# bittremieux/falcon

Hardware: AMD Instinct MI355X
Metric: spectra clustered/sec @1/2/4/8 GPU; cosine-kernel HBM GB/s vs roofline (higher is better)
Workload: dtype f32; 1 GPU; one dataset of 1000000 synthetic spectra (1000000 per GPU; charges 2+3; precursor m/z 400-1200), low_dim=400, n_neighbors=64, n_neighbors_ann=128, n_probe=16, eps=0.1, precursor_tol=20ppm, mz_interval=1.0, batch_size=32768; exchange=none, parallelism=1 GPU

## Files before the change

falcon_amd/_lib.py:

```python
from __future__ import annotations

import ctypes as C
import os
from typing import Optional

_HERE = os.path.dirname(os.path.abspath(__file__))
LIB_PATH = os.path.join(_HERE, "libfalcon_hip.so")

FAL_DTYPE_F32, FAL_DTYPE_F16, FAL_DTYPE_SPLIT16, FAL_OUT_F32_F16, FAL_OUT_F16_IMAGE = 0, 1, 2, 3, 4
PEAK_F64, PEAK_ZLIB, PEAK_BIG_ENDIAN, PEAK_PAIRS = 1, 2, 4, 8
PEAK_NUMPRESS_LINEAR, PEAK_NUMPRESS_PIC, PEAK_NUMPRESS_SLOF, PEAK_NUMPRESS_MASK = 16, 32, 48, 48
PEAK_STATUS = {1: "bad descriptor", 2: "bad base64", 4: "bad zlib header", 8: "bad deflate stream", 16: "more values than declared",
               32: "fewer values than declared", 64: "Adler-32 mismatch", 128: "decode buffer too small",
               256: "bad MS-Numpress stream"}
MGF_FLAG_BYTES, MGF_FLAG_LINES, MGF_ST_HOST = 1, 2, 1
MGF_NUM_MAX = 23
FAL_EINVAL = -1
MZML_FLAG_STRUCT, MZML_FLAG_MARKUP, MZML_FLAG_TAGS = 1, 2, 4
MZML_ST_OK, MZML_ST_SKIP, MZML_ST_HOST = 0, 1, 2
CONS_FALLBACK, CONS_GLOBAL, CONS_CAPACITY, CONS_LDS_PEAKS = 1, 2, 4, 4096
STAGES = {"vectorize": 0, "build": 1, "coarse": 2, "scan": 3, "select": 4, "filter": 5, "dbscan": 6, "tail": 7,
          "kernel": 8}


class FalconHipError(RuntimeError):
    pass


_lib: Optional[C.CDLL] = None

c_void_p, c_int, c_int64, c_uint32, c_float, c_double = C.c_void_p, C.c_int, C.c_int64, C.c_uint32, C.c_float, C.c_double
P = C.POINTER

_SIGNATURES = {
    "fal_version": ([], c_int),
    "fal_last_error": ([], C.c_char_p),
    "fal_device_count": ([P(c_int)], c_int),
    "fal_ctx_create": ([c_int, c_void_p, c_int, P(c_void_p)], c_int),
    "fal_ctx_destroy": ([c_void_p], c_int),
    "fal_ctx_sync": ([c_void_p], c_int),
    "fal_ctx_plan": ([c_void_p, c_int64, c_int, c_int, c_int, c_int64], c_int),
    "fal_ctx_trim": ([c_void_p], c_int),
    "fal_ctx_stage_ms": ([c_void_p, c_int, P(c_float), P(c_int64)], c_int),
    "fal_ctx_enable_timing": ([c_void_p, c_int], c_int),
    "fal_ctx_counter": ([c_void_p, c_int, P(c_int64)], c_int),
    "fal_get_dim": ([c_float, c_float, c_float, P(c_uint32), P(c_float), P(c_float)], c_int),
    "fal_hash_lookup": ([c_uint32, c_uint32, c_uint32, c_void_p], c_int),
    "fal_to_vector_indices": ([c_void_p, c_void_p, c_int64, c_double, c_double, c_void_p], c_int),
    "fal_vectorize": ([c_void_p, c_void_p, c_void_p, c_void_p, c_void_p, c_int64, c_double, c_double,
                       c_uint32, c_uint32, c_uint32, c_int, c_int, c_void_p], c_int),
    "fal_vectorize_pair": ([c_void_p, c_void_p, c_void_p, c_void_p, c_void_p, c_int64, c_double, c_double,
                            c_uint32, c_uint32, c_uint32, c_int, c_void_p, c_void_p], c_int),
    "fal_vectorize_f16_image": ([c_void_p, c_void_p, c_void_p, c_void_p, c_void_p, c_int64, c_double, c_double,
                                 c_uint32, c_uint32, c_uint32, c_int, c_void_p, c_void_p], c_int),
    "fal_row_width": ([c_uint32, P(c_uint32)], c_int),
    "fal_vectorize_rows": ([c_void_p, c_void_p, c_void_p, c_void_p, c_void_p, c_int64, c_double, c_double,
                            c_uint32, c_uint32, c_uint32, c_uint32, c_int, c_int, c_void_p, c_void_p], c_int),
    "fal_window_counts": ([c_void_p, c_void_p, c_void_p, c_int, c_double, c_int64, c_void_p, c_void_p], c_int),
    "fal_window_select": ([c_void_p, c_void_p, c_int64, c_double, c_int64, c_void_p, c_int, c_void_p, c_void_p, P(c_int64)], c_int),
    "fal_precursor_splits": ([c_void_p, c_void_p, c_int64, c_double, c_int, c_int64, c_double, c_int,
                              c_void_p, c_int64, P(c_int64)], c_int),
    "fal_ivf_build": ([c_void_p, c_void_p, c_int64, c_int, c_void_p, c_int64, c_void_p, c_int, P(c_void_p)], c_int),
    "fal_ivf_build_x16": ([c_void_p, c_void_p, c_void_p, c_int64, c_int, c_void_p, c_int64, c_void_p, c_int, P(c_void_p)], c_int),
    "fal_ivf_attach_f16": ([c_void_p, c_void_p, c_int], c_int),
    "fal_ivf_attach_prefilter": ([c_void_p, c_void_p], c_int),
    "fal_ivf_attach_prefilter_ex": ([c_void_p, c_void_p, c_int], c_int),
    "fal_ivf_destroy": ([c_void_p], c_int),
    "fal_ivf_total_lists": ([c_void_p, P(c_int64)], c_int),
    "fal_ivf_export": ([c_void_p, c_void_p, c_void_p, c_void_p, c_void_p, c_void_p], c_int),
    "fal_ivf_search_topk": ([c_void_p, c_void_p, c_int, c_int, c_void_p, c_void_p], c_int),
    "fal_filter_neighbors": ([c_void_p, c_void_p, c_void_p, c_int64, c_int, c_void_p, c_void_p, c_double, c_int,
                              c_double, c_int, c_void_p, c_void_p], c_int),
    "fal_ivf_search_neighbors": ([c_void_p, c_void_p, c_int, c_int, c_void_p, c_void_p, c_double, c_int, c_double, c_int,
                                  c_void_p, c_void_p, c_void_p], c_int),
    "fal_process_spectra": ([c_void_p, c_void_p, c_void_p, c_void_p, c_int64, c_int64, c_void_p, c_void_p, c_int, c_double,
                             c_double, c_double, c_double, c_double, c_int, c_int, c_void_p, c_void_p, c_void_p,
                             c_void_p], c_int),
    "fal_rescore_neighbors": ([c_void_p, c_void_p, c_void_p, c_int64, c_int, c_void_p, c_void_p, c_void_p, c_void_p, c_double,
                               c_int], c_int),
    "fal_neighbors_to_csr": ([c_void_p, c_void_p, c_void_p, c_void_p, c_int64, c_int, c_int64, c_int64, c_void_p, c_void_p, c_void_p],
                             c_int),
    "fal_neighbors_to_csr_mapped": ([c_void_p, c_void_p, c_void_p, c_void_p, c_int64, c_int, c_void_p, c_int64, c_int64, c_void_p,
                                     c_void_p, c_void_p], c_int),
    "fal_dbscan": ([c_void_p, c_void_p, c_void_p, c_int64, c_int, c_float, c_void_p, P(c_int64)], c_int),
    "fal_refine_clusters": ([c_void_p, c_void_p, c_int64, c_void_p, c_void_p, c_double, c_int, c_double,
                             P(c_int64)], c_int),
    "fal_finalize": ([c_void_p, c_void_p, c_int64, c_int64, c_void_p, c_void_p, c_void_p, c_int, c_void_p,
                      c_void_p, P(c_int64)], c_int),
    "fal_cluster_graph": ([c_void_p, c_void_p, c_void_p, c_int64, c_int, c_float, c_void_p, c_void_p, c_double, c_int,
                           c_double, c_void_p, c_void_p, c_void_p, c_void_p, P(c_int64), P(c_int64)], c_int),
    "fal_cluster_graph_counted": ([c_void_p, c_void_p, c_void_p, c_void_p, c_int64, c_int, c_float, c_void_p, c_void_p, c_double,
                                   c_int, c_double, c_void_p, c_void_p, c_void_p, c_void_p, P(c_int64), P(c_int64)], c_int),
    "fal_cluster_graph_linkage": ([c_void_p, c_void_p, c_void_p, c_int64, c_int, c_float, c_int, c_void_p, c_void_p, c_double, c_int,
                                   c_double, c_void_p, c_void_p, c_void_p, c_void_p, P(c_int64), P(c_int64)], c_int),
    "fal_linkage_cluster": ([c_void_p, c_void_p, c_void_p, c_int64, c_int, c_float, c_int, c_void_p, P(c_int64)], c_int),
    "fal_exact_edges": ([c_void_p, c_void_p, c_void_p, c_void_p, c_void_p, c_int64, c_void_p, c_int64, c_double, c_int, c_double,
                         c_void_p, c_void_p, c_void_p, c_int64, P(c_int64)], c_int),
    "fal_linkage_cluster_csr": ([c_void_p, c_void_p, c_void_p, c_void_p, c_int64, c_double, c_int, c_void_p, c_void_p, c_void_p,
                                 c_void_p, c_double, c_int, c_void_p, P(c_int64)], c_int),
    "fal_cluster_exact": ([c_void_p, c_void_p, c_void_p, c_void_p, c_void_p, c_int64, c_void_p, c_int64, c_double, c_int, c_double,
                           c_int, c_void_p, c_void_p, c_double, c_int, c_double, c_void_p, c_void_p, c_void_p, P(c_int64),
                           P(c_int64)], c_int),
    "fal_sort_by_precursor": ([c_void_p, c_void_p, c_int64, c_void_p, c_void_p], c_int),
    "fal_gather_f32": ([c_void_p, c_void_p, c_void_p, c_int64, c_void_p], c_int),
    "fal_decode_peaks": ([c_void_p, c_void_p, c_int64, c_void_p, c_int64, c_void_p, c_int64, c_int64, c_int64, c_void_p, c_void_p,
                          c_void_p, c_void_p], c_int),
    "fal_mgf_index": ([c_void_p, c_void_p, c_int64, P(c_int64)], c_int),
    "fal_mgf_parse": ([c_void_p, c_void_p, c_int64, c_int64, c_int64, c_void_p, c_void_p, c_void_p, c_void_p, c_void_p, c_void_p,
                       c_void_p, c_void_p, c_void_p, c_void_p], c_int),
    "fal_mgf_write_sizes": ([c_void_p, c_void_p, c_void_p, c_void_p, c_int64, c_int64, c_void_p, c_int64, c_void_p, c_void_p, c_void_p,
                             c_void_p, c_void_p, c_int64, c_void_p, c_void_p, P(c_int64)], c_int),
    "fal_mgf_write": ([c_void_p, c_void_p, c_void_p, c_void_p, c_int64, c_int64, c_void_p, c_int64, c_void_p, c_void_p, c_void_p,
                       c_void_p, c_void_p, c_void_p, c_int64, c_void_p, c_int64, c_int64, c_void_p, c_int64, c_void_p], c_int),
    "fal_mzml_index": ([c_void_p, c_void_p, c_int64, P(c_int64)], c_int),
    "fal_mzml_parse": ([c_void_p, c_void_p, c_int64, c_int64, c_void_p, c_int64, c_void_p, c_void_p, c_void_p, c_void_p, c_void_p,
                        c_void_p, c_void_p], c_int),
    "fal_consensus_spectra": ([c_void_p, c_void_p, c_void_p, c_void_p, c_int64, c_void_p, c_void_p, c_int64, c_double, c_double,
                               c_int64, c_void_p, c_void_p, c_void_p, c_void_p], c_int),
    "fal_assign_nearest": ([c_void_p, c_void_p, c_void_p, c_void_p, c_void_p, c_void_p, c_int64, c_void_p, c_void_p, c_void_p,
                            c_void_p, c_void_p, c_int64, c_double, c_int, c_double, c_double, c_int, c_void_p, c_void_p,
                            c_void_p], c_int),
}


def load() -> C.CDLL:
    global _lib
    if _lib is not None:
        return _lib
    if not os.path.isfile(LIB_PATH):
        raise FalconHipError(
            f"{LIB_PATH} is missing: build it with `python -c 'import __graft_entry__ as g; g.build()'` "
            f"(or `make -C falcon_amd/csrc`). falcon_amd has no CPU fallback.")
    import torch
    lib = C.CDLL(LIB_PATH)
    for name, (args, res) in _SIGNATURES.items():
        fn = getattr(lib, name)
        fn.argtypes = args
        fn.restype = res
    _lib = lib
    return lib


def check(rc: int, what: str = "") -> None:
    if rc != 0:
        msg = load().fal_last_error().decode("utf-8", "replace")
        raise FalconHipError(f"{what or 'libfalcon_hip'} failed with code {rc}: {msg}")


def exported_symbols():
    return list(_SIGNATURES)
```

falcon_amd/cluster/cluster.py:

```python
from __future__ import annotations

import logging
import math
from dataclasses import dataclass
from typing import Optional, Tuple

import numpy as np

from .. import device as _device

logger = logging.getLogger("falcon")

F16_INDEX_DIMS = (64, 128, 256, 400, 800)
F16_FLAT_DIMS = (64, 128, 256, 400)
FLAT_MAX = 100
MIN_PTS_PER_LIST = 39
MAX_N_LIST = 1 << 17


class _DefaultClustering(str):
    """AnnParams.clustering's default "dbscan" -- equal to the string, but distinguishable from an explicit choice
    (exact mode turns the default into "hierarchical" and refuses an explicit "dbscan")"""


@dataclass
class AnnParams:
    eps: float = 0.1
    low_dim: int = 400
    n_probe: int = 16
    n_neighbors: int = 64
    n_neighbors_ann: int = 128
    mz_interval: float = 1.0
    kmeans_iters: int = 10
    hash_seed: int = 0
    min_mz: float = 101.0
    max_mz: float = 1500.0
    dtype: str = "f32"
    f16_index: bool = True
    scan: str = "f32"
    prefilter: bool = False
    ivf_prefilter: bool = True
    kmeans_prefilter: bool = True
    rescore: bool = False
    min_matches: int = 0
    clustering: str = _DefaultClustering("dbscan")
    linkage: str = "complete"
    exact: bool = False


def n_list_rule(sizes: np.ndarray, n_probe: int) -> np.ndarray:
    sizes = np.asarray(sizes, np.int64)
    nl = np.ones(len(sizes), np.int64)
    big = sizes > FLAT_MAX
    if big.any():
        nl[big] = 2 ** np.floor(np.log2(sizes[big] / MIN_PTS_PER_LIST)).astype(np.int64)
    nl = np.minimum(nl, MAX_N_LIST)
    nl[nl <= n_probe] = 1
    return nl.astype(np.int32)


class SpectrumDataset:

    def __init__(self, precursor_mz, retention_time, mz, intensity, indptr, precursor_charge=None):
        self.precursor_mz, self.retention_time = precursor_mz, retention_time
        self.mz, self.intensity, self.indptr = mz, intensity, indptr
        self.precursor_charge = precursor_charge

    def __len__(self):
        return int(self.precursor_mz.shape[0])

    def columns(self):
        return (self.precursor_mz, self.retention_time, self.mz, self.intensity, self.indptr)

    def on_host(self) -> bool:
        return not any(t is not None and hasattr(t, "is_cuda") and t.is_cuda for t in self.columns())

    def to_device(self, dev, non_blocking: bool = True) -> "SpectrumDataset":
        import torch
        want = (torch.float32, torch.float32, torch.float32, torch.float32, torch.int64)
        up = []
        for t, dt in zip(self.columns(), want):
            if t is None:
                up.append(None)
                continue
            if not isinstance(t, torch.Tensor):
                t = torch.from_numpy(np.ascontiguousarray(t, dtype=np.float32 if dt == torch.float32 else np.int64))
            up.append(t.to(dev, dtype=dt, non_blocking=non_blocking))
        return SpectrumDataset(*up, self.precursor_charge)

    def take_rows(self, rows: np.ndarray) -> "SpectrumDataset":
        import torch
        as_np = lambda t: t.numpy() if isinstance(t, torch.Tensor) else np.asarray(t)
        rows = np.asarray(rows, np.int64)
        indptr = as_np(self.indptr)
        cnt = indptr[rows + 1] - indptr[rows]
        out = np.zeros(len(rows) + 1, np.int64)
        np.cumsum(cnt, out=out[1:])
        pos = np.repeat(indptr[rows] - out[:-1], cnt) + np.arange(int(out[-1]), dtype=np.int64)

        def pick(col, idx, dt):
            src = as_np(col)
            t = torch.empty(len(idx), dtype=dt, pin_memory=torch.cuda.is_available())
            dst = t.numpy()
            if src.dtype == dst.dtype:
                np.take(src, idx, out=dst)
            else:
                dst[:] = src[idx]
            return t
        rt = None if self.retention_time is None else pick(self.retention_time, rows, torch.float32)
        return SpectrumDataset(pick(self.precursor_mz, rows, torch.float32), rt, pick(self.mz, pos, torch.float32),
                               pick(self.intensity, pos, torch.float32), torch.from_numpy(out), self.precursor_charge)

    @classmethod
    def from_table(cls, table):
        if hasattr(table, "to_pandas"):
            table = table.to_pandas()
        mzs = [np.asarray(x, np.float32) for x in table["mz"]]
        its = [np.asarray(x, np.float32) for x in table["intensity"]]
        indptr = np.zeros(len(mzs) + 1, np.int64)
        np.cumsum([len(x) for x in mzs], out=indptr[1:])
        cat = lambda xs: np.concatenate(xs) if xs else np.zeros(0, np.float32)
        return cls(np.asarray(table["precursor_mz"], np.float32), np.asarray(table["retention_time"], np.float32),
                   cat(mzs), cat(its), indptr,
                   np.asarray(table["precursor_charge"]) if "precursor_charge" in table else None)


class ClusterPipeline:

    def __init__(self, ctx: Optional[_device.Context] = None, device: int = 0):
        self.ctx = ctx or _device.Context(device)
        self.last = {}

    def plan(self, n: int, batch_size: int, p: "AnnParams"):
        if p.exact:
            return
        key = (int(n), int(batch_size), p.low_dim, p.n_neighbors_ann, p.n_probe)
        if getattr(self, "_planned", None) is not None and self._planned[0] >= key[0] and self._planned[1:] == key[1:]:
            return
        self.ctx.plan(n, _device.row_width(p.low_dim), p.n_neighbors_ann, p.n_probe, batch_size)
        self._planned = key

    def trim(self):
        import torch
        for c in (self.ctx, getattr(self, "_front_ctx", None)):
            if c is not None:
                c.trim()
        self._planned = None
        torch.cuda.empty_cache()

    def _front(self, c, ds, precursor_tol_mass, precursor_tol_mode, rt_tol, batch_size, p, pmz=None):
        import torch
        if pmz is None:
            pmz = c.to_dev(ds.precursor_mz, torch.float32)
        order, mzs = c.sort_by_precursor(pmz)
        rts = c.gather_f32(ds.retention_time, order) if (rt_tol is not None and ds.retention_time is not None) else None
        splits = c.precursor_splits(mzs, precursor_tol_mass, precursor_tol_mode, batch_size, p.mz_interval)
        n_list = n_list_rule(np.diff(splits), p.n_probe)
        if p.dtype == "f16" and not p.f16_index:
            n_list[:] = 1
        return dict(order=order, mzs=mzs, rts=rts, splits=splits, n_list=n_list)

    def plan_shards(self, c, datasets, batch_size, p, world, tol=None):
        import torch
        from .. import distributed as fdist
        for ds in datasets:
            if ds.on_host():
                ds._pmz_dev = c.to_dev(ds.precursor_mz, torch.float32)
        counts = c.window_counts([getattr(ds, "_pmz_dev", None) if ds.on_host() else ds.precursor_mz for ds in datasets],
                                 p.mz_interval)
        if p.exact:
            costs = fdist.exact_window_costs(counts, batch_size)
        else:
            costs = fdist.window_costs(counts, batch_size, p.n_probe, p.mz_interval, tol, p.n_neighbors_ann, p.n_neighbors)
        return fdist.deal_job(list(costs), world)

    def _front_windows(self, c, ds, precursor_tol_mass, precursor_tol_mode, rt_tol, batch_size, p, shard, owner=None):
        import torch
        from .. import distributed as fdist
        rank, world = shard[0], shard[1]
        pmz = ds.__dict__.pop("_pmz_dev", None) if ds.on_host() else None
        if pmz is None:
            pmz = c.to_dev(ds.precursor_mz, torch.float32)
        n = int(pmz.numel())
        if owner is None:
            owner = self.plan_shards(c, [ds], batch_size, p, world, tol=(precursor_tol_mass, precursor_tol_mode))[0]
        if len(owner) and (owner == rank).all():
            st = self._front(c, ds, precursor_tol_mass, precursor_tol_mode, rt_tol, batch_size, p, pmz=pmz)
            st.update(rows=st["order"], n_total=n)
            return st
        if not (owner == rank).any():
            rows = torch.zeros(0, dtype=torch.int64, device=c.tdev)
        else:
            rows, mz_sub = c.window_select(pmz, p.mz_interval, owner, rank)
        if rows.numel() == 0:
            e = rows.new_zeros(0)
            return dict(order=e, mzs=pmz[:0], rts=None, splits=np.zeros(1, np.int64), n_list=np.zeros(0, np.int32), rows=e,
                        n_total=n)
        order_sub, mzs = c.sort_by_precursor(mz_sub)
        rows_sorted = rows[order_sub]
        rts = c.gather_f32(ds.retention_time, rows_sorted) if (rt_tol is not None and ds.retention_time is not None) else None
        splits = c.precursor_splits(mzs, precursor_tol_mass, precursor_tol_mode, batch_size, p.mz_interval)
        n_list = n_list_rule(np.diff(splits), p.n_probe)
        if p.dtype == "f16" and not p.f16_index:
            n_list[:] = 1
        return dict(order=rows_sorted, mzs=mzs, rts=rts, splits=splits, n_list=n_list, rows=rows_sorted, n_total=n)

    def _restrict(self, c, st, p, shard):
        import torch
        from .. import distributed as fdist
        rank, world = shard
        splits = np.asarray(st["splits"], np.int64)
        sizes = np.diff(splits)
        costs = fdist.exact_bucket_costs(sizes) if p.exact else fdist.bucket_costs(sizes, st["n_list"], p.n_probe)
        owner = fdist.shard_units(costs, world)
        first, sizes, sub_splits, mine = fdist.shard_buckets(splits, owner, rank)
        n_sub = int(sub_splits[-1])
        if n_sub:
            shift = c.to_dev(np.stack([first - sub_splits[:-1], sizes]), torch.int64)
            pos_d = torch.repeat_interleave(shift[0], shift[1], output_size=n_sub) + torch.arange(n_sub, device=c.tdev)
        order_sub = st["order"][pos_d] if n_sub else st["order"][:0]
        rts = st["rts"]
        return dict(order=order_sub, mzs=st["mzs"][pos_d] if n_sub else st["mzs"][:0],
                    rts=None if rts is None else (rts[pos_d] if n_sub else rts[:0]), splits=sub_splits,
                    n_list=np.asarray(st["n_list"])[mine], rows=order_sub, n_total=int(st["order"].numel()),
                    buckets=mine)

    def _search(self, ds, st, precursor_tol_mass, precursor_tol_mode, rt_tol, fragment_tol, p, keep_intermediates):
        c = self.ctx
        order, mzs, rts, splits, n_list = st["order"], st["mzs"], st["rts"], st["splits"], st["n_list"]
        n_bins, start, _ = _device.get_dim(p.min_mz, p.max_mz, fragment_tol)
        all_flat = bool((n_list == 1).all())
        W = _device.row_width(p.low_dim)
        assert W in F16_INDEX_DIMS
        vec = lambda dt: c.vectorize(ds.mz, ds.intensity, ds.indptr, order, start, fragment_tol, n_bins, p.low_dim,
                                     p.hash_seed, True, dt, width=W)
        X = X16 = Xpre = Xkm = None
        which = 0
        if p.dtype not in ("f32", "f16"):
            raise ValueError(f"unknown dtype {p.dtype!r} (f32 or f16)")
        if p.dtype == "f16" and not all_flat:
            X, X16 = vec("f16+image")
            Xkm = X16 if p.kmeans_prefilter else None
            if p.ivf_prefilter and not keep_intermediates:
                which, Xpre = 2, X16
        elif p.dtype == "f16":
            X16 = vec("f16")
        elif p.scan == "f16x3":
            if W not in F16_FLAT_DIMS:
                raise ValueError(f"scan='f16x3' needs low_dim <= {F16_FLAT_DIMS[-1]} (got {p.low_dim})")
            X16 = vec("split16")
            if not all_flat:
                X = vec("f32")
        else:
            if p.prefilter and not keep_intermediates and W in F16_FLAT_DIMS and bool((n_list == 1).any()):
                which |= 1
            if p.ivf_prefilter and not keep_intermediates and bool((n_list > 1).any()):
                which |= 2
            want_km = p.kmeans_prefilter and bool(((n_list > 1) & (n_list <= 2048)).any())
            if want_km or which:
                X, x16 = vec("f32+f16")
                Xkm = x16 if want_km else None
                Xpre = x16 if which else None
            else:
                X = vec("f32")
        index = c.ivf_build(X, splits, n_list, p.kmeans_iters, X16=X16, Xpre=Xpre, Xkm=Xkm, prefilter_which=max(which, 1))
        if keep_intermediates:
            sim, idx = index.search(p.n_probe, p.n_neighbors_ann)
            nb_idx, nb_dist = c.filter_neighbors(sim, idx, mzs, rts, precursor_tol_mass, precursor_tol_mode, rt_tol,
                                                 p.n_neighbors)
            st.update(sim=sim, idx=idx)
        else:
            nb_idx, nb_dist = index.search_neighbors(p.n_probe, p.n_neighbors_ann, mzs, rts, precursor_tol_mass,
                                                     precursor_tol_mode, rt_tol, p.n_neighbors)
        if p.rescore:
            nb_dist = c.rescore_neighbors(nb_idx, nb_dist, ds.mz, ds.intensity, ds.indptr, order, fragment_tol,
                                          p.min_matches)
        st.update(X=X, X16=X16, Xpre=Xpre, index=index, nb_idx=nb_idx, nb_dist=nb_dist,
                  nb_count=None if keep_intermediates else index.nb_count)

    def _graph(self, st, precursor_tol_mass, precursor_tol_mode, rt_tol, p, keep_intermediates):
        c = self.ctx
        order, mzs, rts, nb_idx, nb_dist, index = (st[k] for k in ("order", "mzs", "rts", "nb_idx", "nb_dist", "index"))
        hier = p.linkage if p.clustering == "hierarchical" else None
        if keep_intermediates:
            db, n_db = c.linkage_cluster(nb_idx, nb_dist, p.eps, hier) if hier else c.dbscan(nb_idx, nb_dist, p.eps)
            last = dict(order=order, mz_sorted=mzs, rt_sorted=rts, splits=st["splits"], X=st["X"], X16=st["X16"],
                        n_list=st["n_list"], sim=st["sim"], idx=st["idx"], nb_idx=nb_idx, nb_dist=nb_dist, db=db.clone(),
                        n_db=n_db, index=index)
            lab, n_cl = c.refine_clusters(db, n_db, mzs, rts, precursor_tol_mass, precursor_tol_mode, rt_tol)
            last.update(lab_sorted=lab, n_clusters=n_cl)
            labels, medoids = c.finalize(lab, n_cl, order, nb_idx, nb_dist)
        else:
            labels, medoids, _, _ = c.cluster_graph(nb_idx, nb_dist, p.eps, mzs, rts, precursor_tol_mass,
                                                    precursor_tol_mode, rt_tol, order, linkage=hier, nb_count=st["nb_count"])
            last = dict(nb_idx=nb_idx, nb_dist=nb_dist, nb_count=st["nb_count"], order=order, n_list=st["n_list"],
                        splits=st["splits"])
            index.close()
        return labels, medoids, last

    def _exact(self, ds, st, precursor_tol_mass, precursor_tol_mode, rt_tol, fragment_tol, p, keep_intermediates):
        c = self.ctx
        order, mzs, rts, splits = (st[k] for k in ("order", "mzs", "rts", "splits"))
        last = dict(order=order, mz_sorted=mzs, rt_sorted=rts, splits=splits, csr=None)
        if keep_intermediates:
            last["csr"] = c.exact_edges(ds.mz, ds.intensity, ds.indptr, order, splits, fragment_tol, p.min_matches, p.eps)
        labels, medoids, lab_sorted, n_cl = c.cluster_exact(ds.mz, ds.intensity, ds.indptr, order, splits, fragment_tol,
                                                            p.min_matches, p.eps, p.linkage, mzs, rts, precursor_tol_mass,
                                                            precursor_tol_mode, rt_tol)
        last.update(lab_sorted=lab_sorted, n_clusters=n_cl)
        return labels, medoids, last

    def run(self, ds: SpectrumDataset, precursor_tol_mass: float, precursor_tol_mode: str,
            rt_tol: Optional[float], fragment_tol: float, batch_size: int, p: AnnParams,
            keep_intermediates: bool = False):
        import torch
        c = self.ctx
        if len(ds) == 0:
            return c.empty((0,), torch.int32), c.empty((0,), torch.int32)
        self.plan(len(ds), batch_size, p)
        st = self._front(c, ds, precursor_tol_mass, precursor_tol_mode, rt_tol, batch_size, p)
        if p.exact:
            labels, medoids, self.last = self._exact(ds, st, precursor_tol_mass, precursor_tol_mode, rt_tol, fragment_tol, p,
                                                     keep_intermediates)
            return labels, medoids
        self._search(ds, st, precursor_tol_mass, precursor_tol_mode, rt_tol, fragment_tol, p, keep_intermediates)
        labels, medoids, self.last = self._graph(st, precursor_tol_mass, precursor_tol_mode, rt_tol, p, keep_intermediates)
        return labels, medoids

    def run_many(self, datasets, precursor_tol_mass: float, precursor_tol_mode: str, rt_tol: Optional[float],
                 fragment_tol: float, batch_size: int, p: AnnParams, shard: Optional[Tuple[int, int]] = None):
        import torch
        c = self.ctx
        if p.exact and shard is not None and shard[1] > 1:
            return self._run_many_exact_sharded(datasets, precursor_tol_mass, precursor_tol_mode, rt_tol, fragment_tol,
                                                batch_size, p, shard)
        if p.exact:
            outs, self.lasts = [], []
            for ds in datasets:
                outs.append(self.run(ds, precursor_tol_mass, precursor_tol_mode, rt_tol, fragment_tol, batch_size, p))
                self.lasts.append(self.last if len(ds) > 0 else {})
            if self.lasts:
                self.last = self.lasts[-1]
            return outs
        args = (precursor_tol_mass, precursor_tol_mode, rt_tol)
        live = [i for i, ds in enumerate(datasets) if len(ds) > 0]
        if live:
            self.plan(max(len(datasets[i]) for i in live), batch_size, p)
        if len(live) > 1 and not hasattr(self, "_front_ctx"):
            self._front_stream = torch.cuda.Stream(device=c.tdev)
            with torch.cuda.stream(self._front_stream):
                self._front_ctx = _device.Context(c.device)
        front_stream = self._front_stream if len(live) > 1 else torch.cuda.current_stream(c.tdev)
        front_ctx = self._front_ctx if len(live) > 1 else c
        states = {}
        sharded = shard is not None and shard[1] > 1
        windows = sharded and bool(p.mz_interval and p.mz_interval > 0)
        owners = None
        if windows:
            owners = shard[2] if len(shard) > 2 else None
            if owners is None:
                front_stream.wait_stream(torch.cuda.current_stream(c.tdev))
                with torch.cuda.stream(front_stream):
                    owners = self.plan_shards(front_ctx, datasets, batch_size, p, shard[1], tol=args[:2])

        def front(i):
            with torch.cuda.stream(front_stream):
                if windows:
                    st = self._front_windows(front_ctx, datasets[i], *args, batch_size, p, shard, owner=owners[i])
                else:
                    st = self._front(front_ctx, datasets[i], *args, batch_size, p)
                    if sharded:
                        st = self._restrict(front_ctx, st, p, shard[:2])
                if sharded:
                    st["order"] = torch.arange(st["rows"].numel(), dtype=torch.int64, device=c.tdev)
                states[i] = st

        if live:
            front_stream.wait_stream(torch.cuda.current_stream(c.tdev))
            front(live[0])
        for pos, i in enumerate(live):
            if states[i]["order"].numel() > 0:
                if sharded and datasets[i].on_host():
                    front_stream.synchronize()
                    sub = datasets[i].take_rows(states[i]["rows"].cpu().numpy())
                    sub = SpectrumDataset(None, None, c.to_dev(sub.mz), c.to_dev(sub.intensity), c.to_dev(sub.indptr))
                    self._search(sub, states[i], *args, fragment_tol, p, False)
                elif sharded:
                    st = dict(states[i], order=states[i]["rows"])
                    torch.cuda.current_stream(c.tdev).wait_stream(front_stream)
                    self._search(datasets[i], st, *args, fragment_tol, p, False)
                    st["order"] = states[i]["order"]
                    states[i] = st
                else:
                    self._search(datasets[i], states[i], *args, fragment_tol, p, False)
            if pos + 1 < len(live):
                front(live[pos + 1])
        outs, self.lasts = [], []
        for i, ds in enumerate(datasets):
            if len(ds) == 0 or states[i]["order"].numel() == 0:
                outs.append((c.empty((0,), torch.int32), c.empty((0,), torch.int32)))
                self.lasts.append({"rows": c.empty((0,), torch.int64)} if sharded else {})
                continue
            labels, medoids, last = self._graph(states[i], *args, p, False)
            if sharded:
                last["rows"] = states[i]["rows"]
            outs.append((labels, medoids))
            self.lasts.append(last)
        if self.lasts:
            self.last = self.lasts[-1]
        return outs

    def _run_many_exact_sharded(self, datasets, precursor_tol_mass, precursor_tol_mode, rt_tol, fragment_tol, batch_size, p,
                                shard):
        import torch
        c = self.ctx
        args = (precursor_tol_mass, precursor_tol_mode, rt_tol)
        windows = bool(p.mz_interval and p.mz_interval > 0)
        owners = shard[2] if len(shard) > 2 else None
        if windows and owners is None:
            owners = self.plan_shards(c, datasets, batch_size, p, shard[1])
        outs, self.lasts = [], []
        for j, ds in enumerate(datasets):
            st = None
            if len(ds) > 0:
                if windows:
                    st = self._front_windows(c, ds, *args, batch_size, p, shard[:2], owner=owners[j])
                else:
                    st = self._restrict(c, self._front(c, ds, *args, batch_size, p), p, shard[:2])
            if st is None or st["rows"].numel() == 0:
                outs.append((c.empty((0,), torch.int32), c.empty((0,), torch.int32)))
                self.lasts.append({"rows": c.empty((0,), torch.int64)})
                continue
            rows = st["rows"]
            st["order"] = torch.arange(rows.numel(), dtype=torch.int64, device=c.tdev)
            labels, medoids, last = self._exact(self._take_rows(c, ds, rows), st, *args, fragment_tol, p, False)
            last["rows"] = rows
            outs.append((labels, medoids))
            self.lasts.append(last)
        if self.lasts:
            self.last = self.lasts[-1]
        return outs

    @staticmethod
    def _take_rows(c, ds, rows):
        import torch
        if ds.on_host():
            sub = ds.take_rows(rows.cpu().numpy())
            return SpectrumDataset(None, None, c.to_dev(sub.mz), c.to_dev(sub.intensity), c.to_dev(sub.indptr))
        indptr = c.to_dev(ds.indptr, torch.int64)
        start = indptr[rows]
        cnt = indptr[rows + 1] - start
        out = torch.zeros(rows.numel() + 1, dtype=torch.int64, device=c.tdev)
        torch.cumsum(cnt, 0, out=out[1:])
        nnz = int(out[-1].item())
        pos = torch.repeat_interleave(start - out[:-1], cnt, output_size=nnz) + torch.arange(nnz, device=c.tdev)
        return SpectrumDataset(None, None, c.to_dev(ds.mz, torch.float32)[pos], c.to_dev(ds.intensity, torch.float32)[pos],
                               out)

    def run_chunked(self, datasets, precursor_tol_mass: float, precursor_tol_mode: str, rt_tol: Optional[float],
                    fragment_tol: float, batch_size: int, p: AnnParams, n_chunks: int, on_chunk=None):
        import torch
        c = self.ctx
        if n_chunks <= 1 or p.exact:
            return self.run_many(datasets, precursor_tol_mass, precursor_tol_mode, rt_tol, fragment_tol, batch_size, p)
        labels = [torch.full((len(ds),), -1, dtype=torch.int32, device=c.tdev) for ds in datasets]
        medoids = [[] for _ in datasets]
        off = [0] * len(datasets)
        for ch in range(n_chunks):
            outs = self.run_many(datasets, precursor_tol_mass, precursor_tol_mode, rt_tol, fragment_tol, batch_size, p,
                                 shard=(ch, n_chunks))
            _merge_share(labels, medoids, off, outs, self.lasts)
            if on_chunk is not None:
                on_chunk(ch, outs, self.lasts)
            del outs
        return [(labels[j], torch.cat(medoids[j]) if medoids[j] else c.empty((0,), torch.int32)) for j in range(len(datasets))]


def _merge_share(labels, medoids, off, outs, lasts):
    import torch
    for j, ((lab, med), last) in enumerate(zip(outs, lasts)):
        rows = last.get("rows")
        if rows is None or rows.numel() == 0:
            continue
        labels[j][rows] = lab + off[j]
        medoids[j].append(rows[med.long()].to(torch.int32))
        off[j] += int(med.numel())


class PartitionRunner:

    def __init__(self, device: int = 0, n_slots: int = 2):
        import threading
        from concurrent.futures import ThreadPoolExecutor
        self.device, self.n_slots = device, n_slots
        self._tls = threading.local()
        self._pool = ThreadPoolExecutor(max_workers=n_slots, thread_name_prefix="falcon-part")
        self.pipelines = []
        self._lock = threading.Lock()

    def _pipeline(self):
        import torch
        if not hasattr(self._tls, "pipe"):
            torch.cuda.set_device(self.device)
            self._tls.stream = torch.cuda.Stream(device=self.device)
            with torch.cuda.stream(self._tls.stream):
                self._tls.pipe = ClusterPipeline(device=self.device)
            with self._lock:
                self.pipelines.append(self._tls.pipe)
        return self._tls.pipe, self._tls.stream

    def _run_one(self, ds, args, kwargs, shard, arrived=None):
        import torch
        pipe, stream = self._pipeline()
        with torch.cuda.stream(stream):
            if arrived is not None:
                stream.wait_event(arrived)
            if shard is not None and shard[1] > 1:
                out = pipe.run_many([ds], *args, shard=shard, **kwargs)[0]
                pipe.last = pipe.lasts[0]
            else:
                out = pipe.run(ds, *args, **kwargs)
            stream.synchronize()
        return out, pipe, dict(pipe.last)

    def run(self, datasets, *args, shard: Optional[Tuple[int, int]] = None, **kwargs):
        return self.collect(self.submit(datasets, *args, shard=shard, **kwargs))

    def collect(self, handle):
        futs, n, nothing = handle
        res = [futs[i].result()[::2] if i in futs else nothing() for i in range(n)]
        self.lasts = [r[1] for r in res]
        return [r[0] for r in res]

    def submit(self, datasets, *args, shard: Optional[Tuple[int, int]] = None, inputs_ready: bool = False, **kwargs):
        import torch
        if not inputs_ready:
            torch.cuda.current_stream(self.device).synchronize()
        p = args[5] if len(args) > 5 else kwargs["p"]
        order = sorted(range(len(datasets)), key=lambda i: -len(datasets[i]))
        shards = [shard] * len(datasets)
        if shard is not None and shard[1] > 1 and p.mz_interval and p.mz_interval > 0:
            if not hasattr(self, "_planner"):
                self._planner = ClusterPipeline(device=self.device)
            owners = self._planner.plan_shards(self._planner.ctx, datasets, args[4], p, shard[1], tol=args[:2])
            shards = [(shard[0], shard[1], [owners[i]]) for i in range(len(datasets))]
            order = [i for i in order if (owners[i] == shard[0]).any()]
        dev = torch.device("cuda", self.device)
        arrived = {}
        sharded = shard is not None and shard[1] > 1
        if not sharded and any(datasets[i].on_host() for i in order):
            if not hasattr(self, "_copy_stream"):
                self._copy_stream = torch.cuda.Stream(device=self.device)
            datasets = list(datasets)
            with torch.cuda.stream(self._copy_stream):
                for i in order:
                    if datasets[i].on_host():
                        datasets[i] = datasets[i].to_device(dev)
                        arrived[i] = torch.cuda.Event()
                        arrived[i].record(self._copy_stream)
        futs = {i: self._pool.submit(self._run_one, datasets[i], args, kwargs, shards[i], arrived.get(i)) for i in order}
        nothing = lambda: ((torch.empty(0, dtype=torch.int32, device=dev), torch.empty(0, dtype=torch.int32, device=dev)),
                           {"rows": torch.empty(0, dtype=torch.int64, device=dev)})
        return futs, len(datasets), nothing

    def plan(self, datasets, *args, **kwargs):
        import threading
        n = max((len(ds) for ds in datasets), default=0)
        batch_size, p = args[4], args[5]
        gate = threading.Barrier(self.n_slots)

        def one():
            pipe, stream = self._pipeline()
            import torch
            with torch.cuda.stream(stream):
                pipe.plan(n, batch_size, p)
            gate.wait()
        for f in [self._pool.submit(one) for _ in range(self.n_slots)]:
            f.result()

    def trim(self):
        with self._lock:
            pipes = list(self.pipelines)
        for pipe in pipes + ([self._planner] if hasattr(self, "_planner") else []):
            pipe.trim()

    def run_chunked(self, datasets, *args, n_chunks: int, on_chunk=None, **kwargs):
        import torch
        if n_chunks <= 1 or (args[5] if len(args) > 5 else kwargs["p"]).exact:
            return self.run(datasets, *args, **kwargs)
        dev = torch.device("cuda", self.device)
        labels = [torch.full((len(ds),), -1, dtype=torch.int32, device=dev) for ds in datasets]
        medoids = [[] for _ in datasets]
        off = [0] * len(datasets)
        for ch in range(n_chunks):
            outs = self.run(datasets, *args, shard=(ch, n_chunks), **kwargs)
            _merge_share(labels, medoids, off, outs, self.lasts)
            if on_chunk is not None:
                on_chunk(ch, outs, self.lasts)
            del outs
        return [(labels[j], torch.cat(medoids[j]) if medoids[j] else torch.empty(0, dtype=torch.int32, device=dev))
                for j in range(len(datasets))]

    def close(self):
        self._pool.shutdown(wait=True)


_default_pipeline: Optional[ClusterPipeline] = None


def resolve_params(linkage: str, distance_threshold: float, min_matches: int, ann: Optional[AnnParams] = None) -> AnnParams:
    import dataclasses
    if linkage not in ("complete", "single", "average"):
        raise ValueError(f"unknown linkage {linkage!r} (choose complete, single or average; cluster.py:283-290)")
    if ann is None:
        p = AnnParams(eps=float(distance_threshold))
    else:
        if abs(float(ann.eps) - float(distance_threshold)) > 1e-12:
            raise ValueError(f"distance_threshold ({distance_threshold}) and ann.eps ({ann.eps}) differ: they name the same "
                             "cosine-distance threshold (README.md:73-79, config.py:104-111)")
        p = dataclasses.replace(ann)
    if p.rescore:
        p.min_matches = int(min_matches)
    if p.exact:
        if p.clustering == "dbscan" and not isinstance(p.clustering, _DefaultClustering):
            raise ValueError("exact mode clusters the all-pairs distances hierarchically (the snapshot's linkage); "
                             "AnnParams(exact=True) does not combine with clustering=\"dbscan\"")
        p.clustering = "hierarchical"
    if p.clustering not in ("dbscan", "hierarchical"):
        raise ValueError(f"unknown clustering {p.clustering!r}")
    if p.clustering == "hierarchical":
        p.linkage = linkage
        p.rescore = True
        p.min_matches = int(min_matches)
    elif linkage != "complete":
        raise ValueError(f"linkage={linkage!r} only applies to the hierarchical clustering of the exact distances "
                         "(AnnParams(clustering=\"hierarchical\", rescore=True) / --clustering hierarchical); the default "
                         "nearest-neighbour path clusters with DBSCAN and would ignore it")
    return p


def generate_clusters(dataset, linkage: str, distance_threshold: float, min_matches: int,
                      precursor_tol_mass: float, precursor_tol_mode: str, rt_tol: Optional[float],
                      fragment_tol: float, batch_size: int, *, ann: Optional[AnnParams] = None,
                      pipeline: Optional[ClusterPipeline] = None) -> Tuple[np.ndarray, np.ndarray]:
    global _default_pipeline
    if not isinstance(dataset, SpectrumDataset):
        dataset = SpectrumDataset.from_table(
            dataset.to_table(columns=["precursor_mz", "precursor_charge", "retention_time", "mz", "intensity"])
            if hasattr(dataset, "to_table") else dataset)
    p = resolve_params(linkage, distance_threshold, min_matches, ann)
    pipe = pipeline or _default_pipeline
    if pipe is None:
        pipe = _default_pipeline = ClusterPipeline()
    logger.info("Cluster %d spectra: low_dim=%d n_probe=%d n_neighbors=%d/%d eps=%.3f", len(dataset), p.low_dim,
                p.n_probe, p.n_neighbors, p.n_neighbors_ann, p.eps)
    labels, medoids = pipe.run(dataset, precursor_tol_mass, precursor_tol_mode, rt_tol, fragment_tol, batch_size, p)
    return labels.cpu().numpy(), medoids.cpu().numpy()


def consensus_spectra(dataset, labels, medoids, fragment_tol: float, min_fraction: float = 0.25,
                      pipeline: Optional[ClusterPipeline] = None):
    global _default_pipeline
    if not isinstance(dataset, SpectrumDataset):
        dataset = SpectrumDataset.from_table(
            dataset.to_table(columns=["precursor_mz", "precursor_charge", "retention_time", "mz", "intensity"])
            if hasattr(dataset, "to_table") else dataset)
    if not 0.0 < float(min_fraction) <= 1.0:
        raise ValueError("min_fraction must lie in (0, 1]")
    pipe = pipeline or _default_pipeline
    if pipe is None:
        pipe = _default_pipeline = ClusterPipeline()
    indptr, mz, intensity, status = pipe.ctx.consensus_spectra(dataset.mz, dataset.intensity, dataset.indptr, labels, medoids,
                                                               fragment_tol, min_fraction)
    return indptr.cpu().numpy(), mz.cpu().numpy(), intensity.cpu().numpy(), status.cpu().numpy()


def write_representatives(filename: str, dataset: SpectrumDataset, medoids, cluster_ids, identifiers, charge: int = 0,
                          consensus=None, pipeline: Optional[ClusterPipeline] = None) -> str:
    global _default_pipeline
    from ..ms_io import ms_io
    pipe = pipeline or _default_pipeline
    if pipe is None:
        pipe = _default_pipeline = ClusterPipeline()
    if dataset.retention_time is None:
        raise ValueError("write_representatives: the dataset has no retention times")
    ctx = pipe.ctx
    import torch
    m = ctx.to_dev(medoids, torch.int64)
    n = int(m.shape[0])
    if consensus is None:
        indptr, mz, intensity, rows = dataset.indptr, dataset.mz, dataset.intensity, m.to(torch.int32)
    else:
        indptr, mz, intensity = consensus
        rows = np.arange(n, dtype=np.int32)
    pmz, rt = ctx.to_dev(dataset.precursor_mz, torch.float32)[m], ctx.to_dev(dataset.retention_time, torch.float32)[m]
    return ms_io.write_representatives(filename, ctx, mz, intensity, indptr, rows, pmz, rt, np.full(n, int(charge), np.int32),
                                       cluster_ids, np.asarray(identifiers, dtype=str))


def assign_to_library(queries: SpectrumDataset, library: SpectrumDataset, eps: float, precursor_tol: float, mode: str,
                      rt_tol: Optional[float], fragment_tol: float, min_matched_peaks: int,
                      pipeline: Optional[ClusterPipeline] = None):
    global _default_pipeline
    pipe = pipeline or _default_pipeline
    if pipe is None:
        pipe = _default_pipeline = ClusterPipeline()
    if mode not in ("ppm", "Da"):
        raise ValueError(f"unknown precursor tolerance mode {mode!r} (ppm or Da)")
    row, dist, cand = pipe.ctx.assign_nearest(queries.mz, queries.intensity, queries.indptr, queries.precursor_mz,
                                              queries.retention_time, library.mz, library.intensity, library.indptr,
                                              library.precursor_mz, library.retention_time, precursor_tol, mode, rt_tol,
                                              fragment_tol, min_matched_peaks)
    row, dist, cand = row.cpu().numpy(), dist.cpu().numpy(), cand.cpu().numpy()
    return row, dist, cand, (row >= 0) & (dist <= np.float32(eps))
```

falcon_amd/csrc/common.h:

```cpp
#pragma once
#include <hip/hip_runtime.h>
#include <stdint.h>
#include <stdio.h>
#include <string.h>
#include <string>
#include <vector>
#include "../../include/falcon_hip.h"

namespace fal {

void set_error(const char* fmt, ...);

#define FAL_CHECK_HIP(expr)                                                          \
    do {                                                                             \
        hipError_t _e = (expr);                                                      \
        if (_e != hipSuccess) {                                                      \
            fal::set_error("%s:%d: %s failed: %s", __FILE__, __LINE__, #expr,        \
                           hipGetErrorString(_e));                                   \
            return (_e == hipErrorOutOfMemory) ? FAL_ENOMEM : FAL_EHIP;              \
        }                                                                            \
    } while (0)

#define FAL_REQUIRE(cond, code, ...)                                                 \
    do {                                                                             \
        if (!(cond)) {                                                               \
            fal::set_error(__VA_ARGS__);                                             \
            return (code);                                                           \
        }                                                                            \
    } while (0)

#define FAL_TRY(expr)                                                                \
    do {                                                                             \
        int _r = (expr);                                                             \
        if (_r != FAL_OK) return _r;                                                 \
    } while (0)

constexpr int kNumStages = 9;
constexpr int kNumSlots = 50;
enum Stage { ST_VECTORIZE = 0, ST_BUILD = 1, ST_COARSE = 2, ST_SCAN = 3, ST_SELECT = 4,
             ST_FILTER = 5, ST_DBSCAN = 6, ST_TAIL = 7,
             ST_KERNEL = 8 };

struct Scratch {
    void* ptr = nullptr;
    size_t cap = 0;
};

}

struct fal_ctx {
    int device = -1;
    hipStream_t stream = nullptr;
    bool own_stream = false;
    void* pinned = nullptr;
    size_t pinned_cap = 0;
    int pinned_reserve(size_t bytes, void** out);
    unsigned char* arena = nullptr;
    size_t arena_off = 0;
    int upload(void* dst, const void* src, size_t bytes);
    int num_cus = 256;
    int persistent_wgs = 256;
    bool timing = false;
    struct StageTimer {
        std::vector<std::pair<hipEvent_t, hipEvent_t>> ev;
        size_t used = 0;
    } timers[fal::kNumStages];
    fal::Scratch scratch[fal::kNumSlots];
    int32_t* fb_host = nullptr;
    int32_t* zero_dev = nullptr;
    int64_t counters[10] = {0, 0, 0, 0, 0, 0, 0, 0, 0, 0};

    struct TextIndex {
        const void* text = nullptr;
        int64_t bytes = -1, spectra = 0, extra = 0, cap_table = 0, cap_spectra = 0;
        const void* blocks[4] = {nullptr, nullptr, nullptr, nullptr};
    } mgf, mzml;

    struct PoolBlock { void* ptr; size_t cap; bool used; };
    std::vector<PoolBlock> pool;
    int pool_alloc(size_t bytes, void** out);
    void pool_free(void* ptr);

    bool debug_poison = false;
    int call_depth = 0;
    uint64_t call_epoch = 1;
    uint64_t slot_epoch[fal::kNumSlots] = {};
    uint32_t slot_gen[fal::kNumSlots] = {};
    std::vector<void*> retired;
    std::vector<bool> retired_held;
    void release_retired();
    int reserve(int slot, size_t bytes, void** out);
    void release(int slot) { slot_epoch[slot] = 0; }
    void stage_reset(int stage);
    int stage_begin(int stage, hipEvent_t* stop_out, hipStream_t on = nullptr);
    int stage_end(hipEvent_t stop, hipStream_t on = nullptr);
};

namespace fal {

struct StageScope {
    fal_ctx* c;
    hipEvent_t stop = nullptr;
    bool on;
    hipStream_t s;
    StageScope(fal_ctx* ctx, int stage, hipStream_t stream = nullptr, bool enable = true)
        : c(ctx), on(ctx->timing && enable), s(stream) {
        if (on) c->stage_begin(stage, &stop, s);
    }
    ~StageScope() {
        if (on && stop) c->stage_end(stop, s);
    }
};

struct CallScope {
    fal_ctx* c;
    explicit CallScope(fal_ctx* ctx) : c(ctx) {
        if (c && c->call_depth++ == 0) {
            ++c->call_epoch;
            if (!c->retired.empty()) c->release_retired();
        }
    }
    ~CallScope() {
        if (c) --c->call_depth;
    }
};

static inline int64_t ceil_div(int64_t a, int64_t b) { return (a + b - 1) / b; }

struct WarmReg {
    explicit WarmReg(const void* kernel);
};
#define FAL_WARM_KERNEL(...) static const ::fal::WarmReg _fal_warm_reg((const void*)(__VA_ARGS__))

__device__ __forceinline__ void wave_lds_sync() {
    __builtin_amdgcn_fence(__ATOMIC_RELEASE, "workgroup");
    __builtin_amdgcn_wave_barrier();
    asm volatile("" ::: "memory");
}

typedef unsigned short ushort2v __attribute__((ext_vector_type(2)));
__device__ __forceinline__ uint32_t pk_sub(uint32_t x, uint32_t y) {
    return __builtin_bit_cast(uint32_t, (ushort2v)(__builtin_bit_cast(ushort2v, x) - __builtin_bit_cast(ushort2v, y)));
}
__device__ __forceinline__ uint32_t pk_add(uint32_t x, uint32_t y) {
    return __builtin_bit_cast(uint32_t, (ushort2v)(__builtin_bit_cast(ushort2v, x) + __builtin_bit_cast(ushort2v, y)));
}
__device__ __forceinline__ uint32_t pk_sub_sat(uint32_t x, uint32_t y) {
    uint32_t r;
    asm("v_pk_sub_u16 %0, %1, %2 clamp" : "=v"(r) : "v"(x), "v"(y));
    return r;
}
__device__ __forceinline__ uint32_t pk_min(uint32_t x, uint32_t y) {
    uint32_t r;
    asm("v_pk_min_u16 %0, %1, %2" : "=v"(r) : "v"(x), "v"(y));
    return r;
}
__device__ __forceinline__ uint32_t pk_max(uint32_t x, uint32_t y) {
    uint32_t r;
    asm("v_pk_max_u16 %0, %1, %2" : "=v"(r) : "v"(x), "v"(y));
    return r;
}

#define FAL_DPP_SCAN(v, OP, IDENT)                                                                  \
    v = OP(v, __builtin_amdgcn_update_dpp(IDENT, v, 0x111, 0xF, 0xF, false));                       \
    v = OP(v, __builtin_amdgcn_update_dpp(IDENT, v, 0x112, 0xF, 0xF, false));                       \
    v = OP(v, __builtin_amdgcn_update_dpp(IDENT, v, 0x114, 0xF, 0xF, false));                       \
    v = OP(v, __builtin_amdgcn_update_dpp(IDENT, v, 0x118, 0xF, 0xF, false));                       \
    v = OP(v, __builtin_amdgcn_update_dpp(IDENT, v, 0x142, 0xA, 0xF, false));                       \
    v = OP(v, __builtin_amdgcn_update_dpp(IDENT, v, 0x143, 0xC, 0xF, false));
__device__ __forceinline__ int fal_add_i(int a, int b) { return a + b; }
__device__ __forceinline__ int fal_min_i(int a, int b) { return a < b ? a : b; }
__device__ __forceinline__ int fal_max_i(int a, int b) { return a > b ? a : b; }
__device__ __forceinline__ int wave_prefix_sum(int v) {
    FAL_DPP_SCAN(v, fal_add_i, 0)
    return v;
}
__device__ __forceinline__ int wave_min(int v) {
    FAL_DPP_SCAN(v, fal_min_i, 0x7FFFFFFF)
    return __builtin_amdgcn_readlane(v, 63);
}
__device__ __forceinline__ uint32_t wave_min_u32(uint32_t u) {
    int v = (int)(u ^ 0x80000000u);
    FAL_DPP_SCAN(v, fal_min_i, 0x7FFFFFFF)
    return (uint32_t)__builtin_amdgcn_readlane(v, 63) ^ 0x80000000u;
}
__device__ __forceinline__ uint32_t wave_max_u32(uint32_t u) {
    int v = (int)(u ^ 0x80000000u);
    FAL_DPP_SCAN(v, fal_max_i, (int)0x80000000)
    return (uint32_t)__builtin_amdgcn_readlane(v, 63) ^ 0x80000000u;
}

__device__ __forceinline__ int row16_sum(int v) {
    v += __builtin_amdgcn_update_dpp(0, v, 0x121, 0xF, 0xF, false);
    v += __builtin_amdgcn_update_dpp(0, v, 0x122, 0xF, 0xF, false);
    v += __builtin_amdgcn_update_dpp(0, v, 0x124, 0xF, 0xF, false);
    v += __builtin_amdgcn_update_dpp(0, v, 0x128, 0xF, 0xF, false);
    return v;
}

__device__ __forceinline__ int row16_prefix_sum(int v) {
    v += __builtin_amdgcn_update_dpp(0, v, 0x111, 0xF, 0xF, true);
    v += __builtin_amdgcn_update_dpp(0, v, 0x112, 0xF, 0xF, true);
    v += __builtin_amdgcn_update_dpp(0, v, 0x114, 0xF, 0xF, true);
    v += __builtin_amdgcn_update_dpp(0, v, 0x118, 0xF, 0xF, true);
    return v;
}

#define FAL_DMA_BARRIER() asm volatile("s_waitcnt vmcnt(0) lgkmcnt(0)\n\ts_barrier" ::: "memory")

__device__ __forceinline__ void lds_dma16(const void* g, const void* lds) {
    const uint32_t l = (uint32_t)__builtin_amdgcn_readfirstlane((int)(uint32_t)(size_t)(__attribute__((address_space(3))) const void*)lds);
    asm volatile("s_mov_b32 m0, %1\n\ts_nop 0\n\tglobal_load_lds_dwordx4 %0, off" ::"v"(g), "s"(l) : "memory", "m0");
}

}
```

falcon_amd/csrc/core.hip:

```cpp
#include <math.h>
#include <stdarg.h>
#include <stdlib.h>
#include <string.h>
#include "common.h"
#include "hash.h"
#include "scan.h"
#include "ivf.h"
#include <algorithm>

#include <chrono>
namespace fal {
static bool trace_alloc() {
    static int v = -1;
    if (v < 0) {
        const char* e = getenv("FALCON_TRACE_ALLOC");
        v = e && e[0] && e[0] != '0';
    }
    return v == 1;
}
static hipError_t traced_malloc(void** p, size_t bytes, const char* what, int id) {
    if (!trace_alloc()) return hipMalloc(p, bytes);
    const auto t0 = std::chrono::steady_clock::now();
    const hipError_t e = hipMalloc(p, bytes);
    const double ms = std::chrono::duration<double, std::milli>(std::chrono::steady_clock::now() - t0).count();
    fprintf(stderr, "[falcon alloc] %s %d: %.1f MB in %.2f ms\n", what, id, bytes / 1048576.0, ms);
    return e;
}
static std::vector<const void*>& warm_kernels() {
    static std::vector<const void*> v;
    return v;
}
WarmReg::WarmReg(const void* kernel) { warm_kernels().push_back(kernel); }
static thread_local char g_err[512] = "";
void set_error(const char* fmt, ...) {
    va_list ap;
    va_start(ap, fmt);
    vsnprintf(g_err, sizeof(g_err), fmt, ap);
    va_end(ap);
}
}

void fal_ctx::release_retired() {
    if (retired.empty()) return;
    (void)hipStreamSynchronize(stream);
    for (void* p : retired) (void)hipFree(p);
    retired.clear();
    retired_held.clear();
}

int fal_ctx::reserve(int slot, size_t bytes, void** out) {
    fal::Scratch& s = scratch[slot];
    if (bytes > s.cap) {
        if (s.ptr) {
            if (debug_poison && call_depth > 0 && slot_epoch[slot] == call_epoch) {
                fal::set_error("scratch slot %d grows (%zu -> %zu bytes) after it was reserved earlier in the same call: "
                               "a pointer into its old block would be stale", slot, s.cap, bytes);
                return FAL_EINTERNAL;
            }
            if (call_depth > 0) {
                retired.push_back(s.ptr);
                retired_held.push_back(slot_epoch[slot] == call_epoch);
            } else {
                FAL_CHECK_HIP(hipStreamSynchronize(stream));
                FAL_CHECK_HIP(hipFree(s.ptr));
            }
            s.ptr = nullptr;
            s.cap = 0;
        }
        const size_t want = bytes + bytes / 8 + 256;
        hipError_t e = fal::traced_malloc(&s.ptr, want, "slot", slot);
        if (e == hipErrorOutOfMemory && !retired.empty()) {
            (void)hipGetLastError();
            (void)hipStreamSynchronize(stream);
            size_t kept = 0;
            for (size_t i = 0; i < retired.size(); ++i) {
                if (retired_held[i]) {
                    retired[kept] = retired[i];
                    retired_held[kept++] = true;
                } else {
                    (void)hipFree(retired[i]);
                }
            }
            retired.resize(kept);
            retired_held.resize(kept);
            e = hipMalloc(&s.ptr, want);
            if (e == hipErrorOutOfMemory) {
                (void)hipGetLastError();
                fal::set_error("out of device memory: scratch slot %d needs %zu bytes (%zu retired block(s) of this call are still "
                               "referenced and cannot be freed before it returns)", slot, want, kept);
                return FAL_ENOMEM;
            }
        }
        FAL_CHECK_HIP(e);
        s.cap = want;
        ++slot_gen[slot];
        if (debug_poison) FAL_CHECK_HIP(hipMemsetAsync(s.ptr, 0xFF, want, stream));
    }
    slot_epoch[slot] = call_epoch;
    *out = s.ptr;
    return FAL_OK;
}

int fal_ctx::pool_alloc(size_t bytes, void** out) {
    if (bytes == 0) bytes = 16;
    int best = -1;
    for (size_t i = 0; i < pool.size(); ++i)
        if (!pool[i].used && pool[i].cap >= bytes && (best < 0 || pool[i].cap < pool[best].cap)) best = (int)i;
    if (best >= 0 && pool[best].cap <= 2 * bytes + (1 << 20)) {
        pool[best].used = true;
        *out = pool[best].ptr;
        if (debug_poison) FAL_CHECK_HIP(hipMemsetAsync(pool[best].ptr, 0xFF, pool[best].cap, stream));
        return FAL_OK;
    }
    void* p = nullptr;
    const size_t cap = bytes + bytes / 16 + 256;
    FAL_CHECK_HIP(fal::traced_malloc(&p, cap, "pool", (int)pool.size()));
    pool.push_back({p, cap, true});
    if (debug_poison) FAL_CHECK_HIP(hipMemsetAsync(p, 0xFF, cap, stream));
    *out = p;
    return FAL_OK;
}

void fal_ctx::pool_free(void* ptr) {
    if (!ptr) return;
    for (auto& b : pool)
        if (b.ptr == ptr) {
            b.used = false;
            return;
        }
}

void fal_ctx::stage_reset(int stage) { timers[stage].used = 0; }

int fal_ctx::pinned_reserve(size_t bytes, void** out) {
    if (bytes > pinned_cap) {
        if (pinned) FAL_CHECK_HIP(hipHostFree(pinned));
        pinned = nullptr;
        pinned_cap = 0;
        FAL_CHECK_HIP(hipHostMalloc(&pinned, bytes + 4096, hipHostMallocDefault));
        pinned_cap = bytes + 4096;
    }
    *out = pinned;
    return FAL_OK;
}

int fal_ctx::upload(void* dst, const void* src, size_t bytes) {
    constexpr size_t kArena = 32u << 20;
    if (bytes == 0) return FAL_OK;
    if (bytes > kArena / 4) {
        FAL_CHECK_HIP(hipMemcpyAsync(dst, src, bytes, hipMemcpyHostToDevice, stream));
        return FAL_OK;
    }
    if (!arena) FAL_CHECK_HIP(hipHostMalloc((void**)&arena, kArena, hipHostMallocDefault));
    size_t off = (arena_off + 63) & ~(size_t)63;
    if (off + bytes > kArena) {
        FAL_CHECK_HIP(hipStreamSynchronize(stream));
        off = 0;
    }
    memcpy(arena + off, src, bytes);
    FAL_CHECK_HIP(hipMemcpyAsync(dst, arena + off, bytes, hipMemcpyHostToDevice, stream));
    arena_off = off + bytes;
    return FAL_OK;
}

int fal_ctx::stage_begin(int stage, hipEvent_t* stop_out, hipStream_t on) {
    StageTimer& t = timers[stage];
    if (t.used == t.ev.size()) {
        hipEvent_t a, b;
        FAL_CHECK_HIP(hipEventCreate(&a));
        FAL_CHECK_HIP(hipEventCreate(&b));
        t.ev.push_back({a, b});
    }
    FAL_CHECK_HIP(hipEventRecord(t.ev[t.used].first, on ? on : stream));
    *stop_out = t.ev[t.used].second;
    t.used++;
    return FAL_OK;
}

int fal_ctx::stage_end(hipEvent_t stop, hipStream_t on) {
    FAL_CHECK_HIP(hipEventRecord(stop, on ? on : stream));
    return FAL_OK;
}

extern "C" {

int fal_version(void) { return 100; }

const char* fal_last_error(void) { return fal::g_err; }

int fal_device_count(int* count) {
    FAL_REQUIRE(count, FAL_EINVAL, "fal_device_count: NULL");
    int n = 0;
    hipError_t e = hipGetDeviceCount(&n);
    if (e != hipSuccess) n = 0;
    *count = n;
    return FAL_OK;
}

int fal_ctx_create(int device, void* stream, int own_stream, fal_ctx** out) {
    FAL_REQUIRE(out, FAL_EINVAL, "fal_ctx_create: out is NULL");
    *out = nullptr;
    int n = 0;
    if (hipGetDeviceCount(&n) != hipSuccess || n <= 0) {
        fal::set_error("fal_ctx_create: no HIP device visible (this library has no CPU fallback)");
        return FAL_ENODEV;
    }
    FAL_REQUIRE(device >= 0 && device < n, FAL_EINVAL, "fal_ctx_create: device %d out of range [0,%d)", device, n);
    FAL_CHECK_HIP(hipSetDevice(device));
    hipDeviceProp_t prop;
    FAL_CHECK_HIP(hipGetDeviceProperties(&prop, device));
    if (strncmp(prop.gcnArchName, "gfx950", 6) != 0) {
        fal::set_error("fal_ctx_create: device %d is %s; this library is built for gfx950 only", device, prop.gcnArchName);
        return FAL_ENODEV;
    }
    fal_ctx* c = new fal_ctx();
    c->device = device;
    c->num_cus = prop.multiProcessorCount;
    c->persistent_wgs = c->num_cus;
    if (const char* e = getenv("FALCON_PERSISTENT_WGS")) {
        const int v = atoi(e);
        if (v >= 8 && v <= c->num_cus) c->persistent_wgs = v;
    }
    if (!own_stream) {
        c->stream = (hipStream_t)stream;
        c->own_stream = false;
    } else {
        hipError_t e = hipStreamCreateWithFlags(&c->stream, hipStreamNonBlocking);
        if (e != hipSuccess) {
            delete c;
            fal::set_error("hipStreamCreate failed: %s", hipGetErrorString(e));
            return FAL_EHIP;
        }
        c->own_stream = true;
    }
    if (hipHostMalloc((void**)&c->fb_host, 64, hipHostMallocDefault) != hipSuccess ||
        hipMalloc((void**)&c->zero_dev, 64) != hipSuccess || hipMemset(c->zero_dev, 0, 64) != hipSuccess) {
        fal::set_error("fal_ctx_create: cannot allocate the context's counters");
        fal_ctx_destroy(c);
        return FAL_ENOMEM;
    }
    memset(c->fb_host, 0, 64);
    const char* dbg = getenv("FALCON_DEBUG_POISON");
    c->debug_poison = dbg && dbg[0] && dbg[0] != '0';
    *out = c;
    return FAL_OK;
}

int fal_ctx_destroy(fal_ctx* c) {
    if (!c) return FAL_OK;
    (void)hipSetDevice(c->device);
    (void)hipStreamSynchronize(c->stream);
    for (auto& s : c->scratch)
        if (s.ptr) (void)hipFree(s.ptr);
    for (void* p : c->retired) (void)hipFree(p);
    for (auto& b : c->pool) (void)hipFree(b.ptr);
    if (c->pinned) (void)hipHostFree(c->pinned);
    if (c->fb_host) (void)hipHostFree(c->fb_host);
    if (c->zero_dev) (void)hipFree(c->zero_dev);
    if (c->arena) (void)hipHostFree(c->arena);
    for (auto& t : c->timers)
        for (auto& p : t.ev) {
            (void)hipEventDestroy(p.first);
            (void)hipEventDestroy(p.second);
        }
    if (c->own_stream) (void)hipStreamDestroy(c->stream);
    delete c;
    return FAL_OK;
}

int fal_ctx_plan(fal_ctx* c, int64_t n, int low_dim, int k_ann, int n_probe, int64_t batch_size) {
    fal::CallScope _call(c);
    FAL_REQUIRE(c && n >= 0 && low_dim >= 1 && k_ann >= 1 && n_probe >= 1 && batch_size >= 1, FAL_EINVAL, "fal_ctx_plan: bad argument");
    FAL_CHECK_HIP(hipSetDevice(c->device));
    for (const void* k : fal::warm_kernels()) {
        hipFuncAttributes attr;
        FAL_CHECK_HIP(hipFuncGetAttributes(&attr, k));
    }
    if (!c->arena) FAL_CHECK_HIP(hipHostMalloc((void**)&c->arena, (size_t)32u << 20, hipHostMallocDefault));
    if (n == 0) return FAL_OK;
    void* p = nullptr;
    using namespace fal;
    const size_t nn = (size_t)n;
    FAL_TRY(c->reserve(SLOT_SORT, 24 * nn + 4096, &p));
    FAL_TRY(c->reserve(SLOT_SORT2, 12 * nn + 4096, &p));
    {
        const char* e = getenv("FALCON_SIMS_MB");
        size_t cap = (e ? (size_t)atoll(e) : 2048) * 1024 * 1024;
        const double need = 4.0 * (double)nn * (double)std::min<int64_t>(n, std::min<int64_t>(batch_size, 4096));
        if (need < (double)cap) cap = (size_t)need;
        FAL_TRY(c->reserve(SLOT_SIMS, cap + sizeof(float) * kSimsSlack, &p));
    }
    for (int slot : {SLOT_DB, SLOT_DB2, SLOT_TAIL, SLOT_TAIL2, SLOT_FIN, SLOT_FIN2}) FAL_TRY(c->reserve(slot, 8 * nn + 4096, &p));
    for (int slot = 0; slot < fal::kNumSlots; ++slot) c->release(slot);
    return FAL_OK;
}

int fal_ctx_trim(fal_ctx* c) {
    fal::CallScope _call(c);
    FAL_REQUIRE(c, FAL_EINVAL, "fal_ctx_trim: NULL ctx");
    FAL_CHECK_HIP(hipStreamSynchronize(c->stream));
    c->release_retired();
    for (auto& s : c->scratch)
        if (s.ptr) {
            (void)hipFree(s.ptr);
            s.ptr = nullptr;
            s.cap = 0;
        }
    size_t kept = 0;
    for (size_t i = 0; i < c->pool.size(); ++i) {
        if (c->pool[i].used) c->pool[kept++] = c->pool[i];
        else (void)hipFree(c->pool[i].ptr);
    }
    c->pool.resize(kept);
    return FAL_OK;
}

int fal_ctx_sync(fal_ctx* c) {
    fal::CallScope _call(c);
    FAL_REQUIRE(c, FAL_EINVAL, "fal_ctx_sync: NULL ctx");
    FAL_CHECK_HIP(hipStreamSynchronize(c->stream));
    return FAL_OK;
}

int fal_ctx_enable_timing(fal_ctx* c, int on) {
    FAL_REQUIRE(c, FAL_EINVAL, "NULL ctx");
    c->timing = on != 0;
    return FAL_OK;
}

int fal_ctx_counter(fal_ctx* c, int which, int64_t* value) {
    FAL_REQUIRE(c && value && which >= 0 && which < 10, FAL_EINVAL, "fal_ctx_counter: bad argument");
    *value = c->counters[which];
    if (which == 5) *value = c->fb_host ? (int64_t)c->fb_host[0] + (int64_t)c->fb_host[2] : 0;
    return FAL_OK;
}

int fal_ctx_stage_ms(fal_ctx* c, int stage, float* ms, int64_t* launches) {
    fal::CallScope _call(c);
    FAL_REQUIRE(c && ms && stage >= 0 && stage < fal::kNumStages, FAL_EINVAL, "fal_ctx_stage_ms: bad argument");
    FAL_CHECK_HIP(hipStreamSynchronize(c->stream));
    float total = 0.f;
    auto& t = c->timers[stage];
    for (size_t i = 0; i < t.used; ++i) {
        float x = 0.f;
        FAL_CHECK_HIP(hipEventElapsedTime(&x, t.ev[i].first, t.ev[i].second));
        total += x;
    }
    *ms = total;
    if (launches) *launches = (int64_t)t.used;
    return FAL_OK;
}

int fal_get_dim(float min_mz, float max_mz, float bin_size, uint32_t* dim, float* start_dim, float* end_dim) {
    FAL_REQUIRE(dim && start_dim && end_dim, FAL_EINVAL, "fal_get_dim: NULL output");
    FAL_REQUIRE(bin_size > 0.f && max_mz >= min_mz, FAL_EINVAL, "fal_get_dim: need bin_size > 0 and max_mz >= min_mz");
    volatile float s = min_mz - fmodf(min_mz, bin_size);
    volatile float t = max_mz + bin_size;
    volatile float e = t - fmodf(max_mz, bin_size);
    volatile float w = e - s;
    volatile float q = w / bin_size;
    *start_dim = s;
    *end_dim = e;
    *dim = (uint32_t)ceilf(q);
    return FAL_OK;
}

int fal_hash_lookup(uint32_t n_bins, uint32_t low_dim, uint32_t seed, uint32_t* out_table) {
    FAL_REQUIRE(out_table && low_dim > 0, FAL_EINVAL, "fal_hash_lookup: bad argument");
    for (uint32_t i = 0; i < n_bins; ++i) out_table[i] = fal::murmur3_32(i, seed) % low_dim;
    return FAL_OK;
}

}
```

falcon_amd/csrc/ivf.h:

```cpp
#pragma once
#include <vector>
#include "common.h"

namespace fal {
constexpr int kSparseW = 64;
constexpr uint16_t kColPad = 0xFFFF;
constexpr uint16_t kColDense = 0xFFFE;

enum { SLOT_JOBS = 0, SLOT_SIMS = 1, SLOT_PROBES = 2, SLOT_PROBE_SIM = 3, SLOT_QOFF = 4, SLOT_JOBS2 = 5,
       SLOT_MISC = 6, SLOT_MISC2 = 7, SLOT_SORT = 8, SLOT_SORT2 = 9, SLOT_TAIL = 10, SLOT_TAIL2 = 11,
       SLOT_TAIL3 = 12, SLOT_TAIL4 = 13, SLOT_DB = 14, SLOT_DB2 = 15, SLOT_DB3 = 16, SLOT_FIN = 17, SLOT_FIN2 = 18,
       SLOT_FIN3 = 19, SLOT_INV = 20, SLOT_INVCNT = 21, SLOT_SIMS2 = 22, SLOT_TILEJOB = 23, SLOT_FUSED = 24, SLOT_FUSED2 = 25, SLOT_FUSED3 = 26, SLOT_JOBS3 = 27, SLOT_WIN = 28, SLOT_CURSORS = 29, SLOT_ITEMS = 30,
       SLOT_EXACT = 31, SLOT_EXACT2 = 32, SLOT_EXACT3 = 33, SLOT_EXACT4 = 34, SLOT_EXACT5 = 35, SLOT_EXACT6 = 36,
       SLOT_MGF = 37, SLOT_MGF2 = 38, SLOT_MGF3 = 39, SLOT_MGF4 = 40, SLOT_MGF5 = 41,
       SLOT_ASSIGN = 42, SLOT_ASSIGN2 = 43,
       SLOT_MZML = 44, SLOT_MZML2 = 45, SLOT_MZML3 = 46, SLOT_MZML4 = 47, SLOT_MZML5 = 48,
       SLOT_MGFW = 49 };
static_assert(SLOT_MGF2 == SLOT_MGF + 1 && SLOT_MGF3 == SLOT_MGF + 2 && SLOT_MGF4 == SLOT_MGF + 3 && SLOT_MZML2 == SLOT_MZML + 1 &&
                  SLOT_MZML3 == SLOT_MZML + 2 && SLOT_MZML4 == SLOT_MZML + 3,
              "fal::matches (textscan.h) addresses the four slots of an index as first + i");
int launch_exclusive_scan(fal_ctx* ctx, const int64_t* in, int64_t n, int64_t* out);
}
struct fal_ivf;
namespace fal {
int ivf_ensure_xl(fal_ctx* ctx, const fal_ivf* ivf);
}

struct fal_ivf {
    fal_ctx* ctx = nullptr;
    int64_t n = 0;
    int d = 0;
    const float* X = nullptr;
    const float* Xl = nullptr;
    float* Xl_owned = nullptr;
    const void* X16 = nullptr;
    int x16_planes = 0;
    const void* Xpre = nullptr;
    int rows_signed = 0;
    int rows_f16 = 0;
    int32_t* neg_dev = nullptr;
    const void* X16pre = nullptr;
    int32_t* pos_of_row = nullptr;
    int ckeys_stride = 0;
    uint16_t* ckeys = nullptr;
    std::vector<int64_t> bucket_off;
    std::vector<int32_t> n_list;
    std::vector<int64_t> list_base;
    int64_t total_lists = 0;
    int n_ivf_buckets = 0;
    int64_t ivf_waves = 0;
    float* centroids = nullptr;
    int32_t* assign = nullptr;
    int32_t* perm = nullptr;
    uint16_t* sp_cols = nullptr;
    float* sp_vals = nullptr;
    uint16_t* sq16 = nullptr;
    int rows_many = 0;
    int64_t* list_off = nullptr;
    int64_t* counts = nullptr;
    void* bk_dev = nullptr;
};
```

falcon_amd/csrc/tail.hip:

```cpp
#include <math.h>
#include "common.h"
#include "ivf.h"
#include "util.h"

namespace fal {

struct RefineScratch {
    float* val;
    int32_t* ord;
    float* smin;
    float* smax;
    int32_t* sid;
    int32_t* zl;
    int32_t* zr;
    double* zmd;
    int32_t* t_a;
    int32_t* t_b;
    int32_t* stack;
    int32_t* visit;
};

__device__ __forceinline__ double link_dist(float hi, float lo, bool ppm) {
    const float diff = hi - lo;
    return ppm ? (double)(diff / lo) * 1e6 : (double)diff;
}

__device__ void flat_cut_1d(const RefineScratch& S, int64_t o, int m, double t, bool ppm, bool exact,
                            int32_t* __restrict__ T, int lane) {
    const float* val = S.val + o;
    int32_t* ord = S.ord + o;
    float *smin = S.smin + o, *smax = S.smax + o;
    int32_t *sid = S.sid + o, *zl = S.zl + o, *zr = S.zr + o, *stack = S.stack + o, *visit = S.visit + o;
    double* zmd = S.zmd + o;
    for (int e = lane; e < m; e += 64) {
        const float v = val[e];
        int rank = 0;
        for (int j = 0; j < m; ++j) {
            const float w = val[j];
            rank += (w < v) || (w == v && j < e);
        }
        ord[rank] = e;
    }
    __syncthreads();
    for (int s = lane; s < m; s += 64) {
        const int e = ord[s];
        smin[s] = smax[s] = val[e];
        sid[s] = e;
    }
    __syncthreads();
    int nseg = m, n_merge = 0;
    for (int it = 0; it < m - 1; ++it) {
        double best = INFINITY;
        int bs = 0x7fffffff;
        for (int s = lane; s < nseg - 1; s += 64) {
            const double dd = link_dist(smax[s + 1], smin[s], ppm);
            if (dd < best) {
                best = dd;
                bs = s;
            }
        }
#pragma unroll
        for (int off = 32; off >= 1; off >>= 1) {
            const double ob = __shfl_xor(best, off, 64);
            const int os = __shfl_xor(bs, off, 64);
            if (ob < best || (ob == best && os < bs)) {
                best = ob;
                bs = os;
            }
        }
        if (bs == 0x7fffffff) bs = 0;
        if (!exact && !(best <= t)) break;
        if (lane == 0) {
            const int l = sid[bs], r = sid[bs + 1];
            double md = best;
            if (l >= m) md = fmax(md, zmd[l - m]);
            if (r >= m) md = fmax(md, zmd[r - m]);
            zl[it] = l;
            zr[it] = r;
            zmd[it] = md;
            smax[bs] = smax[bs + 1];
            sid[bs] = m + it;
        }
        __syncthreads();
        for (int s0 = bs + 1; s0 < nseg - 1; s0 += 64) {
            const int s = s0 + lane;
            float a = 0.f, b = 0.f;
            int c = 0;
            const bool on = s < nseg - 1;
            if (on) {
                a = smin[s + 1];
                b = smax[s + 1];
                c = sid[s + 1];
            }
            __syncthreads();
            if (on) {
                smin[s] = a;
                smax[s] = b;
                sid[s] = c;
            }
            __syncthreads();
        }
        --nseg;
        ++n_merge;
    }
    if (!exact) {
        if (lane == 0) {
            for (int it = 0; it < n_merge; ++it) {
                const int l = zl[it], r = zr[it];
                stack[it] = (l >= m ? stack[l - m] : 1) + (r >= m ? stack[r - m] : 1);
            }
            int p = 0;
            for (int s = 0; s < nseg; ++s) {
                const int id = sid[s];
                const int sz = id >= m ? stack[id - m] : 1;
                for (int q = 0; q < sz; ++q) visit[p++] = s;
            }
        }
        __syncthreads();
        for (int p = lane; p < m; p += 64) T[ord[p]] = visit[p];
        __syncthreads();
        return;
    }
    if (lane == 0) {
        for (int i = 0; i < m - 1; ++i) visit[i] = 0;
        int k = 0, n_cluster = 0, leader = -1;
        stack[0] = 2 * m - 2;
        while (k >= 0) {
            const int root = stack[k] - m;
            const int lc = zl[root], rc = zr[root];
            if (leader == -1 && zmd[root] <= t) {
                leader = root;
                ++n_cluster;
            }
            if (lc >= m && !visit[lc - m]) {
                visit[lc - m] = 1;
                stack[++k] = lc;
                continue;
            }
            if (rc >= m && !visit[rc - m]) {
                visit[rc - m] = 1;
                stack[++k] = rc;
                continue;
            }
            if (lc < m) {
                if (leader == -1) ++n_cluster;
                T[lc] = n_cluster - 1;
            }
            if (rc < m) {
                if (leader == -1) ++n_cluster;
                T[rc] = n_cluster - 1;
            }
            if (leader == root) leader = -1;
            --k;
        }
    }
    __syncthreads();
}

__device__ __forceinline__ void sort_rows(int32_t* __restrict__ rows, int32_t* __restrict__ tmp, int m, int lane) {
    for (int e = lane; e < m; e += 64) tmp[e] = rows[e];
    __syncthreads();
    for (int e = lane; e < m; e += 64) {
        const int32_t v = tmp[e];
        int rank = 0;
        for (int j = 0; j < m; ++j) rank += tmp[j] < v;
        rows[rank] = v;
    }
    __syncthreads();
}

__global__ __launch_bounds__(64) void refine_kernel(int32_t* __restrict__ rows, const int64_t* __restrict__ seg,
                                                    const int64_t* __restrict__ d_count,
                                                    const float* __restrict__ mz, const float* __restrict__ rt,
                                                    double tol, int is_da, double rt_tol, RefineScratch S,
                                                    int32_t* __restrict__ sub, int32_t* __restrict__ n_sub) {
    const int lane = threadIdx.x;
    const int64_t C = *d_count;
    const bool use_rt = rt != nullptr && rt_tol >= 0.0;
    constexpr int kLdsMembers = 64;
    __shared__ __align__(8) unsigned char lds[kLdsMembers * (8 + 11 * 4)];
    RefineScratch L;
    {
        L.zmd = reinterpret_cast<double*>(lds);
        float* f = reinterpret_cast<float*>(lds + 8 * kLdsMembers);
        L.val = f;
        L.smin = f + kLdsMembers;
        L.smax = f + 2 * kLdsMembers;
        int32_t* q = reinterpret_cast<int32_t*>(f + 3 * kLdsMembers);
        L.ord = q;
        L.sid = q + kLdsMembers;
        L.zl = q + 2 * kLdsMembers;
        L.zr = q + 3 * kLdsMembers;
        L.t_a = q + 4 * kLdsMembers;
        L.t_b = q + 5 * kLdsMembers;
        L.stack = q + 6 * kLdsMembers;
        L.visit = q + 7 * kLdsMembers;
    }
    for (int64_t c = blockIdx.x; c < C; c += gridDim.x) {
        const int64_t o = seg[c];
        const int m = (int)(seg[c + 1] - o);
        int32_t* out = sub + o;
        __syncthreads();
        if (m < 2) {
            for (int e = lane; e < m; e += 64) out[e] = -1;
            if (lane == 0) n_sub[c] = 0;
            continue;
        }
        {
            float vmin = INFINITY, vmax = -INFINITY, rmin = INFINITY, rmax = -INFINITY;
            bool bad = false;
            for (int e = lane; e < m; e += 64) {
                const int32_t rr = rows[o + e];
                const float v = mz[rr];
                bad = bad || !(v == v);
                vmin = fminf(vmin, v);
                vmax = fmaxf(vmax, v);
                if (use_rt) {
                    const float u = rt[rr];
                    bad = bad || !(u == u);
                    rmin = fminf(rmin, u);
                    rmax = fmaxf(rmax, u);
                }
            }
#pragma unroll
            for (int off = 32; off >= 1; off >>= 1) {
                vmin = fminf(vmin, __shfl_xor(vmin, off, 64));
                vmax = fmaxf(vmax, __shfl_xor(vmax, off, 64));
                rmin = fminf(rmin, __shfl_xor(rmin, off, 64));
                rmax = fmaxf(rmax, __shfl_xor(rmax, off, 64));
            }
            bool one = !__any(bad) && link_dist(vmax, vmin, !is_da) <= tol;
            if (use_rt) one = one && link_dist(rmax, rmin, false) <= rt_tol;
            if (one) {
                for (int e = lane; e < m; e += 64) out[e] = 0;
                if (lane == 0) n_sub[c] = 1;
                continue;
            }
        }
        const bool small = m <= kLdsMembers;
        const RefineScratch& W = small ? L : S;
        const int64_t wo = small ? 0 : o;
        sort_rows(rows + o, W.stack + wo, m, lane);
        int32_t* A = W.t_a + wo;
        for (int e = lane; e < m; e += 64) W.val[wo + e] = mz[rows[o + e]];
        __syncthreads();
        flat_cut_1d(W, wo, m, tol, !is_da, use_rt, A, lane);
        if (use_rt) {
            int32_t* B = W.t_b + wo;
            for (int e = lane; e < m; e += 64) W.val[wo + e] = rt[rows[o + e]];
            __syncthreads();
            flat_cut_1d(W, wo, m, rt_tol, false, true, B, lane);
            int32_t* V = W.stack + wo;
            int32_t* first = W.visit + wo;
            for (int e = lane; e < m; e += 64) V[e] = A[e] * 2 + B[e] * 3;
            __syncthreads();
            for (int e = lane; e < m; e += 64) {
                bool f = true;
                for (int j = 0; j < e && f; ++j) f = V[j] != V[e];
                first[e] = f;
            }
            __syncthreads();
            for (int e = lane; e < m; e += 64) {
                int r = 0;
                for (int j = 0; j < m; ++j) r += first[j] && V[j] < V[e];
                A[e] = r;
            }
            __syncthreads();
        }
        int mx = 0;
        for (int e = lane; e < m; e += 64) mx = max(mx, A[e]);
#pragma unroll
        for (int off = 32; off >= 1; off >>= 1) mx = max(mx, __shfl_xor(mx, off, 64));
        const int n_flat = mx + 1;
        if (n_flat == 1) {
            for (int e = lane; e < m; e += 64) out[e] = 0;
            if (lane == 0) n_sub[c] = 1;
            continue;
        }
        if (n_flat == m) {
            for (int e = lane; e < m; e += 64) out[e] = -1;
            if (lane == 0) n_sub[c] = 0;
            continue;
        }
        int32_t* fo = W.ord + wo;
        for (int e = lane; e < m; e += 64) {
            int cnt = 0, f = -1;
            for (int j = 0; j < m; ++j) {
                if (A[j] == A[e]) {
                    if (f < 0) f = j;
                    ++cnt;
                }
            }
            fo[e] = cnt >= 2 ? f : -1;
        }
        __syncthreads();
        int total = 0;
        for (int e = lane; e < m; e += 64) {
            int id = -1;
            if (fo[e] >= 0) {
                id = 0;
                for (int j = 0; j < fo[e]; ++j) id += fo[j] == j;
            }
            out[e] = id;
            total += fo[e] == e;
        }
#pragma unroll
        for (int off = 32; off >= 1; off >>= 1) total += __shfl_xor(total, off, 64);
        if (lane == 0) n_sub[c] = total;
    }
}

__global__ void label_hist_kernel(const int32_t* __restrict__ labels, int64_t n, int32_t* __restrict__ counts) {
    for (int64_t i = blockIdx.x * (int64_t)blockDim.x + threadIdx.x; i < n; i += (int64_t)gridDim.x * blockDim.x)
        if (labels[i] >= 0) atomicAdd(&counts[labels[i]], 1);
}

__global__ void member_scatter_kernel(const int32_t* __restrict__ labels, int64_t n, const int64_t* __restrict__ seg,
                                      int32_t* __restrict__ cursor, int32_t* __restrict__ rows) {
    for (int64_t i = blockIdx.x * (int64_t)blockDim.x + threadIdx.x; i < n; i += (int64_t)gridDim.x * blockDim.x) {
        const int32_t l = labels[i];
        if (l >= 0) rows[seg[l] + atomicAdd(&cursor[l], 1)] = (int32_t)i;
    }
}

__global__ __launch_bounds__(64) void relabel_kernel(const int32_t* __restrict__ rows, const int64_t* __restrict__ seg,
                                                     const int64_t* __restrict__ d_count,
                                                     const int32_t* __restrict__ sub, const int64_t* __restrict__ base,
                                                     int32_t* __restrict__ labels) {
    const int64_t C = *d_count;
    for (int64_t c = blockIdx.x; c < C; c += gridDim.x) {
        const int64_t o = seg[c];
        const int m = (int)(seg[c + 1] - o);
        for (int e = threadIdx.x; e < m; e += 64) labels[rows[o + e]] = sub[o + e] >= 0 ? (int32_t)(base[c] + sub[o + e]) : -1;
    }
}

__global__ void cluster_size_kernel(const int32_t* __restrict__ labels, int64_t n, int32_t* __restrict__ size,
                                    const int64_t* __restrict__ row_order, int32_t* __restrict__ noise_by_dataset_row) {
    for (int64_t i = blockIdx.x * (int64_t)blockDim.x + threadIdx.x; i < n; i += (int64_t)gridDim.x * blockDim.x) {
        const int32_t l = labels[i];
        if (l >= 0) atomicAdd(&size[l], 1);
        noise_by_dataset_row[row_order[i]] = l < 0;
    }
}

__global__ __launch_bounds__(256) void medoid_score_kernel(const int32_t* __restrict__ labels, int64_t n,
                                                           const int32_t* __restrict__ nb_idx,
                                                           const float* __restrict__ nb_dist, int k,
                                                           const int32_t* __restrict__ extent,
                                                           const int32_t* __restrict__ size,
                                                           unsigned long long* __restrict__ best) {
    const int lane = threadIdx.x & 63;
    for (int64_t i = blockIdx.x * 4ll + (threadIdx.x >> 6); i < n; i += (int64_t)gridDim.x * 4) {
        const int32_t l = labels[i];
        if (l < 0) continue;
        float s = 0.f;
        int same = 0;
        const int ext = extent ? extent[i] : k;
        for (int c0 = 0; c0 < ext; c0 += 64) {
            const int c = c0 + lane;
            int32_t j = -1;
            float dv = 0.f;
            if (c < ext) {
                j = nb_idx[i * k + c];
                dv = nb_dist[i * k + c];
            }
            const bool in = j >= 0 && (int64_t)j < n && (int64_t)j != i && labels[j] == l;
            uint64_t mask = __ballot(in);
            same += __popcll(mask);
            while (mask) {
                const int b = __ffsll((unsigned long long)mask) - 1;
                mask &= mask - 1;
                s += __shfl(dv, b, 64);
            }
        }
        if (lane == 0) {
            s += (float)(size[l] - 1 - same);
            const unsigned long long key = ((unsigned long long)__float_as_uint(s) << 32) | (unsigned long long)(uint32_t)i;
            atomicMin(&best[l], key);
        }
    }
}

__global__ __launch_bounds__(256) void medoid_score_rows_kernel(const int32_t* __restrict__ labels, int64_t n,
                                                                const int32_t* __restrict__ nb_idx,
                                                                const float* __restrict__ nb_dist, int k,
                                                                const int32_t* __restrict__ extent,
                                                                const int32_t* __restrict__ size,
                                                                unsigned long long* __restrict__ best) {
    for (int64_t i = blockIdx.x * (int64_t)blockDim.x + threadIdx.x; i < n; i += (int64_t)gridDim.x * blockDim.x) {
        const int32_t l = labels[i];
        if (l < 0) continue;
        float s = 0.f;
        int same = 0;
        const int ext = min(extent[i], k);
        for (int c = 0; c < ext; ++c) {
            const int32_t j = nb_idx[i * k + c];
            if (j >= 0 && (int64_t)j < n && (int64_t)j != i && labels[j] == l) {
                s += nb_dist[i * k + c];
                ++same;
            }
        }
        s += (float)(size[l] - 1 - same);
        const unsigned long long key = ((unsigned long long)__float_as_uint(s) << 32) | (unsigned long long)(uint32_t)i;
        atomicMin(&best[l], key);
    }
}

__global__ void finalize_kernel(const int32_t* __restrict__ labels, int64_t n, const int64_t* __restrict__ d_count,
                                const int64_t* __restrict__ row_order, const int64_t* __restrict__ noise_rank,
                                const unsigned long long* __restrict__ best, int32_t* __restrict__ labels_out,
                                int32_t* __restrict__ medoids_out) {
    const int64_t n_clusters = *d_count;
    for (int64_t i = blockIdx.x * (int64_t)blockDim.x + threadIdx.x; i < n; i += (int64_t)gridDim.x * blockDim.x) {
        const int64_t ds = row_order[i];
        const int32_t l = labels[i];
        if (l >= 0) {
            labels_out[ds] = l;
        } else {
            const int64_t r = n_clusters + noise_rank[ds];
            labels_out[ds] = (int32_t)r;
            medoids_out[r] = (int32_t)ds;
        }
        if (i < n_clusters) medoids_out[i] = (int32_t)row_order[(uint32_t)(best[i] & 0xFFFFFFFFull)];
    }
}

}
FAL_WARM_KERNEL(fal::refine_kernel);

using namespace fal;

int fal::refine_dev(fal_ctx* ctx, int32_t* labels, int64_t n, const float* mz, const float* rt, double tol, int is_da,
                    double rt_tol, const int64_t* d_count_in, int64_t** d_count_out) {
    hipStream_t st = ctx->stream;
    const int64_t cmax = n + 1;
    int32_t *counts = nullptr, *rows = nullptr;
    int64_t *seg = nullptr, *base = nullptr;
    unsigned char* slab = nullptr;
    FAL_TRY(ctx->reserve(SLOT_TAIL, sizeof(int32_t) * (size_t)(3 * cmax + 2 * n) + 64, (void**)&counts));
    int32_t* cursor = counts + cmax;
    int32_t* n_sub = cursor + cmax;
    rows = n_sub + cmax;
    int32_t* sub = rows + n;
    FAL_TRY(ctx->reserve(SLOT_TAIL2, sizeof(int64_t) * (size_t)(2 * (cmax + 2)), (void**)&seg));
    base = seg + (cmax + 2);
    const size_t per = 4 * 11 + 8;
    FAL_TRY(ctx->reserve(SLOT_TAIL4, per * (size_t)n + 256, (void**)&slab));
    RefineScratch S;
    S.zmd = reinterpret_cast<double*>(slab);
    float* f = reinterpret_cast<float*>(slab + 8 * (size_t)n);
    S.val = f;            S.smin = f + n;       S.smax = f + 2 * n;
    int32_t* q = reinterpret_cast<int32_t*>(f + 3 * n);
    S.ord = q;            S.sid = q + n;        S.zl = q + 2 * n;     S.zr = q + 3 * n;
    S.t_a = q + 4 * n;    S.t_b = q + 5 * n;    S.stack = q + 6 * n;  S.visit = q + 7 * n;
    const int grid = (int)std::min<int64_t>(ceil_div(n, 256), (int64_t)ctx->num_cus * 16);
    const int cgrid = (int)std::min<int64_t>(cmax, (int64_t)ctx->num_cus * 32);
    FAL_CHECK_HIP(hipMemsetAsync(counts, 0, sizeof(int32_t) * (size_t)(3 * cmax), st));
    {
        StageScope ts(ctx, ST_TAIL);
        hipLaunchKernelGGL(label_hist_kernel, dim3(grid), dim3(256), 0, st, labels, n, counts);
        FAL_TRY(device_scan_i32(ctx, counts, cmax, seg, SLOT_TAIL3));
        hipLaunchKernelGGL(member_scatter_kernel, dim3(grid), dim3(256), 0, st, labels, n, seg, cursor, rows);
        hipLaunchKernelGGL(refine_kernel, dim3(cgrid), dim3(64), 0, st, rows, seg, d_count_in, mz,
                           rt_tol >= 0.0 ? rt : nullptr, tol, is_da, rt_tol, S, sub, n_sub);
        FAL_TRY(device_scan_i32(ctx, n_sub, cmax, base, SLOT_TAIL3));
        hipLaunchKernelGGL(relabel_kernel, dim3(cgrid), dim3(64), 0, st, rows, seg, d_count_in, sub, base, labels);
    }
    FAL_CHECK_HIP(hipGetLastError());
    *d_count_out = base + cmax;
    return FAL_OK;
}

int fal::finalize_dev(fal_ctx* ctx, const int32_t* labels_sorted, int64_t n, const int64_t* d_count,
                      const int64_t* row_order, const int32_t* nb_idx, const float* nb_dist, int k,
                      int32_t* labels_out, int32_t* medoids_out, int64_t** d_noise_out, const int32_t* extent,
                      const ExactPeaks* exact) {
    hipStream_t st = ctx->stream;
    const int64_t cmax = n + 1;
    int32_t *size = nullptr, *noise = nullptr;
    unsigned long long* best = nullptr;
    int64_t* rank = nullptr;
    FAL_TRY(ctx->reserve(SLOT_FIN, sizeof(int32_t) * (size_t)(n + cmax + 2), (void**)&size));
    noise = size + cmax + 1;
    FAL_TRY(ctx->reserve(SLOT_FIN2, sizeof(unsigned long long) * (size_t)(cmax + 1), (void**)&best));
    FAL_TRY(ctx->reserve(SLOT_FIN3, sizeof(int64_t) * (size_t)(n + 1), (void**)&rank));
    FAL_CHECK_HIP(hipMemsetAsync(size, 0, sizeof(int32_t) * (size_t)(cmax + 1), st));
    FAL_CHECK_HIP(hipMemsetAsync(best, 0xFF, sizeof(unsigned long long) * (size_t)(cmax + 1), st));
    const int grid = (int)std::min<int64_t>(ceil_div(n, 256), (int64_t)ctx->num_cus * 16);
    {
        StageScope ts(ctx, ST_TAIL);
        hipLaunchKernelGGL(cluster_size_kernel, dim3(grid), dim3(256), 0, st, labels_sorted, n, size, row_order, noise);
        if (exact)
            FAL_TRY(exact_medoids_dev(ctx, *exact, labels_sorted, n, size, best));
        else if (extent)
            hipLaunchKernelGGL(medoid_score_rows_kernel, dim3((unsigned)std::min<int64_t>(ceil_div(n, 256), (int64_t)ctx->num_cus * 32)),
                               dim3(256), 0, st, labels_sorted, n, nb_idx, nb_dist, k, extent, size, best);
        else
            hipLaunchKernelGGL(medoid_score_kernel, dim3((unsigned)std::min<int64_t>(ceil_div(n, 4), (int64_t)ctx->num_cus * 64)), dim3(256), 0, st, labels_sorted, n, nb_idx, nb_dist, k, extent, size, best);
        FAL_TRY(device_scan_i32(ctx, noise, n, rank, SLOT_TAIL3));
        hipLaunchKernelGGL(finalize_kernel, dim3(grid), dim3(256), 0, st, labels_sorted, n, d_count, row_order, rank,
                           best, labels_out, medoids_out);
    }
    FAL_CHECK_HIP(hipGetLastError());
    *d_noise_out = rank + n;
    return FAL_OK;
}

extern "C" {

int fal_refine_clusters(fal_ctx* ctx, int32_t* labels, int64_t n, const float* precursor_mz_sorted,
                        const float* rt_sorted, double tol, int tol_is_da, double rt_tol, int64_t* n_clusters) {
    fal::CallScope _call(ctx);
    FAL_REQUIRE(ctx && n_clusters && n >= 0 && n < (int64_t)INT32_MAX, FAL_EINVAL, "fal_refine_clusters: bad argument");
    const int64_t C = *n_clusters;
    FAL_REQUIRE(C >= 0 && C <= n, FAL_EINVAL, "fal_refine_clusters: *n_clusters must hold the DBSCAN cluster count");
    if (n == 0 || C == 0) {
        *n_clusters = 0;
        return FAL_OK;
    }
    FAL_REQUIRE(labels && precursor_mz_sorted, FAL_EINVAL, "fal_refine_clusters: NULL array");
    int64_t *d_in = nullptr, *d_out = nullptr;
    FAL_TRY(ctx->reserve(SLOT_MISC2, sizeof(int64_t) * 4, (void**)&d_in));
    FAL_CHECK_HIP(hipMemcpyAsync(d_in, &C, sizeof(int64_t), hipMemcpyHostToDevice, ctx->stream));
    ctx->stage_reset(ST_TAIL);
    FAL_TRY(refine_dev(ctx, labels, n, precursor_mz_sorted, rt_sorted, tol, tol_is_da, rt_tol, d_in, &d_out));
    FAL_CHECK_HIP(hipMemcpyAsync(n_clusters, d_out, sizeof(int64_t), hipMemcpyDeviceToHost, ctx->stream));
    FAL_CHECK_HIP(hipStreamSynchronize(ctx->stream));
    return FAL_OK;
}

int fal_finalize(fal_ctx* ctx, const int32_t* labels_sorted, int64_t n, int64_t n_clusters, const int64_t* row_order,
                 const int32_t* nb_idx, const float* nb_dist, int k, int32_t* labels_out, int32_t* medoids_out,
                 int64_t* n_labels) {
    fal::CallScope _call(ctx);
    FAL_REQUIRE(ctx && n >= 0 && n_clusters >= 0 && n_clusters <= n && k >= 1, FAL_EINVAL, "fal_finalize: bad argument");
    if (n_labels) *n_labels = 0;
    if (n == 0) return FAL_OK;
    FAL_REQUIRE(labels_sorted && row_order && nb_idx && nb_dist && labels_out && medoids_out, FAL_EINVAL,
                "fal_finalize: NULL array");
    int64_t *d_c = nullptr, *d_noise = nullptr;
    FAL_TRY(ctx->reserve(SLOT_MISC2, sizeof(int64_t) * 4, (void**)&d_c));
    FAL_CHECK_HIP(hipMemcpyAsync(d_c, &n_clusters, sizeof(int64_t), hipMemcpyHostToDevice, ctx->stream));
    FAL_TRY(finalize_dev(ctx, labels_sorted, n, d_c, row_order, nb_idx, nb_dist, k, labels_out, medoids_out, &d_noise));
    if (n_labels) {
        int64_t n_noise = 0;
        FAL_CHECK_HIP(hipMemcpyAsync(&n_noise, d_noise, sizeof(int64_t), hipMemcpyDeviceToHost, ctx->stream));
        FAL_CHECK_HIP(hipStreamSynchronize(ctx->stream));
        *n_labels = n_clusters + n_noise;
    }
    return FAL_OK;
}

static int cluster_graph_impl(fal_ctx* ctx, const int32_t* nb_idx, const float* nb_dist, int64_t n, int k, float eps, int method,
                              const float* precursor_mz_sorted, const float* rt_sorted, double tol, int tol_is_da,
                              double rt_tol, const int64_t* row_order, int32_t* labels_sorted_scratch, int32_t* labels_out,
                              int32_t* medoids_out, int64_t* n_clusters, int64_t* n_labels, const int32_t* nb_count = nullptr) {
    FAL_REQUIRE(ctx && n >= 0 && k >= 1 && n < (int64_t)INT32_MAX && n_clusters && n_labels, FAL_EINVAL,
                "fal_cluster_graph: bad argument");
    *n_clusters = *n_labels = 0;
    if (n == 0) return FAL_OK;
    FAL_REQUIRE(nb_idx && nb_dist && precursor_mz_sorted && row_order && labels_sorted_scratch && labels_out && medoids_out,
                FAL_EINVAL, "fal_cluster_graph: NULL array");
    int64_t *d_db = nullptr, *d_cl = nullptr, *d_noise = nullptr;
    const int32_t* extent = nullptr;
    ctx->stage_reset(ST_TAIL);
    if (method < 0) FAL_TRY(dbscan_dev(ctx, nb_idx, nb_dist, n, k, eps, labels_sorted_scratch, &d_db, &extent, nb_count));
    else FAL_TRY(linkage_dev(ctx, nb_idx, nb_dist, n, k, eps, method, labels_sorted_scratch, &d_db));
    FAL_TRY(refine_dev(ctx, labels_sorted_scratch, n, precursor_mz_sorted, rt_sorted, tol, tol_is_da, rt_tol, d_db, &d_cl));
    FAL_TRY(finalize_dev(ctx, labels_sorted_scratch, n, d_cl, row_order, nb_idx, nb_dist, k, labels_out, medoids_out,
                         &d_noise, extent));
    int64_t h[2] = {0, 0};
    FAL_CHECK_HIP(hipMemcpyAsync(&h[0], d_cl, sizeof(int64_t), hipMemcpyDeviceToHost, ctx->stream));
    FAL_CHECK_HIP(hipMemcpyAsync(&h[1], d_noise, sizeof(int64_t), hipMemcpyDeviceToHost, ctx->stream));
    FAL_CHECK_HIP(hipStreamSynchronize(ctx->stream));
    *n_clusters = h[0];
    *n_labels = h[0] + h[1];
    return FAL_OK;
}

int fal_cluster_graph(fal_ctx* ctx, const int32_t* nb_idx, const float* nb_dist, int64_t n, int k, float eps,
                      const float* precursor_mz_sorted, const float* rt_sorted, double tol, int tol_is_da,
                      double rt_tol, const int64_t* row_order, int32_t* labels_sorted_scratch, int32_t* labels_out,
                      int32_t* medoids_out, int64_t* n_clusters, int64_t* n_labels) {
    fal::CallScope _call(ctx);
    return cluster_graph_impl(ctx, nb_idx, nb_dist, n, k, eps, -1, precursor_mz_sorted, rt_sorted, tol, tol_is_da, rt_tol,
                              row_order, labels_sorted_scratch, labels_out, medoids_out, n_clusters, n_labels);
}

int fal_cluster_graph_counted(fal_ctx* ctx, const int32_t* nb_idx, const float* nb_dist, const int32_t* nb_count, int64_t n, int k,
                              float eps, const float* precursor_mz_sorted, const float* rt_sorted, double tol, int tol_is_da,
                              double rt_tol, const int64_t* row_order, int32_t* labels_sorted_scratch, int32_t* labels_out,
                              int32_t* medoids_out, int64_t* n_clusters, int64_t* n_labels) {
    fal::CallScope _call(ctx);
    FAL_REQUIRE(nb_count || n == 0, FAL_EINVAL, "fal_cluster_graph_counted: NULL nb_count");
    return cluster_graph_impl(ctx, nb_idx, nb_dist, n, k, eps, -1, precursor_mz_sorted, rt_sorted, tol, tol_is_da, rt_tol,
                              row_order, labels_sorted_scratch, labels_out, medoids_out, n_clusters, n_labels, nb_count);
}

int fal_cluster_graph_linkage(fal_ctx* ctx, const int32_t* nb_idx, const float* nb_dist, int64_t n, int k, float threshold,
                              int method, const float* precursor_mz_sorted, const float* rt_sorted, double tol, int tol_is_da,
                              double rt_tol, const int64_t* row_order, int32_t* labels_sorted_scratch, int32_t* labels_out,
                              int32_t* medoids_out, int64_t* n_clusters, int64_t* n_labels) {
    fal::CallScope _call(ctx);
    FAL_REQUIRE(method >= 0 && method <= 2, FAL_EINVAL, "fal_cluster_graph_linkage: method must be 0 (single), 1 (complete) or 2 (average)");
    FAL_REQUIRE(threshold < 1.0f, FAL_EUNSUPPORTED, "fal_cluster_graph_linkage: the threshold must be below 1 (the distance of a missing pair)");
    return cluster_graph_impl(ctx, nb_idx, nb_dist, n, k, threshold, method, precursor_mz_sorted, rt_sorted, tol, tol_is_da, rt_tol,
                              row_order, labels_sorted_scratch, labels_out, medoids_out, n_clusters, n_labels);
}

}
```

falcon_amd/device.py:

```python
from __future__ import annotations

import ctypes as C
from typing import Optional, Sequence

import numpy as np

from . import _lib
from ._lib import FalconHipError, check


def _torch():
    import torch
    return torch


class Context:

    def __init__(self, device: int = 0):
        torch = _torch()
        self.lib = _lib.load()
        if not torch.cuda.is_available():
            raise FalconHipError("no HIP device visible to torch; falcon_amd has no CPU fallback")
        self.device = int(device)
        self.tdev = torch.device("cuda", self.device)
        torch.cuda.set_device(self.device)
        stream = torch.cuda.current_stream(self.device).cuda_stream
        h = C.c_void_p()
        check(self.lib.fal_ctx_create(self.device, C.c_void_p(stream), 0, C.byref(h)), "fal_ctx_create")
        self._h = h

    def close(self):
        if getattr(self, "_h", None):
            self.lib.fal_ctx_destroy(self._h)
            self._h = None

    def __del__(self):
        try:
            self.close()
        except Exception:
            pass

    h2d_bytes = 0

    def to_dev(self, a, dtype=None):
        torch = _torch()
        if isinstance(a, torch.Tensor):
            if not a.is_cuda:
                self.h2d_bytes += a.numel() * a.element_size()
            t = a.to(self.tdev, non_blocking=True)
            return t.to(dtype).contiguous() if dtype is not None else t.contiguous()
        t = torch.from_numpy(np.ascontiguousarray(a))
        if dtype is not None:
            t = t.to(dtype)
        self.h2d_bytes += t.numel() * t.element_size()
        return t.to(self.tdev)

    def empty(self, shape, dtype):
        return _torch().empty(shape, dtype=dtype, device=self.tdev)

    @staticmethod
    def _p(t):
        return C.c_void_p(0) if t is None else C.c_void_p(t.data_ptr())

    def sync(self):
        check(self.lib.fal_ctx_sync(self._h), "fal_ctx_sync")

    def plan(self, n: int, low_dim: int = 400, k_ann: int = 128, n_probe: int = 16, batch_size: int = 2 ** 15):
        check(self.lib.fal_ctx_plan(self._h, int(n), int(low_dim), int(k_ann), int(n_probe), int(batch_size)), "fal_ctx_plan")

    def trim(self):
        check(self.lib.fal_ctx_trim(self._h), "fal_ctx_trim")

    def enable_timing(self, on: bool = True):
        check(self.lib.fal_ctx_enable_timing(self._h, int(on)))

    def stage_ms(self, stage: str):
        ms, k = C.c_float(), C.c_int64()
        check(self.lib.fal_ctx_stage_ms(self._h, _lib.STAGES[stage], C.byref(ms), C.byref(k)))
        return ms.value, k.value

    def counter(self, which: int) -> int:
        v = C.c_int64()
        check(self.lib.fal_ctx_counter(self._h, int(which), C.byref(v)))
        return int(v.value)

    def to_vector_indices(self, mz, min_mz: float, bin_size: float):
        torch = _torch()
        mz = self.to_dev(mz, torch.float32)
        out = self.empty((mz.numel(),), torch.int32)
        check(self.lib.fal_to_vector_indices(self._h, self._p(mz), mz.numel(), min_mz, bin_size, self._p(out)),
              "fal_to_vector_indices")
        return out

    def vectorize(self, mz, intensity, indptr, row_order, min_mz: float, bin_size: float, n_bins: int,
                  low_dim: int, seed: int = 0, normalize: bool = True, dtype: str = "f32", width: Optional[int] = None):
        torch = _torch()
        mz = self.to_dev(mz, torch.float32)
        intensity = self.to_dev(intensity, torch.float32)
        indptr = self.to_dev(indptr, torch.int64)
        row_order = None if row_order is None else self.to_dev(row_order, torch.int64)
        n = indptr.numel() - 1 if row_order is None else row_order.numel()
        w = int(low_dim if width is None else width)
        out2 = None
        if dtype in ("f32+f16", "f16+image"):
            out, out2 = self.empty((n, w), torch.float32), self.empty((n, w), torch.float16)
            code = _lib.FAL_OUT_F32_F16 if dtype == "f32+f16" else _lib.FAL_OUT_F16_IMAGE
        elif dtype == "split16":
            out, code = self.empty((n, 2, w), torch.float16), _lib.FAL_DTYPE_SPLIT16
        elif dtype in ("f16", "float16"):
            out, code = self.empty((n, w), torch.float16), _lib.FAL_DTYPE_F16
        else:
            out, code = self.empty((n, w), torch.float32), _lib.FAL_DTYPE_F32
        check(self.lib.fal_vectorize_rows(self._h, self._p(mz), self._p(intensity), self._p(indptr), self._p(row_order),
                                          n, float(min_mz), float(bin_size), int(n_bins), int(low_dim), w, int(seed),
                                          int(normalize), code, self._p(out), self._p(out2)), "fal_vectorize_rows")
        return out if out2 is None else (out, out2)


    def ivf_build(self, X, bucket_off: np.ndarray, n_list: np.ndarray, kmeans_iters: int = 10,
                  X16=None, Xpre=None, Xkm=None, prefilter_which: int = 1) -> "IvfIndex":
        torch = _torch()
        if X is not None:
            assert X.dtype == torch.float32 and X.is_contiguous() and X.device == self.tdev
            n, d = X.shape
        else:
            assert X16 is not None
            n, d = X16.shape[0], X16.shape[-1]
        bo = np.ascontiguousarray(bucket_off, np.int64)
        nl = np.ascontiguousarray(n_list, np.int32)
        h = C.c_void_p()
        if Xkm is not None:
            assert Xkm.dtype == torch.float16 and Xkm.is_contiguous() and Xkm.device == self.tdev and tuple(Xkm.shape) == (n, d)
        check(self.lib.fal_ivf_build_x16(self._h, self._p(X), self._p(Xkm), n, d, bo.ctypes.data_as(C.c_void_p), len(nl),
                                         nl.ctypes.data_as(C.c_void_p), int(kmeans_iters), C.byref(h)), "fal_ivf_build")
        index = IvfIndex(self, h, X, bo, nl, n, d)
        index.Xkm = Xkm
        if X16 is not None:
            assert X16.dtype == torch.float16 and X16.is_contiguous() and X16.device == self.tdev
            planes = 2 if X16.dim() == 3 else 1
            check(self.lib.fal_ivf_attach_f16(h, self._p(X16), planes), "fal_ivf_attach_f16")
            index.X16 = X16
        if Xpre is not None:
            assert Xpre.dtype == torch.float16 and Xpre.is_contiguous() and Xpre.device == self.tdev and Xpre.shape == (n, d)
            check(self.lib.fal_ivf_attach_prefilter_ex(h, self._p(Xpre), int(prefilter_which)), "fal_ivf_attach_prefilter_ex")
            index.Xpre = Xpre
        return index


    def sort_by_precursor(self, precursor_mz):
        torch = _torch()
        pmz = self.to_dev(precursor_mz, torch.float32)
        n = pmz.numel()
        order = self.empty((n,), torch.int64)
        mzs = self.empty((n,), torch.float32)
        check(self.lib.fal_sort_by_precursor(self._h, self._p(pmz), n, self._p(order), self._p(mzs)),
              "fal_sort_by_precursor")
        return order, mzs

    def gather_f32(self, src, order):
        torch = _torch()
        src = self.to_dev(src, torch.float32)
        out = self.empty((order.numel(),), torch.float32)
        check(self.lib.fal_gather_f32(self._h, self._p(src), self._p(order), order.numel(), self._p(out)),
              "fal_gather_f32")
        return out

    N_WINDOWS = 1 << 14

    def window_counts(self, precursor_mzs, mz_interval: float):
        torch = _torch()
        pmz = [self.to_dev(x, torch.float32) for x in precursor_mzs]
        n_parts = len(pmz)
        if n_parts == 0:
            return np.zeros((0, 0), np.int64)
        counts = self.empty((n_parts, self.N_WINDOWS), torch.int32)
        if getattr(self, "_wc_host", None) is None or self._wc_host.numel() < n_parts * (self.N_WINDOWS + 2):
            self._wc_host = torch.empty(n_parts * (self.N_WINDOWS + 2), dtype=torch.int32, pin_memory=True)
        host = self._wc_host
        ptrs = (C.c_void_p * n_parts)(*[x.data_ptr() if x.numel() else None for x in pmz])
        ns = (C.c_int64 * n_parts)(*[x.numel() for x in pmz])
        check(self.lib.fal_window_counts(self._h, ptrs, ns, n_parts, float(mz_interval), self.N_WINDOWS, self._p(counts),
                                         C.c_void_p(host.data_ptr())), "fal_window_counts")
        self.sync()
        h = host.numpy()
        last = h[n_parts * self.N_WINDOWS: n_parts * (self.N_WINDOWS + 2)].reshape(n_parts, 2)
        last = last[last[:, 0] <= last[:, 1], 1]
        width = int(last.max()) + 1 if len(last) else 0
        return h[: n_parts * self.N_WINDOWS].reshape(n_parts, self.N_WINDOWS)[:, :width].astype(np.int64)

    def window_select(self, precursor_mz, mz_interval: float, owner: np.ndarray, rank: int):
        torch = _torch()
        pmz = self.to_dev(precursor_mz, torch.float32)
        n = pmz.numel()
        own = np.full(self.N_WINDOWS, -1, np.int32)
        own[:len(owner)] = owner
        if len(owner):
            own[len(owner):] = owner[-1]
        own_d = self.to_dev(own, torch.int32)
        rows = self.empty((max(n, 1),), torch.int64)
        mzs = self.empty((max(n, 1),), torch.float32)
        m = C.c_int64()
        check(self.lib.fal_window_select(self._h, self._p(pmz), n, float(mz_interval), self.N_WINDOWS, self._p(own_d), int(rank),
                                         self._p(rows), self._p(mzs), C.byref(m)), "fal_window_select")
        return rows[: m.value], mzs[: m.value]

    def precursor_splits(self, mz_sorted, tol: float, mode: str, batch_size: int, mz_interval: float = 1.0,
                         chunk_last: bool = True) -> np.ndarray:
        torch = _torch()
        mzs = self.to_dev(mz_sorted, torch.float32)
        n = mzs.numel()
        cap = n + 2
        out = np.empty(cap, np.int64)
        k = C.c_int64()
        check(self.lib.fal_precursor_splits(self._h, self._p(mzs), n, float(tol), int(mode == "Da"), int(batch_size),
                                            float(mz_interval or 0.0), int(chunk_last),
                                            out.ctypes.data_as(C.c_void_p), cap, C.byref(k)), "fal_precursor_splits")
        return out[:k.value].copy()

    def filter_neighbors(self, sim, idx, mz_sorted, rt_sorted, tol: float, mode: str, rt_tol, n_neighbors: int):
        torch = _torch()
        n, k_ann = idx.shape
        nb_idx = self.empty((n, n_neighbors), torch.int32)
        nb_dist = self.empty((n, n_neighbors), torch.float32)
        check(self.lib.fal_filter_neighbors(self._h, self._p(sim), self._p(idx), n, k_ann, self._p(mz_sorted),
                                            self._p(rt_sorted), float(tol), int(mode == "Da"),
                                            -1.0 if rt_tol is None else float(rt_tol), int(n_neighbors),
                                            self._p(nb_idx), self._p(nb_dist)), "fal_filter_neighbors")
        return nb_idx, nb_dist

    SCALING = {None: 0, "off": 0, "root": 1, "log": 2, "rank": 3}

    def process_spectra(self, mz, intensity, indptr, precursor_mz, precursor_charge, min_peaks: int,
                        min_mz_range: float, mz_min=None, mz_max=None, remove_precursor_tolerance=None,
                        min_intensity=None, max_peaks_used=None, scaling=None):
        torch = _torch()
        mz = self.to_dev(mz, torch.float64)
        intensity = self.to_dev(intensity, torch.float32)
        indptr = self.to_dev(indptr, torch.int64)
        pmz = self.to_dev(precursor_mz, torch.float64)
        charge = self.to_dev(precursor_charge, torch.int32)
        n, nnz = indptr.numel() - 1, mz.numel()
        if scaling not in self.SCALING:
            raise ValueError(f"unknown scaling {scaling!r}")
        valid = self.empty((n,), torch.int32)
        out_indptr = self.empty((n + 1,), torch.int64)
        out_mz = self.empty((max(nnz, 1),), torch.float32)
        out_it = self.empty((max(nnz, 1),), torch.float32)
        nan = float("nan")
        check(self.lib.fal_process_spectra(
            self._h, self._p(mz), self._p(intensity), self._p(indptr), n, nnz, self._p(pmz), self._p(charge),
            int(min_peaks), float(min_mz_range), nan if mz_min is None else float(mz_min),
            nan if mz_max is None else float(mz_max),
            -1.0 if remove_precursor_tolerance is None else float(remove_precursor_tolerance),
            -1.0 if min_intensity is None else float(min_intensity), 0 if max_peaks_used is None else int(max_peaks_used),
            self.SCALING[scaling], self._p(valid), self._p(out_indptr), self._p(out_mz), self._p(out_it)),
            "fal_process_spectra")
        nnz_out = int(out_indptr[-1].item())
        return valid.bool(), out_indptr, out_mz[:nnz_out], out_it[:nnz_out]

    def decode_peaks(self, payload, arrays, spectra):
        torch = _torch()
        arrays = np.ascontiguousarray(arrays, np.int64).reshape(-1, 4)
        spectra = np.ascontiguousarray(spectra, np.int64).reshape(-1, 2)
        payload = np.frombuffer(payload, np.uint8) if isinstance(payload, (bytes, bytearray, memoryview)) else payload
        n = len(spectra)
        flags, counts = arrays[:, 3], arrays[:, 2]
        cnt = np.maximum(counts, 0)
        codec = flags & _lib.PEAK_NUMPRESS_MASK
        nbytes = cnt * np.where(flags & _lib.PEAK_F64, 8, 4) * np.where(flags & _lib.PEAK_PAIRS, 2, 1)
        linear = np.where(cnt == 0, 8, np.where(cnt == 1, 12, 16 + (9 * (cnt - 2) + 1) // 2))
        nbytes = np.select([codec == _lib.PEAK_NUMPRESS_LINEAR, codec == _lib.PEAK_NUMPRESS_PIC,
                            codec == _lib.PEAK_NUMPRESS_SLOF], [linear, (9 * cnt + 1) // 2, 8 + 2 * cnt], nbytes)
        inflate_bytes = int(((nbytes + 7) // 8 * 8)[(flags & _lib.PEAK_ZLIB) != 0].sum() + (cnt * 8)[codec != 0].sum())
        ma = spectra[:, 0]
        ok = (ma >= 0) & (ma < len(arrays))
        nnz = int(np.maximum(counts[ma[ok]], 0).sum()) if len(arrays) else 0
        indptr = self.empty((n + 1,), torch.int64)
        mz = self.empty((max(nnz, 1),), torch.float64)
        it = self.empty((max(nnz, 1),), torch.float32)
        status = self.empty((max(n, 1),), torch.int32)
        d_payload = self.to_dev(payload, torch.uint8) if len(payload) else None
        d_arrays = self.to_dev(arrays) if len(arrays) else None
        d_spectra = self.to_dev(spectra) if n else None
        check(self.lib.fal_decode_peaks(self._h, self._p(d_payload), len(payload), self._p(d_arrays), len(arrays),
                                        self._p(d_spectra), n, inflate_bytes, nnz, self._p(indptr), self._p(mz), self._p(it),
                                        self._p(status)), "fal_decode_peaks")
        return indptr, mz[:nnz], it[:nnz], status[:n]

    def _text_to_dev(self, text):
        torch = _torch()
        if isinstance(text, torch.Tensor):
            return self.to_dev(text, torch.uint8)
        raw = np.frombuffer(text, np.uint8) if isinstance(text, (bytes, bytearray, memoryview)) else np.asarray(text, np.uint8)
        if not raw.flags.writeable:
            raw = raw.copy()
        return self.to_dev(raw) if len(raw) else self.empty((0,), torch.uint8)

    def _text_index(self, name, d_text):
        counts = (C.c_int64 * 4)()
        check(getattr(self.lib, name)(self._h, self._p(d_text) if d_text.numel() else None, d_text.numel(), counts), name)
        return tuple(int(c) for c in counts)

    def mgf_index(self, d_text):
        return self._text_index("fal_mgf_index", d_text)

    def mgf_parse(self, d_text, n: int, nnz: int):
        torch = _torch()
        m = max(n, 1)
        indptr, mz, it = self.empty((n + 1,), torch.int64), self.empty((max(nnz, 1),), torch.float64), self.empty((max(nnz, 1),), torch.float32)
        pmz, rt = self.empty((m,), torch.float64), self.empty((m,), torch.float64)
        charge, has_charge, status = (self.empty((m,), torch.int32) for _ in range(3))
        title, span = self.empty((m, 2), torch.int64), self.empty((m, 2), torch.int64)
        check(self.lib.fal_mgf_parse(self._h, self._p(d_text) if d_text.numel() else None, d_text.numel(), n, nnz, self._p(indptr),
                                     self._p(mz), self._p(it), self._p(pmz), self._p(charge), self._p(has_charge), self._p(rt),
                                     self._p(title), self._p(span), self._p(status)), "fal_mgf_parse")
        return indptr, mz[:nnz], it[:nnz], pmz[:n], charge[:n], has_charge[:n], rt[:n], title[:n], span[:n], status[:n]

    def parse_mgf(self, text):
        d_text = self._text_to_dev(text)
        n, nnz, flags, lines = self.mgf_index(d_text)
        if flags:
            return dict(flags=flags, lines=lines)
        indptr, mz, it, *cols = self.mgf_parse(d_text, n, nnz)
        pmz, charge, has_charge, rt, title, span, status = (c.cpu().numpy() for c in cols)
        return dict(flags=0, lines=lines, indptr=indptr, mz=mz, intensity=it, precursor_mz=pmz, charge=charge,
                    has_charge=has_charge.astype(bool), retention_time=rt, title=title, span=span, status=status)

    def _mgf_entries(self, mz, intensity, indptr, rows, precursor_mz, retention_time, charge, cluster, title, title_ptr):
        torch = _torch()
        cols = dict(mz=self.to_dev(mz, torch.float32), intensity=self.to_dev(intensity, torch.float32),
                    indptr=self.to_dev(indptr, torch.int64), rows=self.to_dev(rows, torch.int32),
                    precursor_mz=self.to_dev(precursor_mz, torch.float32), retention_time=self.to_dev(retention_time, torch.float32),
                    charge=self.to_dev(charge, torch.int32), cluster=self.to_dev(cluster, torch.int64),
                    title=self._text_to_dev(title), title_ptr=self.to_dev(title_ptr, torch.int64))
        n = int(cols["rows"].shape[0])
        for name in ("precursor_mz", "retention_time", "charge", "cluster"):
            if cols[name].shape[0] != n:
                raise ValueError(f"format_mgf: {name} has {cols[name].shape[0]} entries for {n} rows")
        if cols["title_ptr"].shape[0] != n + 1 or cols["indptr"].shape[0] < 1 or cols["mz"].shape != cols["intensity"].shape:
            raise ValueError("format_mgf: title_ptr needs one entry more than rows, indptr at least one, mz and intensity the same size")
        return cols

    def _mgf_entry_args(self, c, with_title: bool):
        head = [self._p(c["mz"]), self._p(c["intensity"]), self._p(c["indptr"]), c["indptr"].shape[0] - 1, c["mz"].shape[0],
                self._p(c["rows"]), c["rows"].shape[0], self._p(c["precursor_mz"]), self._p(c["retention_time"]), self._p(c["charge"]),
                self._p(c["cluster"])]
        return head + ([self._p(c["title"])] if with_title else []) + [self._p(c["title_ptr"]), c["title"].numel()]

    def mgf_write_sizes(self, cols):
        torch = _torch()
        n = int(cols["rows"].shape[0])
        sizes, offsets = self.empty((max(n, 1),), torch.int64), self.empty((n + 1,), torch.int64)
        total = C.c_int64(0)
        check(self.lib.fal_mgf_write_sizes(self._h, *self._mgf_entry_args(cols, False), self._p(sizes), self._p(offsets),
                                           C.byref(total)), "fal_mgf_write_sizes")
        return sizes[:n], offsets, int(total.value)

    def mgf_write(self, cols, offsets, first: int, last: int, out, host_out=None):
        if host_out is not None and (not host_out.is_pinned() or host_out.numel() != out.numel()):
            raise ValueError("mgf_write: host_out must be pinned and of out's size")
        check(self.lib.fal_mgf_write(self._h, *self._mgf_entry_args(cols, True), self._p(offsets), int(first), int(last),
                                     self._p(out) if out.numel() else None, out.numel(),
                                     self._p(host_out) if host_out is not None and out.numel() else None), "fal_mgf_write")

    def format_mgf(self, mz, intensity, indptr, rows, precursor_mz, retention_time, charge, cluster, title, title_ptr,
                   max_bytes: Optional[int] = None, copy: bool = True):
        torch = _torch()
        if max_bytes is None:
            from .ms_io.mgf_io import DEFAULT_CHUNK_BYTES as max_bytes
        cols = self._mgf_entries(mz, intensity, indptr, rows, precursor_mz, retention_time, charge, cluster, title, title_ptr)
        n = int(cols["rows"].shape[0])
        if n == 0:
            return
        _, offsets, total = self.mgf_write_sizes(cols)
        off = offsets.cpu().numpy()
        cuts = [0]
        while cuts[-1] < n:
            last = int(np.searchsorted(off, off[cuts[-1]] + max(int(max_bytes), 1), side="right")) - 1
            cuts.append(min(max(last, cuts[-1] + 1), n))
        cap = int(max(off[b] - off[a] for a, b in zip(cuts[:-1], cuts[1:])))
        d_out = self.empty((max(cap, 1),), torch.uint8)
        h_out = torch.empty((max(cap, 1),), dtype=torch.uint8, pin_memory=True)
        for a, b in zip(cuts[:-1], cuts[1:]):
            need = int(off[b] - off[a])
            self.mgf_write(cols, offsets, a, b, d_out[:need], h_out[:need])
            chunk = h_out[:need].numpy()
            yield chunk.copy() if copy else chunk

    def mzml_index(self, d_text):
        return self._text_index("fal_mzml_index", d_text)

    def mzml_parse(self, d_text, n: int):
        torch = _torch()
        m = max(n, 1)
        payload = self.empty((d_text.numel() + 16 * n,), torch.uint8)
        status, charge = self.empty((m,), torch.int32), self.empty((m,), torch.int32)
        ident, span = self.empty((m, 2), torch.int64), self.empty((m, 2), torch.int64)
        pmz, rt = self.empty((m,), torch.float64), self.empty((m,), torch.float64)
        arrays = self.empty((2 * m, 4), torch.int64)
        check(self.lib.fal_mzml_parse(self._h, self._p(d_text) if d_text.numel() else None, d_text.numel(), n,
                                      self._p(payload) if payload.numel() else None, payload.numel(), self._p(status), self._p(ident),
                                      self._p(span), self._p(pmz), self._p(charge), self._p(rt), self._p(arrays)), "fal_mzml_parse")
        return payload, status[:n], ident[:n], span[:n], pmz[:n], charge[:n], rt[:n], arrays[:2 * n]

    def scan_mzml(self, text):
        d_text = self._text_to_dev(text)
        n, inside, flags, tags = self.mzml_index(d_text)
        if flags:
            return dict(flags=flags, tags=tags)
        payload, *cols = self.mzml_parse(d_text, n)
        status, ident, span, pmz, charge, rt, arrays = (c.cpu().numpy() for c in cols)
        return dict(flags=0, tags=tags, inside=inside, payload=payload, status=status, id=ident, span=span, precursor_mz=pmz,
                    charge=charge, retention_time=rt, arrays=arrays)

    def consensus_spectra(self, mz, intensity, indptr, labels, medoids, fragment_tol: float, min_fraction: float = 0.25,
                          nnz_cap: Optional[int] = None):
        torch = _torch()
        mz = self.to_dev(mz, torch.float32)
        intensity = self.to_dev(intensity, torch.float32)
        indptr = self.to_dev(indptr, torch.int64)
        labels = self.to_dev(labels, torch.int32)
        medoids = self.to_dev(medoids, torch.int32)
        n, nc = int(labels.shape[0]), int(medoids.shape[0])
        if indptr.shape[0] != n + 1:
            raise ValueError(f"consensus_spectra: indptr has {indptr.shape[0]} entries for {n} labels")
        cap = int(mz.shape[0]) if nnz_cap is None else int(nnz_cap)
        out_indptr = self.empty((nc + 1,), torch.int64)
        out_mz = self.empty((max(cap, 1),), torch.float32)
        out_it = self.empty((max(cap, 1),), torch.float32)
        status = self.empty((max(nc, 1),), torch.int32)
        check(self.lib.fal_consensus_spectra(self._h, self._p(mz), self._p(intensity), self._p(indptr), n, self._p(labels),
                                             self._p(medoids), nc, float(fragment_tol), float(min_fraction), cap,
                                             self._p(out_indptr), self._p(out_mz), self._p(out_it), self._p(status)),
              "fal_consensus_spectra")
        used = int(out_indptr[-1].item())
        if used > cap:
            raise FalconHipError(f"consensus_spectra: the consensus holds {used} peaks, nnz_cap = {cap} is too small")
        return out_indptr, out_mz[:used], out_it[:used], status[:nc]

    def rescore_neighbors(self, nb_idx, nb_dist, mz, intensity, indptr, order, fragment_tol: float, min_matches: int):
        torch = _torch()
        n, k = nb_idx.shape
        mz = self.to_dev(mz, torch.float32)
        intensity = self.to_dev(intensity, torch.float32)
        indptr = self.to_dev(indptr, torch.int64)
        order = self.to_dev(order, torch.int64)
        check(self.lib.fal_rescore_neighbors(self._h, self._p(nb_idx), self._p(nb_dist), n, k, self._p(mz), self._p(intensity),
                                             self._p(indptr), self._p(order), float(fragment_tol), int(min_matches)),
              "fal_rescore_neighbors")
        return nb_dist

    def neighbors_to_csr(self, nb_idx, nb_dist, id_offset: int = 0, out=None, row0: int = 0, nb_count=None, id_map=None):
        torch = _torch()
        n, k = nb_idx.shape
        if out is None:
            out = (self.empty((row0 + n + 1,), torch.int64), self.empty((max((row0 + n) * k, 1),), torch.int32),
                   self.empty((max((row0 + n) * k, 1),), torch.float32))
        indptr, idx, dist = out
        if indptr.numel() < row0 + n + 1:
            raise FalconHipError("neighbors_to_csr: indptr buffer too small")
        check(self.lib.fal_neighbors_to_csr_mapped(self._h, self._p(nb_idx), self._p(nb_dist), self._p(nb_count), n, k,
                                                   self._p(id_map), int(id_offset), int(row0),
                                                   self._p(indptr), self._p(idx), self._p(dist)), "fal_neighbors_to_csr")
        return indptr, idx, dist

    def dbscan(self, nb_idx, nb_dist, eps: float):
        torch = _torch()
        n, k = nb_idx.shape
        labels = self.empty((n,), torch.int32)
        nc = C.c_int64()
        check(self.lib.fal_dbscan(self._h, self._p(nb_idx), self._p(nb_dist), n, k, float(eps), self._p(labels),
                                  C.byref(nc)), "fal_dbscan")
        return labels, int(nc.value)

    def refine_clusters(self, labels, n_clusters: int, mz_sorted, rt_sorted, tol: float, mode: str, rt_tol):
        nc = C.c_int64(int(n_clusters))
        check(self.lib.fal_refine_clusters(self._h, self._p(labels), labels.numel(), self._p(mz_sorted),
                                           self._p(rt_sorted), float(tol), int(mode == "Da"),
                                           -1.0 if rt_tol is None else float(rt_tol), C.byref(nc)),
              "fal_refine_clusters")
        return labels, int(nc.value)

    def finalize(self, labels_sorted, n_clusters: int, order, nb_idx, nb_dist):
        torch = _torch()
        n, k = nb_idx.shape
        labels = self.empty((n,), torch.int32)
        medoids = self.empty((n,), torch.int32)
        nl = C.c_int64()
        check(self.lib.fal_finalize(self._h, self._p(labels_sorted), n, int(n_clusters), self._p(order),
                                    self._p(nb_idx), self._p(nb_dist), k, self._p(labels), self._p(medoids),
                                    C.byref(nl)), "fal_finalize")
        return labels, medoids[:int(nl.value)]


    LINKAGE = {"single": 0, "complete": 1, "average": 2}

    def cluster_graph(self, nb_idx, nb_dist, eps: float, mz_sorted, rt_sorted, tol: float, mode: str, rt_tol, order,
                      linkage: Optional[str] = None, nb_count=None):
        torch = _torch()
        n, k = nb_idx.shape
        lab_sorted = self.empty((n,), torch.int32)
        labels = self.empty((n,), torch.int32)
        medoids = self.empty((n,), torch.int32)
        nc, nl = C.c_int64(), C.c_int64()
        tail = (self._p(mz_sorted), self._p(rt_sorted), float(tol), int(mode == "Da"),
                -1.0 if rt_tol is None else float(rt_tol), self._p(order), self._p(lab_sorted), self._p(labels),
                self._p(medoids), C.byref(nc), C.byref(nl))
        if linkage is None and nb_count is not None:
            check(self.lib.fal_cluster_graph_counted(self._h, self._p(nb_idx), self._p(nb_dist), self._p(nb_count), n, k,
                                                     float(eps), *tail), "fal_cluster_graph_counted")
        elif linkage is None:
            check(self.lib.fal_cluster_graph(self._h, self._p(nb_idx), self._p(nb_dist), n, k, float(eps), *tail),
                  "fal_cluster_graph")
        else:
            check(self.lib.fal_cluster_graph_linkage(self._h, self._p(nb_idx), self._p(nb_dist), n, k, float(eps),
                                                     self.LINKAGE[linkage], *tail), "fal_cluster_graph_linkage")
        return labels, medoids[:int(nl.value)], lab_sorted, int(nc.value)

    def linkage_cluster(self, nb_idx, nb_dist, threshold: float, linkage: str):
        torch = _torch()
        n, k = nb_idx.shape
        labels = self.empty((n,), torch.int32)
        nc = C.c_int64()
        check(self.lib.fal_linkage_cluster(self._h, self._p(nb_idx), self._p(nb_dist), n, k, float(threshold),
                                           self.LINKAGE[linkage], self._p(labels), C.byref(nc)), "fal_linkage_cluster")
        return labels, int(nc.value)

    def _peaks(self, mz, intensity, indptr, order):
        torch = _torch()
        mz, intensity = self.to_dev(mz, torch.float32), self.to_dev(intensity, torch.float32)
        if mz.numel() == 0:
            mz, intensity = self.empty((1,), torch.float32), self.empty((1,), torch.float32)
        return mz, intensity, self.to_dev(indptr, torch.int64), self.to_dev(order, torch.int64)

    @staticmethod
    def _check_order(order, indptr, n_out: int, what: str):
        if order.numel() == 0:
            return
        lo, hi = (int(x) for x in _torch().aminmax(order))
        if lo < 0 or hi >= min(int(n_out), int(indptr.numel()) - 1):
            raise ValueError(f"{what}: row_order holds rows in [{lo}, {hi}], outside the {n_out} output rows / "
                             f"{int(indptr.numel()) - 1} CSR rows (run a subset as a compact CSR with order = arange)")

    def exact_edges(self, mz, intensity, indptr, order, splits, fragment_tol: float, min_matches: int, threshold: float,
                    max_edges: Optional[int] = None):
        torch = _torch()
        mz, intensity, indptr, order = self._peaks(mz, intensity, indptr, order)
        n = order.numel()
        self._check_order(order, indptr, int(indptr.numel()) - 1, "exact_edges")
        sp = np.ascontiguousarray(splits, dtype=np.int64)
        if max_edges is None:
            nb = np.diff(sp)
            max_edges = int((nb * (nb - 1)).sum())
        ptr = self.empty((n + 1,), torch.int64)
        idx = self.empty((max(max_edges, 1),), torch.int32)
        dist = self.empty((max(max_edges, 1),), torch.float64)
        m = C.c_int64()
        check(self.lib.fal_exact_edges(self._h, self._p(mz), self._p(intensity), self._p(indptr), self._p(order), n,
                                       sp.ctypes.data_as(C.c_void_p), len(sp), float(fragment_tol), int(min_matches),
                                       float(threshold), self._p(ptr), self._p(idx), self._p(dist), int(max_edges), C.byref(m)),
              "fal_exact_edges")
        return ptr, idx[:m.value], dist[:m.value]

    def linkage_cluster_csr(self, indptr_csr, idx, dist, threshold: float, linkage: str, mz=None, intensity=None, indptr=None,
                            order=None, fragment_tol: float = 0.0, min_matches: int = 0):
        torch = _torch()
        n = indptr_csr.numel() - 1
        peaks = (None,) * 4 if mz is None else self._peaks(mz, intensity, indptr, order)
        labels = self.empty((max(n, 1),), torch.int32)
        nc = C.c_int64()
        check(self.lib.fal_linkage_cluster_csr(self._h, self._p(indptr_csr), self._p(idx), self._p(dist), n, float(threshold),
                                               self.LINKAGE[linkage], *(self._p(t) for t in peaks), float(fragment_tol),
                                               int(min_matches), self._p(labels), C.byref(nc)), "fal_linkage_cluster_csr")
        return labels[:n], int(nc.value)

    def cluster_exact(self, mz, intensity, indptr, order, splits, fragment_tol: float, min_matches: int, threshold: float,
                      linkage: str, mz_sorted, rt_sorted, tol: float, mode: str, rt_tol):
        torch = _torch()
        mz, intensity, indptr, order = self._peaks(mz, intensity, indptr, order)
        n = order.numel()
        self._check_order(order, indptr, n, "cluster_exact")
        sp = np.ascontiguousarray(splits, dtype=np.int64)
        lab_sorted = self.empty((n,), torch.int32)
        labels = self.empty((n,), torch.int32)
        medoids = self.empty((n,), torch.int32)
        nc, nl = C.c_int64(), C.c_int64()
        check(self.lib.fal_cluster_exact(self._h, self._p(mz), self._p(intensity), self._p(indptr), self._p(order), n,
                                         sp.ctypes.data_as(C.c_void_p), len(sp), float(fragment_tol), int(min_matches),
                                         float(threshold), self.LINKAGE[linkage], self._p(mz_sorted), self._p(rt_sorted),
                                         float(tol), int(mode == "Da"), -1.0 if rt_tol is None else float(rt_tol),
                                         self._p(lab_sorted), self._p(labels), self._p(medoids), C.byref(nc), C.byref(nl)),
              "fal_cluster_exact")
        return labels, medoids[:int(nl.value)], lab_sorted, int(nc.value)


    def assign_nearest(self, q_mz, q_intensity, q_indptr, q_precursor_mz, q_rt, l_mz, l_intensity, l_indptr, l_precursor_mz, l_rt,
                       tol: float, mode: str, rt_tol, fragment_tol: float, min_matches: int):
        torch = _torch()
        q_pmz, l_pmz = self.to_dev(q_precursor_mz, torch.float32), self.to_dev(l_precursor_mz, torch.float32)
        nq, nl = int(q_pmz.numel()), int(l_pmz.numel())
        if rt_tol is not None and nq and nl and (q_rt is None or l_rt is None):
            raise ValueError("assign_nearest: rt_tol needs the retention times of both sides")
        q_mz, q_intensity, q_indptr, _ = self._peaks(q_mz, q_intensity, q_indptr, np.zeros(0, np.int64))
        l_mz, l_intensity, l_indptr, _ = self._peaks(l_mz, l_intensity, l_indptr, np.zeros(0, np.int64))
        if q_indptr.numel() != nq + 1 or l_indptr.numel() != nl + 1:
            raise ValueError(f"assign_nearest: indptr has {q_indptr.numel()} / {l_indptr.numel()} entries for {nq} / {nl} spectra")
        q_rt = None if q_rt is None or rt_tol is None else self.to_dev(q_rt, torch.float32)
        l_rt = None if l_rt is None or rt_tol is None else self.to_dev(l_rt, torch.float32)
        best_row = self.empty((nq,), torch.int32)
        best_dist = self.empty((nq,), torch.float32)
        n_cand = self.empty((nq,), torch.int32)
        ptr = lambda t: self._p(t if t is not None and t.numel() else None)
        check(self.lib.fal_assign_nearest(self._h, ptr(q_mz), ptr(q_intensity), ptr(q_indptr), ptr(q_pmz), ptr(q_rt), nq, ptr(l_mz),
                                          ptr(l_intensity), ptr(l_indptr), ptr(l_pmz), ptr(l_rt), nl, float(tol), int(mode == "Da"),
                                          -1.0 if rt_tol is None else float(rt_tol), float(fragment_tol), int(min_matches),
                                          ptr(best_row), ptr(best_dist), ptr(n_cand)), "fal_assign_nearest")
        return best_row, best_dist, n_cand


class IvfIndex:

    def __init__(self, ctx: Context, handle, X, bucket_off, n_list, n, d):
        self.ctx, self._h, self.X, self.X16, self.Xpre = ctx, handle, X, None, None
        self.bucket_off, self.n_list = bucket_off, n_list
        self.n, self.d = n, d
        t = C.c_int64()
        check(ctx.lib.fal_ivf_total_lists(self._h, C.byref(t)))
        self.total_lists = int(t.value)

    def close(self):
        if getattr(self, "_h", None):
            if getattr(self.ctx, "_h", None):
                self.ctx.lib.fal_ivf_destroy(self._h)
            self._h = None

    def __del__(self):
        try:
            self.close()
        except Exception:
            pass

    def export(self):
        torch = _torch()
        c = self.ctx
        cent = c.empty((self.total_lists, self.d), torch.float32)
        asg = c.empty((self.n,), torch.int32)
        perm = c.empty((self.n,), torch.int32)
        off = c.empty((self.total_lists + 1,), torch.int64)
        check(c.lib.fal_ivf_export(c._h, self._h, c._p(cent), c._p(asg), c._p(perm), c._p(off)), "fal_ivf_export")
        return cent, asg, perm, off

    def search(self, n_probe: int, k_ann: int):
        torch = _torch()
        c = self.ctx
        sim = c.empty((self.n, k_ann), torch.float32)
        idx = c.empty((self.n, k_ann), torch.int32)
        check(c.lib.fal_ivf_search_topk(c._h, self._h, int(n_probe), int(k_ann), c._p(sim), c._p(idx)),
              "fal_ivf_search_topk")
        return sim, idx

    def search_neighbors(self, n_probe: int, k_ann: int, mz_sorted, rt_sorted, tol: float, mode: str, rt_tol,
                         n_neighbors: int):
        torch = _torch()
        c = self.ctx
        nb_idx = c.empty((self.n, n_neighbors), torch.int32)
        nb_dist = c.empty((self.n, n_neighbors), torch.float32)
        self.nb_count = c.empty((self.n,), torch.int32)
        check(c.lib.fal_ivf_search_neighbors(c._h, self._h, int(n_probe), int(k_ann), c._p(mz_sorted), c._p(rt_sorted),
                                             float(tol), int(mode == "Da"), -1.0 if rt_tol is None else float(rt_tol),
                                             int(n_neighbors), c._p(nb_idx), c._p(nb_dist), c._p(self.nb_count)),
              "fal_ivf_search_neighbors")
        return nb_idx, nb_dist


def get_dim(min_mz: float, max_mz: float, bin_size: float):
    lib = _lib.load()
    dim, s, e = C.c_uint32(), C.c_float(), C.c_float()
    check(lib.fal_get_dim(min_mz, max_mz, bin_size, C.byref(dim), C.byref(s), C.byref(e)), "fal_get_dim")
    return int(dim.value), float(s.value), float(e.value)


def row_width(low_dim: int) -> int:
    lib = _lib.load()
    w = C.c_uint32()
    if int(low_dim) < 1:
        raise FalconHipError(f"low_dim must be a positive integer (got {low_dim})")
    check(lib.fal_row_width(int(low_dim), C.byref(w)), "fal_row_width")
    return int(w.value)


def hash_lookup(n_bins: int, low_dim: int, seed: int = 0) -> np.ndarray:
    lib = _lib.load()
    out = np.empty(n_bins, np.uint32)
    check(lib.fal_hash_lookup(n_bins, low_dim, seed, out.ctypes.data_as(C.c_void_p)), "fal_hash_lookup")
    return out
```

include/falcon_hip.h:

```cpp
#ifndef FALCON_HIP_H
#define FALCON_HIP_H

#include <stdint.h>

#ifdef __cplusplus
extern "C" {
#endif

#define FAL_OK            0
#define FAL_EINVAL       -1
#define FAL_EHIP         -2
#define FAL_ENOMEM       -3
#define FAL_ENODEV       -4
#define FAL_EUNSUPPORTED -5
#define FAL_EINTERNAL    -6

#define FAL_DTYPE_F32 0
#define FAL_DTYPE_F16 1
#define FAL_DTYPE_SPLIT16 2
#define FAL_OUT_F32_F16   3
#define FAL_OUT_F16_IMAGE 4

#define FAL_MAX_LOW_DIM   1024
#define FAL_MAX_K_ANN      256
#define FAL_MAX_N_PROBE    128
#define FAL_MAX_N_LIST  131072

typedef struct fal_ctx fal_ctx;
typedef struct fal_ivf fal_ivf;

int         fal_version(void);
const char* fal_last_error(void);
int fal_device_count(int* count);
int fal_ctx_create(int device, void* stream, int own_stream, fal_ctx** out);
int fal_ctx_destroy(fal_ctx* ctx);
int fal_ctx_sync(fal_ctx* ctx);
int fal_ctx_plan(fal_ctx* ctx, int64_t n, int low_dim, int k_ann, int n_probe, int64_t batch_size);
int fal_ctx_trim(fal_ctx* ctx);
int fal_ctx_stage_ms(fal_ctx* ctx, int stage, float* ms, int64_t* launches);
int fal_ctx_enable_timing(fal_ctx* ctx, int on);
int fal_ctx_counter(fal_ctx* ctx, int which, int64_t* value);

int fal_get_dim(float min_mz, float max_mz, float bin_size,
                uint32_t* dim, float* start_dim, float* end_dim);

int fal_hash_lookup(uint32_t n_bins, uint32_t low_dim, uint32_t seed, uint32_t* out_table);

int fal_to_vector_indices(fal_ctx* ctx, const float* mz, int64_t nnz,
                          double min_mz, double bin_size, int32_t* out_indices);

int fal_vectorize(fal_ctx* ctx, const float* mz, const float* intensity,
                  const int64_t* indptr, const int64_t* row_order, int64_t n,
                  double min_mz, double bin_size, uint32_t n_bins,
                  uint32_t low_dim, uint32_t seed, int normalize, int out_dtype, void* out);
int fal_vectorize_pair(fal_ctx* ctx, const float* mz, const float* intensity, const int64_t* indptr,
                       const int64_t* row_order, int64_t n, double min_mz, double bin_size, uint32_t n_bins,
                       uint32_t low_dim, uint32_t seed, int normalize, float* out_f32, void* out_f16);
int fal_vectorize_f16_image(fal_ctx* ctx, const float* mz, const float* intensity, const int64_t* indptr,
                            const int64_t* row_order, int64_t n, double min_mz, double bin_size, uint32_t n_bins,
                            uint32_t low_dim, uint32_t seed, int normalize, float* out_f32_image, void* out_f16);

int fal_row_width(uint32_t low_dim, uint32_t* row_width);
int fal_vectorize_rows(fal_ctx* ctx, const float* mz, const float* intensity, const int64_t* indptr,
                       const int64_t* row_order, int64_t n, double min_mz, double bin_size, uint32_t n_bins,
                       uint32_t low_dim, uint32_t row_width, uint32_t seed, int normalize, int out_mode,
                       void* out, void* out2 );

int fal_precursor_splits(fal_ctx* ctx, const float* precursor_mz_sorted , int64_t n,
                         double tol, int tol_is_da, int64_t batch_size,
                         double mz_interval, int chunk_last,
                         int64_t* splits_out , int64_t max_splits, int64_t* n_splits);

int fal_window_counts(fal_ctx* ctx, const float* const* precursor_mz , const int64_t* n , int n_parts,
                      double mz_interval, int64_t n_windows, int32_t* counts, int32_t* counts_host );
int fal_window_select(fal_ctx* ctx, const float* precursor_mz, int64_t n, double mz_interval, int64_t n_windows,
                      const int32_t* owner, int rank, int64_t* rows_out, float* mz_out, int64_t* count );

int fal_ivf_build(fal_ctx* ctx, const float* X, int64_t n, int low_dim,
                  const int64_t* bucket_off, int64_t n_buckets, const int32_t* n_list,
                  int kmeans_iters, fal_ivf** out);
int fal_ivf_build_x16(fal_ctx* ctx, const float* X, const void* X16, int64_t n, int low_dim,
                      const int64_t* bucket_off, int64_t n_buckets, const int32_t* n_list,
                      int kmeans_iters, fal_ivf** out);
int fal_ivf_attach_f16(fal_ivf* ivf, const void* X16, int planes);
int fal_ivf_attach_prefilter(fal_ivf* ivf, const void* X16);
int fal_ivf_attach_prefilter_ex(fal_ivf* ivf, const void* X16, int which);
int fal_ivf_destroy(fal_ivf* ivf);
int fal_ivf_total_lists(const fal_ivf* ivf, int64_t* total_lists);
int fal_ivf_export(fal_ctx* ctx, const fal_ivf* ivf, float* centroids, int32_t* assign,
                   int32_t* perm, int64_t* list_off);

int fal_ivf_search_topk(fal_ctx* ctx, const fal_ivf* ivf, int n_probe, int k_ann,
                        float* sim, int32_t* idx);

int fal_filter_neighbors(fal_ctx* ctx, const float* sim, const int32_t* idx, int64_t n,
                         int k_ann, const float* precursor_mz_sorted, const float* rt_sorted,
                         double tol, int tol_is_da, double rt_tol, int n_neighbors,
                         int32_t* nb_idx, float* nb_dist);

int fal_ivf_search_neighbors(fal_ctx* ctx, const fal_ivf* ivf, int n_probe, int k_ann,
                             const float* precursor_mz_sorted, const float* rt_sorted,
                             double tol, int tol_is_da, double rt_tol, int n_neighbors,
                             int32_t* nb_idx, float* nb_dist, int32_t* nb_count );

int fal_rescore_neighbors(fal_ctx* ctx, const int32_t* nb_idx, float* nb_dist, int64_t n, int k,
                          const float* mz, const float* intensity, const int64_t* indptr,
                          const int64_t* row_order, double fragment_tol, int min_matches);

int fal_neighbors_to_csr(fal_ctx* ctx, const int32_t* nb_idx, const float* nb_dist,
                         const int32_t* nb_count ,
                         int64_t n, int k, int64_t id_offset, int64_t row0, int64_t* indptr_out,
                         int32_t* idx_out, float* dist_out);
int fal_neighbors_to_csr_mapped(fal_ctx* ctx, const int32_t* nb_idx, const float* nb_dist,
                                const int32_t* nb_count, int64_t n, int k,
                                const int64_t* id_map , int64_t id_offset, int64_t row0,
                                int64_t* indptr_out, int32_t* idx_out, float* dist_out);

int fal_dbscan(fal_ctx* ctx, const int32_t* nb_idx, const float* nb_dist, int64_t n, int k,
               float eps, int32_t* labels, int64_t* n_clusters );

int fal_refine_clusters(fal_ctx* ctx, int32_t* labels, int64_t n,
                        const float* precursor_mz_sorted, const float* rt_sorted,
                        double tol, int tol_is_da, double rt_tol,
                        int64_t* n_clusters );

int fal_finalize(fal_ctx* ctx, const int32_t* labels_sorted, int64_t n, int64_t n_clusters,
                 const int64_t* row_order, const int32_t* nb_idx, const float* nb_dist, int k,
                 int32_t* labels_out, int32_t* medoids_out, int64_t* n_labels );

int fal_cluster_graph(fal_ctx* ctx, const int32_t* nb_idx, const float* nb_dist, int64_t n, int k,
                      float eps, const float* precursor_mz_sorted, const float* rt_sorted,
                      double tol, int tol_is_da, double rt_tol, const int64_t* row_order,
                      int32_t* labels_sorted_scratch, int32_t* labels_out, int32_t* medoids_out,
                      int64_t* n_clusters , int64_t* n_labels );

int fal_cluster_graph_counted(fal_ctx* ctx, const int32_t* nb_idx, const float* nb_dist, const int32_t* nb_count,
                              int64_t n, int k, float eps, const float* precursor_mz_sorted, const float* rt_sorted,
                              double tol, int tol_is_da, double rt_tol, const int64_t* row_order,
                              int32_t* labels_sorted_scratch, int32_t* labels_out, int32_t* medoids_out,
                              int64_t* n_clusters , int64_t* n_labels );

int fal_linkage_cluster(fal_ctx* ctx, const int32_t* nb_idx, const float* nb_dist, int64_t n, int k,
                        float threshold, int method, int32_t* labels, int64_t* n_clusters );
int fal_cluster_graph_linkage(fal_ctx* ctx, const int32_t* nb_idx, const float* nb_dist, int64_t n, int k,
                              float threshold, int method, const float* precursor_mz_sorted,
                              const float* rt_sorted, double tol, int tol_is_da, double rt_tol,
                              const int64_t* row_order, int32_t* labels_sorted_scratch, int32_t* labels_out,
                              int32_t* medoids_out, int64_t* n_clusters , int64_t* n_labels );

int fal_exact_edges(fal_ctx* ctx, const float* mz, const float* intensity, const int64_t* indptr, const int64_t* row_order,
                    int64_t n, const int64_t* splits , int64_t n_splits, double fragment_tol, int min_matches,
                    double threshold, int64_t* csr_indptr, int32_t* csr_idx, double* csr_dist, int64_t max_edges,
                    int64_t* n_edges );
int fal_linkage_cluster_csr(fal_ctx* ctx, const int64_t* csr_indptr, const int32_t* csr_idx, const double* csr_dist, int64_t n,
                            double threshold, int method, const float* mz, const float* intensity, const int64_t* indptr,
                            const int64_t* row_order, double fragment_tol, int min_matches, int32_t* labels,
                            int64_t* n_clusters );
int fal_cluster_exact(fal_ctx* ctx, const float* mz, const float* intensity, const int64_t* indptr, const int64_t* row_order,
                      int64_t n, const int64_t* splits , int64_t n_splits, double fragment_tol, int min_matches,
                      double threshold, int method, const float* precursor_mz_sorted, const float* rt_sorted, double tol,
                      int tol_is_da, double rt_tol, int32_t* labels_sorted_scratch, int32_t* labels_out, int32_t* medoids_out,
                      int64_t* n_clusters , int64_t* n_labels );

int fal_process_spectra(fal_ctx* ctx, const double* mz, const float* intensity,
                        const int64_t* indptr, int64_t n, int64_t nnz,
                        const double* precursor_mz, const int32_t* precursor_charge,
                        int min_peaks, double min_mz_range, double mz_min, double mz_max,
                        double remove_precursor_tol, double min_intensity, int max_peaks_used,
                        int scaling, int32_t* valid_out, int64_t* out_indptr, float* out_mz,
                        float* out_intensity);

#define FAL_PEAK_F64         1
#define FAL_PEAK_ZLIB        2
#define FAL_PEAK_BIG_ENDIAN  4
#define FAL_PEAK_PAIRS       8
#define FAL_PEAK_NUMPRESS_LINEAR 16
#define FAL_PEAK_NUMPRESS_PIC    32
#define FAL_PEAK_NUMPRESS_SLOF   48
#define FAL_PEAK_NUMPRESS_MASK   48
#define FAL_PEAK_ST_DESC      1
#define FAL_PEAK_ST_BASE64    2
#define FAL_PEAK_ST_HEADER    4
#define FAL_PEAK_ST_CODE      8
#define FAL_PEAK_ST_OVERFLOW 16
#define FAL_PEAK_ST_SHORT    32
#define FAL_PEAK_ST_ADLER    64
#define FAL_PEAK_ST_CAPACITY 128
#define FAL_PEAK_ST_NUMPRESS 256
int fal_decode_peaks(fal_ctx* ctx, const uint8_t* payload, int64_t payload_bytes,
                     const int64_t* arrays, int64_t n_arrays, const int64_t* spectra, int64_t n_spectra,
                     int64_t inflate_bytes, int64_t nnz_cap, int64_t* out_indptr, double* out_mz,
                     float* out_intensity, int32_t* status_out);

#define FAL_MGF_FLAG_BYTES 1
#define FAL_MGF_FLAG_LINES 2
#define FAL_MGF_ST_HOST    1
int fal_mgf_index(fal_ctx* ctx, const uint8_t* text, int64_t n_bytes, int64_t* counts_out);
int fal_mgf_parse(fal_ctx* ctx, const uint8_t* text, int64_t n_bytes, int64_t n_spectra, int64_t nnz_cap,
                  int64_t* out_indptr, double* out_mz, float* out_intensity, double* precursor_mz, int32_t* charge,
                  int32_t* has_charge, double* retention_time, int64_t* title, int64_t* span, int32_t* status_out);

int fal_mgf_write_sizes(fal_ctx* ctx, const float* mz, const float* intensity, const int64_t* indptr, int64_t n_rows, int64_t nnz,
                        const int32_t* rows, int64_t n, const float* precursor_mz, const float* retention_time,
                        const int32_t* charge, const int64_t* cluster, const int64_t* title_ptr, int64_t title_bytes,
                        int64_t* sizes_out, int64_t* offsets_out, int64_t* total_out);
int fal_mgf_write(fal_ctx* ctx, const float* mz, const float* intensity, const int64_t* indptr, int64_t n_rows, int64_t nnz,
                  const int32_t* rows, int64_t n, const float* precursor_mz, const float* retention_time, const int32_t* charge,
                  const int64_t* cluster, const uint8_t* title, const int64_t* title_ptr, int64_t title_bytes,
                  const int64_t* offsets, int64_t first, int64_t last, uint8_t* out, int64_t out_bytes, uint8_t* host_out);

#define FAL_MZML_FLAG_STRUCT 1
#define FAL_MZML_FLAG_MARKUP 2
#define FAL_MZML_FLAG_TAGS   4
#define FAL_MZML_ST_OK   0
#define FAL_MZML_ST_SKIP 1
#define FAL_MZML_ST_HOST 2
int fal_mzml_index(fal_ctx* ctx, const uint8_t* text, int64_t n_bytes, int64_t* counts_out);
int fal_mzml_parse(fal_ctx* ctx, const uint8_t* text, int64_t n_bytes, int64_t n_spectra, uint8_t* payload, int64_t payload_cap,
                   int32_t* status_out, int64_t* id, int64_t* span, double* precursor_mz, int32_t* charge,
                   double* retention_time, int64_t* arrays);

#define FAL_CONS_LDS_PEAKS 4096
#define FAL_CONS_ST_FALLBACK 1
#define FAL_CONS_ST_GLOBAL   2
#define FAL_CONS_ST_CAPACITY 4
int fal_consensus_spectra(fal_ctx* ctx, const float* mz, const float* intensity, const int64_t* indptr, int64_t n,
                          const int32_t* labels, const int32_t* medoids, int64_t n_clusters, double fragment_tol,
                          double min_fraction, int64_t nnz_cap, int64_t* out_indptr, float* out_mz, float* out_intensity,
                          int32_t* status_out);

int fal_assign_nearest(fal_ctx* ctx, const float* q_mz, const float* q_intensity, const int64_t* q_indptr,
                       const float* q_precursor_mz, const float* q_rt, int64_t nq, const float* l_mz, const float* l_intensity,
                       const int64_t* l_indptr, const float* l_precursor_mz, const float* l_rt, int64_t nl, double tol,
                       int tol_is_da, double rt_tol, double fragment_tol, int min_matches, int32_t* best_row, float* best_dist,
                       int32_t* n_cand);

int fal_sort_by_precursor(fal_ctx* ctx, const float* precursor_mz, int64_t n,
                          int64_t* order_out, float* mz_sorted_out);
int fal_gather_f32(fal_ctx* ctx, const float* src, const int64_t* order, int64_t n, float* out);

#ifdef __cplusplus
}
#endif
#endif
```

Before: 198.1 million spectra/s.

## Add tiled bucket-local DBSCAN and tail pipeline using per-tile LDS union-find

Adds a new graph clustering path that groups rows into tiles along precursor bucket boundaries. Each tile then runs DBSCAN core detection and union-find in LDS with one workgroup, followed by a per-tile bitonic sort of members, refinement that skips the per-cluster sort, and medoid selection. The aim is to replace global-memory union-find and sorting passes with workgroup-local work, which needs fewer global atomics and fewer launches. The path depends on every neighbour lying inside its row's bucket tile and errors out otherwise. Tiles that overflow LDS fall back to rescanning the neighbour lists.

```diff
diff --git a/falcon_amd/_lib.py b/falcon_amd/_lib.py
--- a/falcon_amd/_lib.py
+++ b/falcon_amd/_lib.py
@@ -91,6 +91,10 @@
                            c_double, c_void_p, c_void_p, c_void_p, c_void_p, P(c_int64), P(c_int64)], c_int),
     "fal_cluster_graph_counted": ([c_void_p, c_void_p, c_void_p, c_void_p, c_int64, c_int, c_float, c_void_p, c_void_p, c_double,
                                    c_int, c_double, c_void_p, c_void_p, c_void_p, c_void_p, P(c_int64), P(c_int64)], c_int),
+    "fal_cluster_graph_tiled": ([c_void_p, c_void_p, c_void_p, c_void_p, c_int64, c_int, c_float, c_void_p, c_int64, c_void_p,
+                                 c_void_p, c_double, c_int, c_double, c_void_p, c_void_p, c_void_p, c_void_p, P(c_int64),
+                                 P(c_int64)], c_int),
+    "fal_graph_tile_limits": ([P(c_int), P(c_int)], None),
     "fal_cluster_graph_linkage": ([c_void_p, c_void_p, c_void_p, c_int64, c_int, c_float, c_int, c_void_p, c_void_p, c_double, c_int,
                                    c_double, c_void_p, c_void_p, c_void_p, c_void_p, P(c_int64), P(c_int64)], c_int),
     "fal_linkage_cluster": ([c_void_p, c_void_p, c_void_p, c_int64, c_int, c_float, c_int, c_void_p, P(c_int64)], c_int),
diff --git a/falcon_amd/cluster/cluster.py b/falcon_amd/cluster/cluster.py
--- a/falcon_amd/cluster/cluster.py
+++ b/falcon_amd/cluster/cluster.py
@@ -292,7 +292,8 @@
             labels, medoids = c.finalize(lab, n_cl, order, nb_idx, nb_dist)
         else:
             labels, medoids, _, _ = c.cluster_graph(nb_idx, nb_dist, p.eps, mzs, rts, precursor_tol_mass,
-                                                    precursor_tol_mode, rt_tol, order, linkage=hier, nb_count=st["nb_count"])
+                                                    precursor_tol_mode, rt_tol, order, linkage=hier, nb_count=st["nb_count"],
+                                                    splits=st["splits"])
             last = dict(nb_idx=nb_idx, nb_dist=nb_dist, nb_count=st["nb_count"], order=order, n_list=st["n_list"],
                         splits=st["splits"])
             index.close()
diff --git a/falcon_amd/csrc/common.h b/falcon_amd/csrc/common.h
--- a/falcon_amd/csrc/common.h
+++ b/falcon_amd/csrc/common.h
@@ -36,7 +36,7 @@
     } while (0)
 
 constexpr int kNumStages = 9;
-constexpr int kNumSlots = 50;
+constexpr int kNumSlots = 51;
 enum Stage { ST_VECTORIZE = 0, ST_BUILD = 1, ST_COARSE = 2, ST_SCAN = 3, ST_SELECT = 4,
              ST_FILTER = 5, ST_DBSCAN = 6, ST_TAIL = 7,
              ST_KERNEL = 8 };
@@ -68,7 +68,7 @@
     fal::Scratch scratch[fal::kNumSlots];
     int32_t* fb_host = nullptr;
     int32_t* zero_dev = nullptr;
-    int64_t counters[10] = {0, 0, 0, 0, 0, 0, 0, 0, 0, 0};
+    int64_t counters[11] = {0, 0, 0, 0, 0, 0, 0, 0, 0, 0, 0};
 
     struct TextIndex {
         const void* text = nullptr;
diff --git a/falcon_amd/csrc/core.hip b/falcon_amd/csrc/core.hip
--- a/falcon_amd/csrc/core.hip
+++ b/falcon_amd/csrc/core.hip
@@ -6,6 +6,7 @@
 #include "hash.h"
 #include "scan.h"
 #include "ivf.h"
+#include "tiles.h"
 #include <algorithm>
 
 #include <chrono>
@@ -291,6 +292,7 @@
         FAL_TRY(c->reserve(SLOT_SIMS, cap + sizeof(float) * kSimsSlack, &p));
     }
     for (int slot : {SLOT_DB, SLOT_DB2, SLOT_TAIL, SLOT_TAIL2, SLOT_FIN, SLOT_FIN2}) FAL_TRY(c->reserve(slot, 8 * nn + 4096, &p));
+    FAL_TRY(c->reserve(SLOT_TILES, 40 * (2 * nn / (size_t)kTileRows + 4) + 4096, &p));
     for (int slot = 0; slot < fal::kNumSlots; ++slot) c->release(slot);
     return FAL_OK;
 }
@@ -329,7 +331,7 @@
 }
 
 int fal_ctx_counter(fal_ctx* c, int which, int64_t* value) {
-    FAL_REQUIRE(c && value && which >= 0 && which < 10, FAL_EINVAL, "fal_ctx_counter: bad argument");
+    FAL_REQUIRE(c && value && which >= 0 && which < 11, FAL_EINVAL, "fal_ctx_counter: bad argument");
     *value = c->counters[which];
     if (which == 5) *value = c->fb_host ? (int64_t)c->fb_host[0] + (int64_t)c->fb_host[2] : 0;
     return FAL_OK;
diff --git a/falcon_amd/csrc/ivf.h b/falcon_amd/csrc/ivf.h
--- a/falcon_amd/csrc/ivf.h
+++ b/falcon_amd/csrc/ivf.h
@@ -15,7 +15,8 @@
        SLOT_MGF = 37, SLOT_MGF2 = 38, SLOT_MGF3 = 39, SLOT_MGF4 = 40, SLOT_MGF5 = 41,
        SLOT_ASSIGN = 42, SLOT_ASSIGN2 = 43,
        SLOT_MZML = 44, SLOT_MZML2 = 45, SLOT_MZML3 = 46, SLOT_MZML4 = 47, SLOT_MZML5 = 48,
-       SLOT_MGFW = 49 };
+       SLOT_MGFW = 49,
+       SLOT_TILES = 50 };
 static_assert(SLOT_MGF2 == SLOT_MGF + 1 && SLOT_MGF3 == SLOT_MGF + 2 && SLOT_MGF4 == SLOT_MGF + 3 && SLOT_MZML2 == SLOT_MZML + 1 &&
                   SLOT_MZML3 == SLOT_MZML + 2 && SLOT_MZML4 == SLOT_MZML + 3,
               "fal::matches (textscan.h) addresses the four slots of an index as first + i");
diff --git a/falcon_amd/csrc/tail.hip b/falcon_amd/csrc/tail.hip
--- a/falcon_amd/csrc/tail.hip
+++ b/falcon_amd/csrc/tail.hip
@@ -1,6 +1,9 @@
 #include <math.h>
+#include <stdlib.h>
+#include <algorithm>
 #include "common.h"
 #include "ivf.h"
+#include "tiles.h"
 #include "util.h"
 
 namespace fal {
@@ -173,7 +176,7 @@
                                                     const int64_t* __restrict__ d_count,
                                                     const float* __restrict__ mz, const float* __restrict__ rt,
                                                     double tol, int is_da, double rt_tol, RefineScratch S,
-                                                    int32_t* __restrict__ sub, int32_t* __restrict__ n_sub) {
+                                                    int32_t* __restrict__ sub, int32_t* __restrict__ n_sub, int sorted) {
     const int lane = threadIdx.x;
     const int64_t C = *d_count;
     const bool use_rt = rt != nullptr && rt_tol >= 0.0;
@@ -240,7 +243,7 @@
         const bool small = m <= kLdsMembers;
         const RefineScratch& W = small ? L : S;
         const int64_t wo = small ? 0 : o;
-        sort_rows(rows + o, W.stack + wo, m, lane);
+        if (!sorted) sort_rows(rows + o, W.stack + wo, m, lane);
         int32_t* A = W.t_a + wo;
         for (int e = lane; e < m; e += 64) W.val[wo + e] = mz[rows[o + e]];
         __syncthreads();
@@ -426,34 +429,377 @@
     }
 }
 
+constexpr int kTileThreads = 512;
+constexpr int32_t kCore = -2;
+constexpr int32_t kNoVote = 0x7fffffff;
+
+__device__ __forceinline__ int block_excl_scan(int v, int* s_w, int* total) {
+    const int lane = threadIdx.x & 63, w = threadIdx.x >> 6;
+    const int inc = wave_prefix_sum(v);
+    if (lane == 63) s_w[w] = inc;
+    __syncthreads();
+    int off = 0, tot = 0;
+#pragma unroll
+    for (int q = 0; q < kTileThreads / 64; ++q) {
+        const int s = s_w[q];
+        off += q < w ? s : 0;
+        tot += s;
+    }
+    __syncthreads();
+    *total = tot;
+    return off + inc - v;
+}
+
+__device__ __forceinline__ int32_t tile_find(int32_t* parent, int32_t x) {
+    int32_t p = __hip_atomic_load(&parent[x], __ATOMIC_RELAXED, __HIP_MEMORY_SCOPE_WORKGROUP);
+    while (p != x) {
+        const int32_t g = __hip_atomic_load(&parent[p], __ATOMIC_RELAXED, __HIP_MEMORY_SCOPE_WORKGROUP);
+        if (g != p) __hip_atomic_store(&parent[x], g, __ATOMIC_RELAXED, __HIP_MEMORY_SCOPE_WORKGROUP);
+        x = p;
+        p = g;
+    }
+    return x;
+}
+__device__ __forceinline__ int32_t tile_find_final(const int32_t* parent, int32_t x) {
+    int32_t p = __hip_atomic_load(&parent[x], __ATOMIC_RELAXED, __HIP_MEMORY_SCOPE_WORKGROUP);
+    while (p != x) {
+        x = p;
+        p = __hip_atomic_load(&parent[x], __ATOMIC_RELAXED, __HIP_MEMORY_SCOPE_WORKGROUP);
+    }
+    return x;
+}
+__device__ __forceinline__ void tile_union(int32_t* parent, int32_t a, int32_t b) {
+    while (true) {
+        a = tile_find(parent, a);
+        b = tile_find(parent, b);
+        if (a == b) return;
+        if (a < b) { const int32_t t = a; a = b; b = t; }
+        if (atomicCAS(&parent[a], a, b) == a) return;
+    }
+}
+
+__global__ __launch_bounds__(kTileThreads) void tile_dbscan_kernel(const int32_t* __restrict__ nb_idx, const float* __restrict__ nb_dist,
+                                                                   const int32_t* __restrict__ count, int64_t n, int k, float eps,
+                                                                   const int32_t* __restrict__ tile_row, int nt, int lds_words,
+                                                                   int32_t* __restrict__ labels, int32_t* __restrict__ cnt) {
+    extern __shared__ __align__(16) int32_t tile_lds[];
+    __shared__ int s_w[kTileThreads / 64];
+    __shared__ int s_err, s_nlab, s_ne;
+    const int tid = threadIdx.x, lane = tid & 63, sub = tid & 7;
+    const int t = blockIdx.x;
+    const int r0 = tile_row[t], m = tile_row[t + 1] - r0;
+    int32_t *parent = tile_lds, *vote = tile_lds + m, *rank = tile_lds + 2 * m, *ext_l = tile_lds + 3 * m;
+    uint32_t* edges = reinterpret_cast<uint32_t*>(tile_lds + 4 * m);
+    const int cap = lds_words - 4 * m;
+    if (tid == 0) s_err = s_nlab = s_ne = 0;
+    for (int li = tid; li < m; li += kTileThreads) ext_l[li] = min(count[r0 + li], k);
+    __syncthreads();
+    constexpr int U = 4;
+    for (int e0 = tid; e0 < (m + 7) / 8 * 64; e0 += U * kTileThreads) {
+        int li[U], ext[U], most = 0;
+        bool c[U];
+        bool bad = false;
+#pragma unroll
+        for (int u = 0; u < U; ++u) {
+            li[u] = (e0 + u * kTileThreads) >> 3;
+            ext[u] = li[u] < m ? ext_l[li[u]] : 0;
+            most = max(most, ext[u]);
+            c[u] = false;
+        }
+        for (int s = sub; __any(s < most); s += 8) {
+            int32_t j[U];
+            float d[U];
+#pragma unroll
+            for (int u = 0; u < U; ++u) {
+                const bool on = s < ext[u];
+                j[u] = on ? nb_idx[(int64_t)(r0 + li[u]) * k + s] : -1;
+                d[u] = on ? nb_dist[(int64_t)(r0 + li[u]) * k + s] : INFINITY;
+            }
+#pragma unroll
+            for (int u = 0; u < U; ++u) {
+                bool edge = false;
+                int lj = 0;
+                if (j[u] >= 0 && (int64_t)j[u] < n) {
+                    lj = j[u] - r0;
+                    if (lj < 0 || lj >= m) bad = true;
+                    else edge = lj != li[u] && d[u] <= eps;
+                }
+                const uint64_t em = __ballot(edge);
+                if (em) {
+                    int base = 0;
+                    if (lane == 0) base = atomicAdd(&s_ne, __popcll(em));
+                    base = __shfl(base, 0, 64);
+                    const int pos = base + __popcll(em & ((1ull << lane) - 1ull));
+                    if (edge && pos < cap) edges[pos] = ((uint32_t)li[u] << 16) | (uint32_t)lj;
+                }
+                c[u] = c[u] || edge;
+            }
+        }
+        if (bad) s_err = 1;
+#pragma unroll
+        for (int u = 0; u < U; ++u) {
+            const uint64_t any = __ballot(c[u]);
+            if (sub == 0 && li[u] < m) {
+                parent[li[u]] = li[u];
+                vote[li[u]] = ((any >> (lane & ~7)) & 0xffull) ? kCore : kNoVote;
+            }
+        }
+    }
+    __syncthreads();
+    const int ne = s_ne;
+    if (ne <= cap) {
+        for (int e = tid; e < ne; e += kTileThreads) {
+            const int li = (int)(edges[e] >> 16), lj = (int)(edges[e] & 0xFFFFu);
+            if (__hip_atomic_load(&vote[lj], __ATOMIC_RELAXED, __HIP_MEMORY_SCOPE_WORKGROUP) == kCore) tile_union(parent, li, lj);
+            else atomicMin(&vote[lj], li);
+        }
+    } else {
+        for (int e = tid; e < m * 8; e += kTileThreads) {
+            const int li = e >> 3;
+            if (vote[li] != kCore) continue;
+            const int64_t i = r0 + li;
+            const int ext = ext_l[li];
+            for (int s = sub; s < ext; s += 8) {
+                const int32_t j = nb_idx[i * k + s];
+                const float d = nb_dist[i * k + s];
+                if (j < 0 || (int64_t)j >= n) continue;
+                const int lj = j - r0;
+                if (lj < 0 || lj >= m || lj == li || !(d <= eps)) continue;
+                if (__hip_atomic_load(&vote[lj], __ATOMIC_RELAXED, __HIP_MEMORY_SCOPE_WORKGROUP) == kCore) tile_union(parent, li, lj);
+                else atomicMin(&vote[lj], li);
+            }
+        }
+    }
+    __syncthreads();
+    for (int li = tid; li < m; li += kTileThreads)
+        if (vote[li] == kCore)
+            __hip_atomic_store(&parent[li], tile_find_final(parent, li), __ATOMIC_RELAXED, __HIP_MEMORY_SCOPE_WORKGROUP);
+    __syncthreads();
+    int n_roots = 0;
+    for (int base = 0; base < m; base += kTileThreads) {
+        const int li = base + tid;
+        const int f = li < m && vote[li] == kCore && parent[li] == li;
+        int tot;
+        const int ex = block_excl_scan(f, s_w, &tot);
+        if (li < m) rank[li] = n_roots + ex;
+        n_roots += tot;
+    }
+    __syncthreads();
+    int mine = 0;
+    for (int li = tid; li < m; li += kTileThreads) {
+        const int32_t v = vote[li];
+        int32_t lab = -1;
+        if (v == kCore) lab = rank[parent[li]];
+        else if (v != kNoVote) lab = rank[parent[v]];
+        labels[r0 + li] = lab;
+        mine += lab >= 0;
+    }
+    if (mine) atomicAdd(&s_nlab, mine);
+    __syncthreads();
+    if (tid == 0) {
+        cnt[t] = n_roots;
+        cnt[nt + t] = s_nlab;
+        cnt[2 * nt + t] = s_err;
+    }
+}
+
+__global__ __launch_bounds__(kTileThreads) void tile_scan_kernel(const int32_t* __restrict__ in, int nt, int ncol,
+                                                                 int32_t* __restrict__ out, int64_t* __restrict__ totals) {
+    __shared__ int s_w[kTileThreads / 64];
+    for (int c = 0; c < ncol; ++c) {
+        int carry = 0;
+        for (int base = 0; base < nt; base += kTileThreads) {
+            const int t = base + (int)threadIdx.x;
+            const int v = t < nt ? in[(int64_t)c * nt + t] : 0;
+            int tot;
+            const int ex = block_excl_scan(v, s_w, &tot);
+            if (t < nt) out[(int64_t)c * (nt + 1) + t] = carry + ex;
+            carry += tot;
+        }
+        if (threadIdx.x == 0) {
+            out[(int64_t)c * (nt + 1) + nt] = carry;
+            totals[c] = carry;
+        }
+    }
+}
+
+__global__ __launch_bounds__(kTileThreads) void tile_members_kernel(const int32_t* __restrict__ tile_row, const int32_t* __restrict__ base,
+                                                                    int nt, int32_t* __restrict__ labels, int64_t* __restrict__ seg,
+                                                                    int32_t* __restrict__ rows) {
+    extern __shared__ __align__(16) int32_t tile_lds[];
+    uint32_t* keys = reinterpret_cast<uint32_t*>(tile_lds);
+    const int tid = threadIdx.x, t = blockIdx.x;
+    const int r0 = tile_row[t], m = tile_row[t + 1] - r0;
+    const int c0 = base[t], m0 = base[nt + 1 + t], n_lab = base[nt + 1 + t + 1] - m0;
+    int P = 2;
+    while (P < m) P <<= 1;
+    for (int li = tid; li < P; li += kTileThreads) {
+        uint32_t key = 0xFFFFFFFFu;
+        if (li < m) {
+            const int32_t l = labels[r0 + li];
+            if (l >= 0) {
+                key = ((uint32_t)l << 16) | (uint32_t)li;
+                labels[r0 + li] = c0 + l;
+            }
+        }
+        keys[li] = key;
+    }
+    __syncthreads();
+    for (int k2 = 2; k2 <= P; k2 <<= 1)
+        for (int j = k2 >> 1; j > 0; j >>= 1) {
+            for (int x = tid; x < P / 2; x += kTileThreads) {
+                const int a = ((x & ~(j - 1)) << 1) | (x & (j - 1)), b = a | j;
+                const uint32_t ka = keys[a], kb = keys[b];
+                if ((ka > kb) == ((a & k2) == 0)) {
+                    keys[a] = kb;
+                    keys[b] = ka;
+                }
+            }
+            __syncthreads();
+        }
+    for (int p = tid; p < n_lab; p += kTileThreads) {
+        const uint32_t key = keys[p];
+        rows[m0 + p] = r0 + (int32_t)(key & 0xFFFFu);
+        if (p == 0 || (keys[p - 1] >> 16) != (key >> 16)) seg[c0 + (int32_t)(key >> 16)] = m0 + p;
+    }
+    if (t == nt - 1 && tid == 0) seg[base[nt]] = base[nt + 1 + nt];
+}
+
+__global__ __launch_bounds__(256) void tile_kept_kernel(const int32_t* __restrict__ cbase, const int32_t* __restrict__ n_sub,
+                                                        int32_t* __restrict__ kept) {
+    __shared__ int s_sum;
+    const int t = blockIdx.x, c0 = cbase[t], c1 = cbase[t + 1];
+    if (threadIdx.x == 0) s_sum = 0;
+    __syncthreads();
+    int v = 0;
+    for (int c = c0 + (int)threadIdx.x; c < c1; c += 256) v += n_sub[c];
+    if (v) atomicAdd(&s_sum, v);
+    __syncthreads();
+    if (threadIdx.x == 0) kept[t] = s_sum;
+}
+
+__global__ __launch_bounds__(kTileThreads) void tile_medoid_kernel(const int32_t* __restrict__ nb_idx, const float* __restrict__ nb_dist,
+                                                                   const int32_t* __restrict__ count, int64_t n, int k,
+                                                                   const int32_t* __restrict__ tile_row, const int32_t* __restrict__ base,
+                                                                   const int32_t* __restrict__ fbase, int nt,
+                                                                   const int32_t* __restrict__ n_sub, const int32_t* __restrict__ rows,
+                                                                   const int32_t* __restrict__ sub, int32_t* __restrict__ labels,
+                                                                   const int64_t* __restrict__ row_order, int32_t* __restrict__ noise,
+                                                                   unsigned long long* __restrict__ best) {
+    extern __shared__ __align__(16) int32_t tile_lds[];
+    __shared__ int s_w[kTileThreads / 64];
+    const int tid = threadIdx.x, t = blockIdx.x;
+    const int r0 = tile_row[t], m = tile_row[t + 1] - r0;
+    const int c0 = base[t], nc = base[t + 1] - c0, m0 = base[nt + 1 + t], nm = base[nt + 1 + t + 1] - m0;
+    const int fb = fbase[t], nf = fbase[t + 1] - fb;
+    int32_t *flab = tile_lds, *size = tile_lds + m;
+    unsigned long long* bestl = reinterpret_cast<unsigned long long*>(tile_lds + 2 * m);
+    int carry = 0;
+    for (int b = 0; b < nc; b += kTileThreads) {
+        const int c = b + tid;
+        const int v = c < nc ? n_sub[c0 + c] : 0;
+        int tot;
+        const int ex = block_excl_scan(v, s_w, &tot);
+        if (c < nc) size[c] = carry + ex;
+        carry += tot;
+    }
+    for (int li = tid; li < m; li += kTileThreads) flab[li] = -1;
+    __syncthreads();
+    for (int p = tid; p < nm; p += kTileThreads) {
+        const int32_t s = sub[m0 + p];
+        if (s >= 0) {
+            const int32_t row = rows[m0 + p];
+            flab[row - r0] = size[labels[row] - c0] + s;
+        }
+    }
+    __syncthreads();
+    for (int c = tid; c < nf; c += kTileThreads) {
+        size[c] = 0;
+        bestl[c] = ~0ull;
+    }
+    __syncthreads();
+    for (int li = tid; li < m; li += kTileThreads) {
+        const int32_t f = flab[li];
+        const int64_t i = r0 + li;
+        labels[i] = f >= 0 ? fb + f : -1;
+        noise[row_order[i]] = f < 0;
+        if (f >= 0) atomicAdd(&size[f], 1);
+    }
+    __syncthreads();
+    for (int li = tid; li < m; li += kTileThreads) {
+        const int32_t f = flab[li];
+        if (f < 0) continue;
+        const int64_t i = r0 + li;
+        float s = 0.f;
+        int same = 0;
+        const int ext = min(count[i], k);
+        for (int s0 = 0; s0 < ext; s0 += 4) {
+            int32_t j4[4];
+            float d4[4];
+#pragma unroll
+            for (int u = 0; u < 4; ++u) {
+                const bool on = s0 + u < ext;
+                j4[u] = on ? nb_idx[i * k + s0 + u] : -1;
+                d4[u] = on ? nb_dist[i * k + s0 + u] : 0.f;
+            }
+#pragma unroll
+            for (int u = 0; u < 4; ++u) {
+                const int32_t j = j4[u];
+                const int lj = j - r0;
+                if (j >= 0 && (int64_t)j < n && lj >= 0 && lj < m && lj != li && flab[lj] == f) {
+                    s += d4[u];
+                    ++same;
+                }
+            }
+        }
+        s += (float)(size[f] - 1 - same);
+        atomicMin(&bestl[f], ((unsigned long long)__float_as_uint(s) << 32) | (unsigned long long)(uint32_t)i);
+    }
+    __syncthreads();
+    for (int c = tid; c < nf; c += kTileThreads) best[fb + c] = bestl[c];
+}
+
 }
 FAL_WARM_KERNEL(fal::refine_kernel);
 
 using namespace fal;
 
-int fal::refine_dev(fal_ctx* ctx, int32_t* labels, int64_t n, const float* mz, const float* rt, double tol, int is_da,
-                    double rt_tol, const int64_t* d_count_in, int64_t** d_count_out) {
-    hipStream_t st = ctx->stream;
+struct RefineArrays {
+    int32_t *counts, *cursor, *n_sub, *rows, *sub;
+    int64_t *seg, *base;
+    RefineScratch S;
+};
+static int refine_arrays(fal_ctx* ctx, int64_t n, RefineArrays* A) {
     const int64_t cmax = n + 1;
-    int32_t *counts = nullptr, *rows = nullptr;
-    int64_t *seg = nullptr, *base = nullptr;
     unsigned char* slab = nullptr;
-    FAL_TRY(ctx->reserve(SLOT_TAIL, sizeof(int32_t) * (size_t)(3 * cmax + 2 * n) + 64, (void**)&counts));
-    int32_t* cursor = counts + cmax;
-    int32_t* n_sub = cursor + cmax;
-    rows = n_sub + cmax;
-    int32_t* sub = rows + n;
-    FAL_TRY(ctx->reserve(SLOT_TAIL2, sizeof(int64_t) * (size_t)(2 * (cmax + 2)), (void**)&seg));
-    base = seg + (cmax + 2);
+    FAL_TRY(ctx->reserve(SLOT_TAIL, sizeof(int32_t) * (size_t)(3 * cmax + 2 * n) + 64, (void**)&A->counts));
+    A->cursor = A->counts + cmax;
+    A->n_sub = A->cursor + cmax;
+    A->rows = A->n_sub + cmax;
+    A->sub = A->rows + n;
+    FAL_TRY(ctx->reserve(SLOT_TAIL2, sizeof(int64_t) * (size_t)(2 * (cmax + 2)), (void**)&A->seg));
+    A->base = A->seg + (cmax + 2);
     const size_t per = 4 * 11 + 8;
     FAL_TRY(ctx->reserve(SLOT_TAIL4, per * (size_t)n + 256, (void**)&slab));
-    RefineScratch S;
+    RefineScratch& S = A->S;
     S.zmd = reinterpret_cast<double*>(slab);
     float* f = reinterpret_cast<float*>(slab + 8 * (size_t)n);
     S.val = f;            S.smin = f + n;       S.smax = f + 2 * n;
     int32_t* q = reinterpret_cast<int32_t*>(f + 3 * n);
     S.ord = q;            S.sid = q + n;        S.zl = q + 2 * n;     S.zr = q + 3 * n;
     S.t_a = q + 4 * n;    S.t_b = q + 5 * n;    S.stack = q + 6 * n;  S.visit = q + 7 * n;
+    return FAL_OK;
+}
+
+int fal::refine_dev(fal_ctx* ctx, int32_t* labels, int64_t n, const float* mz, const float* rt, double tol, int is_da,
+                    double rt_tol, const int64_t* d_count_in, int64_t** d_count_out) {
+    hipStream_t st = ctx->stream;
+    const int64_t cmax = n + 1;
+    RefineArrays A;
+    FAL_TRY(refine_arrays(ctx, n, &A));
+    int32_t *counts = A.counts, *cursor = A.cursor, *n_sub = A.n_sub, *rows = A.rows, *sub = A.sub;
+    int64_t *seg = A.seg, *base = A.base;
+    const RefineScratch& S = A.S;
     const int grid = (int)std::min<int64_t>(ceil_div(n, 256), (int64_t)ctx->num_cus * 16);
     const int cgrid = (int)std::min<int64_t>(cmax, (int64_t)ctx->num_cus * 32);
     FAL_CHECK_HIP(hipMemsetAsync(counts, 0, sizeof(int32_t) * (size_t)(3 * cmax), st));
@@ -463,7 +809,7 @@
         FAL_TRY(device_scan_i32(ctx, counts, cmax, seg, SLOT_TAIL3));
         hipLaunchKernelGGL(member_scatter_kernel, dim3(grid), dim3(256), 0, st, labels, n, seg, cursor, rows);
         hipLaunchKernelGGL(refine_kernel, dim3(cgrid), dim3(64), 0, st, rows, seg, d_count_in, mz,
-                           rt_tol >= 0.0 ? rt : nullptr, tol, is_da, rt_tol, S, sub, n_sub);
+                           rt_tol >= 0.0 ? rt : nullptr, tol, is_da, rt_tol, S, sub, n_sub, 0);
         FAL_TRY(device_scan_i32(ctx, n_sub, cmax, base, SLOT_TAIL3));
         hipLaunchKernelGGL(relabel_kernel, dim3(cgrid), dim3(64), 0, st, rows, seg, d_count_in, sub, base, labels);
     }
@@ -598,6 +944,97 @@
                               row_order, labels_sorted_scratch, labels_out, medoids_out, n_clusters, n_labels, nb_count);
 }
 
+void fal_graph_tile_limits(int* tile_rows, int* max_tile_rows) {
+    if (tile_rows) *tile_rows = kTileRows;
+    if (max_tile_rows) *max_tile_rows = kTileMaxRows;
+}
+
+int fal_cluster_graph_tiled(fal_ctx* ctx, const int32_t* nb_idx, const float* nb_dist, const int32_t* nb_count, int64_t n, int k,
+                            float eps, const int64_t* bucket_off, int64_t n_buckets, const float* precursor_mz_sorted,
+                            const float* rt_sorted, double tol, int tol_is_da, double rt_tol, const int64_t* row_order,
+                            int32_t* labels_sorted_scratch, int32_t* labels_out, int32_t* medoids_out, int64_t* n_clusters,
+                            int64_t* n_labels) {
+    fal::CallScope _call(ctx);
+    FAL_REQUIRE(ctx && n >= 0 && k >= 1 && n < (int64_t)INT32_MAX && n_clusters && n_labels, FAL_EINVAL,
+                "fal_cluster_graph_tiled: bad argument");
+    FAL_REQUIRE(nb_count || n == 0, FAL_EINVAL, "fal_cluster_graph_tiled: NULL nb_count");
+    FAL_REQUIRE(bucket_off && n_buckets >= 0, FAL_EINVAL, "fal_cluster_graph_tiled: NULL bucket table");
+    ctx->counters[10] = 0;
+    std::vector<int32_t> tile_row;
+    int64_t max_rows = 0;
+    const char* sw = getenv("FALCON_GRAPH_TILED");
+    const bool forced_off = sw && sw[0] == '0';
+    const int rc = build_tile_table(bucket_off, n_buckets, n, kTileRows, kTileMaxRows, tile_row, &max_rows);
+    FAL_REQUIRE(rc >= 0, FAL_EINVAL, "fal_cluster_graph_tiled: bucket_off must ascend from 0 to n");
+    if (rc == 1 || forced_off || n == 0)
+        return cluster_graph_impl(ctx, nb_idx, nb_dist, n, k, eps, -1, precursor_mz_sorted, rt_sorted, tol, tol_is_da, rt_tol,
+                                  row_order, labels_sorted_scratch, labels_out, medoids_out, n_clusters, n_labels, nb_count);
+    *n_clusters = *n_labels = 0;
+    FAL_REQUIRE(nb_idx && nb_dist && precursor_mz_sorted && row_order && labels_sorted_scratch && labels_out && medoids_out,
+                FAL_EINVAL, "fal_cluster_graph_tiled: NULL array");
+    ctx->counters[10] = 1;
+    hipStream_t st = ctx->stream;
+    const int nt = (int)tile_row.size() - 1;
+    int32_t* labels = labels_sorted_scratch;
+    int32_t* tt = nullptr;
+    const size_t words = (size_t)(nt + 1) + 3 * (size_t)nt + 3 * (size_t)(nt + 1) + (size_t)nt + (size_t)(nt + 1);
+    FAL_TRY(ctx->reserve(SLOT_TILES, sizeof(int32_t) * (words + 2) + sizeof(int64_t) * 4, (void**)&tt));
+    int32_t *d_tile_row = tt, *cnt = d_tile_row + (nt + 1), *base = cnt + 3 * (size_t)nt, *kept = base + 3 * (size_t)(nt + 1),
+            *fbase = kept + nt;
+    int64_t* totals = reinterpret_cast<int64_t*>(tt + ((words + 1) & ~(size_t)1));
+    FAL_TRY(ctx->upload(d_tile_row, tile_row.data(), sizeof(int32_t) * (size_t)(nt + 1)));
+    const int64_t cmax = n + 1;
+    RefineArrays A;
+    FAL_TRY(refine_arrays(ctx, n, &A));
+    int32_t *n_sub = A.n_sub, *rows = A.rows, *sub = A.sub, *noise = nullptr;
+    int64_t *seg = A.seg, *rank = nullptr;
+    const RefineScratch& S = A.S;
+    unsigned long long* best = nullptr;
+    FAL_TRY(ctx->reserve(SLOT_FIN, sizeof(int32_t) * (size_t)(n + 2), (void**)&noise));
+    FAL_TRY(ctx->reserve(SLOT_FIN2, sizeof(unsigned long long) * (size_t)(cmax + 1), (void**)&best));
+    FAL_TRY(ctx->reserve(SLOT_FIN3, sizeof(int64_t) * (size_t)(n + 1), (void**)&rank));
+    constexpr size_t kLdsMost = 16 * (size_t)kTileMaxRows + 24 * 1024;
+    const size_t lds_db = std::min<size_t>(32 * (size_t)max_rows, kLdsMost), lds_md = 16 * (size_t)max_rows;
+    size_t lds_mem = 8;
+    while (lds_mem < 4 * (size_t)max_rows) lds_mem <<= 1;
+    if (lds_db > 48 * 1024) {
+        FAL_CHECK_HIP(hipFuncSetAttribute((const void*)tile_dbscan_kernel, hipFuncAttributeMaxDynamicSharedMemorySize, (int)kLdsMost));
+        FAL_CHECK_HIP(hipFuncSetAttribute((const void*)tile_medoid_kernel, hipFuncAttributeMaxDynamicSharedMemorySize, 16 * kTileMaxRows));
+    }
+    ctx->stage_reset(ST_DBSCAN);
+    ctx->stage_reset(ST_TAIL);
+    {
+        StageScope ts(ctx, ST_DBSCAN);
+        hipLaunchKernelGGL(tile_dbscan_kernel, dim3(nt), dim3(kTileThreads), lds_db, st, nb_idx, nb_dist, nb_count, n, k, eps,
+                           d_tile_row, nt, (int)(lds_db / 4), labels, cnt);
+        hipLaunchKernelGGL(tile_scan_kernel, dim3(1), dim3(kTileThreads), 0, st, cnt, nt, 3, base, totals);
+    }
+    {
+        StageScope ts(ctx, ST_TAIL);
+        hipLaunchKernelGGL(tile_members_kernel, dim3(nt), dim3(kTileThreads), lds_mem, st, d_tile_row, base, nt, labels, seg, rows);
+        hipLaunchKernelGGL(refine_kernel, dim3((unsigned)std::min<int64_t>(cmax, (int64_t)ctx->num_cus * 32)), dim3(64), 0, st, rows,
+                           seg, totals, precursor_mz_sorted, rt_tol >= 0.0 ? rt_sorted : nullptr, tol, tol_is_da, rt_tol, S, sub,
+                           n_sub, 1);
+        hipLaunchKernelGGL(tile_kept_kernel, dim3(nt), dim3(256), 0, st, base, n_sub, kept);
+        hipLaunchKernelGGL(tile_scan_kernel, dim3(1), dim3(kTileThreads), 0, st, kept, nt, 1, fbase, totals + 3);
+        hipLaunchKernelGGL(tile_medoid_kernel, dim3(nt), dim3(kTileThreads), lds_md, st, nb_idx, nb_dist, nb_count, n, k, d_tile_row,
+                           base, fbase, nt, n_sub, rows, sub, labels, row_order, noise, best);
+        FAL_TRY(device_scan_i32(ctx, noise, n, rank, SLOT_TAIL3));
+        hipLaunchKernelGGL(finalize_kernel, dim3((unsigned)std::min<int64_t>(ceil_div(n, 256), (int64_t)ctx->num_cus * 16)), dim3(256),
+                           0, st, labels, n, totals + 3, row_order, rank, best, labels_out, medoids_out);
+    }
+    FAL_CHECK_HIP(hipGetLastError());
+    int64_t h[3] = {0, 0, 0};
+    FAL_CHECK_HIP(hipMemcpyAsync(&h[0], totals + 2, 2 * sizeof(int64_t), hipMemcpyDeviceToHost, st));
+    FAL_CHECK_HIP(hipMemcpyAsync(&h[2], rank + n, sizeof(int64_t), hipMemcpyDeviceToHost, st));
+    FAL_CHECK_HIP(hipStreamSynchronize(st));
+    FAL_REQUIRE(h[0] == 0, FAL_EINVAL, "fal_cluster_graph_tiled: a stored neighbour id lies outside its row's bucket tile "
+                "(%lld tile(s)): nb_idx and bucket_off do not describe the same partition", (long long)h[0]);
+    *n_clusters = h[1];
+    *n_labels = h[1] + h[2];
+    return FAL_OK;
+}
+
 int fal_cluster_graph_linkage(fal_ctx* ctx, const int32_t* nb_idx, const float* nb_dist, int64_t n, int k, float threshold,
                               int method, const float* precursor_mz_sorted, const float* rt_sorted, double tol, int tol_is_da,
                               double rt_tol, const int64_t* row_order, int32_t* labels_sorted_scratch, int32_t* labels_out,
diff --git a/falcon_amd/csrc/tiles.h b/falcon_amd/csrc/tiles.h
--- /dev/null
+++ b/falcon_amd/csrc/tiles.h
@@ -0,0 +1,36 @@
+#pragma once
+#include <stddef.h>
+#include <stdint.h>
+#include <vector>
+
+namespace fal {
+
+constexpr int kTileRows = 1024;
+constexpr int kTileMaxRows = 8192;
+
+static inline int build_tile_table(const int64_t* bucket_off, int64_t n_buckets, int64_t n, int64_t tile_rows, int64_t max_tile,
+                                   std::vector<int32_t>& tile_row, int64_t* max_rows) {
+    tile_row.clear();
+    *max_rows = 0;
+    if (!bucket_off || n_buckets < 0 || n < 0 || n > (int64_t)INT32_MAX || bucket_off[0] != 0 || bucket_off[n_buckets] != n) return -1;
+    if (tile_rows < 1 || max_tile < tile_rows) return -1;
+    tile_row.push_back(0);
+    int64_t start = 0;
+    for (int64_t b = 0; b < n_buckets; ++b) {
+        const int64_t lo = bucket_off[b], hi = bucket_off[b + 1];
+        if (hi < lo) return -1;
+        if (hi - lo > max_tile) return 1;
+        if (hi - start > tile_rows && lo > start) {
+            tile_row.push_back((int32_t)lo);
+            start = lo;
+        }
+    }
+    if (n > start) tile_row.push_back((int32_t)n);
+    for (size_t t = 0; t + 1 < tile_row.size(); ++t) {
+        const int64_t r = (int64_t)tile_row[t + 1] - tile_row[t];
+        if (r > *max_rows) *max_rows = r;
+    }
+    return 0;
+}
+
+}
diff --git a/falcon_amd/device.py b/falcon_amd/device.py
--- a/falcon_amd/device.py
+++ b/falcon_amd/device.py
@@ -495,8 +495,13 @@
 
     LINKAGE = {"single": 0, "complete": 1, "average": 2}
 
+    def graph_tile_limits(self):
+        t, m = C.c_int(), C.c_int()
+        self.lib.fal_graph_tile_limits(C.byref(t), C.byref(m))
+        return t.value, m.value
+
     def cluster_graph(self, nb_idx, nb_dist, eps: float, mz_sorted, rt_sorted, tol: float, mode: str, rt_tol, order,
-                      linkage: Optional[str] = None, nb_count=None):
+                      linkage: Optional[str] = None, nb_count=None, splits=None):
         torch = _torch()
         n, k = nb_idx.shape
         lab_sorted = self.empty((n,), torch.int32)
@@ -506,7 +511,12 @@
         tail = (self._p(mz_sorted), self._p(rt_sorted), float(tol), int(mode == "Da"),
                 -1.0 if rt_tol is None else float(rt_tol), self._p(order), self._p(lab_sorted), self._p(labels),
                 self._p(medoids), C.byref(nc), C.byref(nl))
-        if linkage is None and nb_count is not None:
+        if linkage is None and nb_count is not None and splits is not None:
+            sp = np.ascontiguousarray(splits, dtype=np.int64)
+            check(self.lib.fal_cluster_graph_tiled(self._h, self._p(nb_idx), self._p(nb_dist), self._p(nb_count), n, k,
+                                                   float(eps), sp.ctypes.data_as(C.c_void_p), len(sp) - 1, *tail),
+                  "fal_cluster_graph_tiled")
+        elif linkage is None and nb_count is not None:
             check(self.lib.fal_cluster_graph_counted(self._h, self._p(nb_idx), self._p(nb_dist), self._p(nb_count), n, k,
                                                      float(eps), *tail), "fal_cluster_graph_counted")
         elif linkage is None:
diff --git a/include/falcon_hip.h b/include/falcon_hip.h
--- a/include/falcon_hip.h
+++ b/include/falcon_hip.h
@@ -139,6 +139,14 @@
                               double tol, int tol_is_da, double rt_tol, const int64_t* row_order,
                               int32_t* labels_sorted_scratch, int32_t* labels_out, int32_t* medoids_out,
                               int64_t* n_clusters , int64_t* n_labels );
+
+int fal_cluster_graph_tiled(fal_ctx* ctx, const int32_t* nb_idx, const float* nb_dist, const int32_t* nb_count,
+                            int64_t n, int k, float eps, const int64_t* bucket_off , int64_t n_buckets,
+                            const float* precursor_mz_sorted, const float* rt_sorted,
+                            double tol, int tol_is_da, double rt_tol, const int64_t* row_order,
+                            int32_t* labels_sorted_scratch, int32_t* labels_out, int32_t* medoids_out,
+                            int64_t* n_clusters , int64_t* n_labels );
+void fal_graph_tile_limits(int* tile_rows, int* max_tile_rows);
 
 int fal_linkage_cluster(fal_ctx* ctx, const int32_t* nb_idx, const float* nb_dist, int64_t n, int k,
                         float threshold, int method, int32_t* labels, int64_t* n_clusters );
```

Measured after the change: 211.1 million spectra/s (median of 6 runs). 1.07x the previous value.
